# spiraldb/vortex

Hardware: AMD Instinct MI355X
Metric: decoded GB/s/GPU (device-resident) per encoding; % HBM roofline (higher is better)
Workload: dtype u32

## Files before the change

include/vortex_gpu.h:

```cpp
#ifndef VORTEX_GPU_H
#define VORTEX_GPU_H

#include <stddef.h>
#include <stdint.h>

#ifdef __cplusplus
extern "C" {
#endif

#define VXG_ABI_VERSION 10

typedef enum vxg_status {
    VXG_OK = 0,
    VXG_ERR_OUT_OF_BOUNDS = 1,
    VXG_ERR_COMPUTE = 2,
    VXG_ERR_INVALID_ARGUMENT = 3,
    VXG_ERR_INVALID_SERDE = 4,
    VXG_ERR_NOT_IMPLEMENTED = 5,
    VXG_ERR_MISMATCHED_TYPES = 6,
    VXG_ERR_ASSERTION_FAILED = 7,
    VXG_ERR_HIP = 8,
    VXG_ERR_OUT_OF_MEMORY = 9
} vxg_status;

enum {
    VXG_ENC_BOOL = 2, VXG_ENC_PRIMITIVE = 3, VXG_ENC_STRUCT = 4, VXG_ENC_VARBIN = 5,
    VXG_ENC_VARBINVIEW = 6, VXG_ENC_SPARSE = 8, VXG_ENC_CONSTANT = 9, VXG_ENC_CHUNKED = 10,
    VXG_ENC_ALP = 17, VXG_ENC_BYTE_BOOL = 18, VXG_ENC_DICT = 20, VXG_ENC_FL_BITPACKED = 21,
    VXG_ENC_FL_DELTA = 22, VXG_ENC_FL_FOR = 23, VXG_ENC_FSST = 24, VXG_ENC_ROARING_BOOL = 25, VXG_ENC_RUN_END = 27,
    VXG_ENC_RUN_END_BOOL = 28, VXG_ENC_ZIGZAG = 29, VXG_ENC_ALP_RD = 30
};

enum {
    VXG_U8 = 0, VXG_U16 = 1, VXG_U32 = 2, VXG_U64 = 3, VXG_I8 = 4, VXG_I16 = 5, VXG_I32 = 6,
    VXG_I64 = 7, VXG_F16 = 8, VXG_F32 = 9, VXG_F64 = 10
};

enum { VXG_DTYPE_NULL = 0, VXG_DTYPE_BOOL = 1, VXG_DTYPE_PRIMITIVE = 2, VXG_DTYPE_UTF8 = 3,
       VXG_DTYPE_BINARY = 4 };

enum { VXG_VALIDITY_NON_NULLABLE = 0, VXG_VALIDITY_ALL_VALID = 1, VXG_VALIDITY_ALL_INVALID = 2,
       VXG_VALIDITY_ARRAY = 3 };

typedef struct vxg_buffer {
    const void* ptr;
    uint64_t len;
} vxg_buffer;

typedef union vxg_meta {
    struct { uint8_t bit_width; uint8_t has_patches; uint16_t offset; } bitpacked;
    struct { uint64_t reference; uint8_t shift; } for_;
    struct { uint64_t deltas_len; uint16_t offset; } delta;
    struct { uint8_t e; uint8_t f; uint8_t has_patches; } alp;
    struct { uint8_t right_bit_width; uint8_t dict_len; uint8_t left_parts_ptype;
             uint8_t has_exceptions; uint16_t dict[8]; } alprd;
    struct { uint8_t codes_ptype; uint64_t values_len; } dict;
    struct { uint64_t symbols_len; uint8_t codes_nullable; uint8_t uncompressed_lengths_ptype; } fsst;
    struct { uint8_t ends_ptype; uint64_t num_runs; uint64_t offset; } runend;
    struct { uint64_t indices_offset; uint64_t indices_len; uint8_t fill_is_null; uint8_t fill[16]; } sparse;
    struct { uint8_t is_null; uint8_t scalar[16]; } constant;
    struct { uint64_t nchunks; } chunked;
    struct { uint8_t offsets_ptype; uint64_t bytes_len; } varbin;
    struct { uint8_t first_byte_bit_offset; } boolean;
    struct { uint8_t start; uint8_t ends_ptype; uint64_t num_runs; uint64_t offset; } runendbool;
    struct { uint32_t n_buffers; } varbinview;
    uint64_t raw[5];
} vxg_meta;

typedef struct vxg_array {
    uint16_t encoding;
    uint8_t dtype;
    uint8_t ptype;
    uint8_t nullable;
    uint8_t validity;
    uint16_t reserved;
    uint64_t len;
    vxg_meta meta;
    uint32_t n_buffers;
    uint32_t n_children;
    const vxg_buffer* buffers;
    const struct vxg_array* children;
} vxg_array;

typedef struct vxg_data_buffer {
    uint64_t offset;
    uint64_t len;
} vxg_data_buffer;

typedef struct vxg_canonical {
    uint16_t kind;
    uint8_t ptype;
    uint8_t dtype;
    uint32_t reserved;
    uint64_t len;
    void* values;
    uint64_t values_bytes;
    void* views;
    void* data;
    uint64_t data_bytes;
    void* validity;
    uint32_t n_data_buffers;
    uint32_t data_buffers_cap;
    vxg_data_buffer* data_buffers;
} vxg_canonical;

typedef struct vxg_ctx vxg_ctx;

int vxg_abi_version(void);
vxg_status vxg_open(int device, vxg_ctx** out);
vxg_status vxg_close(vxg_ctx* ctx);
const char* vxg_last_error(void);
vxg_status vxg_alloc(vxg_ctx* ctx, uint64_t bytes, void** dptr);
vxg_status vxg_free(vxg_ctx* ctx, void* dptr);
vxg_status vxg_host_alloc(vxg_ctx* ctx, uint64_t bytes, void** hptr);
vxg_status vxg_host_free(vxg_ctx* ctx, void* hptr);
vxg_status vxg_memcpy_h2d(vxg_ctx* ctx, void* dst, const void* src, uint64_t bytes, void* stream);
vxg_status vxg_memcpy_d2h(vxg_ctx* ctx, void* dst, const void* src, uint64_t bytes, void* stream);
vxg_status vxg_memcpy_d2d(vxg_ctx* ctx, void* dst, const void* src, uint64_t bytes, void* stream);
vxg_status vxg_stream_sync(vxg_ctx* ctx, void* stream);

typedef enum vxg_option {
    VXG_OPT_K1W_MIN_GROUPS = 1,
    VXG_OPT_K1W_BPW = 2,
    VXG_OPT_K1_WAVE = 3
} vxg_option;
vxg_status vxg_set_option(vxg_ctx* ctx, int option, int64_t value);
vxg_status vxg_get_option(vxg_ctx* ctx, int option, int64_t* value);

typedef struct vxg_launch_stats {
    uint64_t k1w_launches;
    uint64_t k1w_last_groups;
    uint32_t k1w_last_bpw;
    uint32_t k1w_last_bpw_max;
    uint32_t k1w_min_bpw;
    uint32_t k1w_max_bpw;
} vxg_launch_stats;
vxg_status vxg_get_launch_stats(vxg_ctx* ctx, vxg_launch_stats* out, int reset);

vxg_status vxg_canonical_size(vxg_ctx* ctx, const vxg_array* a, uint64_t* values_bytes,
                              uint64_t* data_bytes);
vxg_status vxg_canonicalize(vxg_ctx* ctx, const vxg_array* a, vxg_canonical* out, void* stream);

vxg_status vxg_canonical_layout(vxg_ctx* ctx, const vxg_array* a, uint64_t* values_bytes,
                                uint64_t* data_bytes, vxg_data_buffer* bufs, uint32_t cap,
                                uint32_t* n_bufs);

typedef struct vxg_plan vxg_plan;
enum { VXG_PLAN_MEASURE = 1 };
vxg_status vxg_plan_create(vxg_ctx* ctx, const vxg_array* arrays, vxg_canonical* outs, uint32_t n,
                           vxg_plan** plan);
vxg_status vxg_plan_create_ex(vxg_ctx* ctx, const vxg_array* arrays, vxg_canonical* outs, uint32_t n,
                              uint32_t flags, vxg_plan** plan);
vxg_status vxg_plan_launch(vxg_plan* plan, void* stream);
vxg_status vxg_plan_destroy(vxg_plan* plan);

typedef struct vxg_plan_info {
    uint32_t batched;
    uint32_t branches;
    uint32_t direct_nodes;
    uint32_t n_candidates;
    uint32_t candidate_batched[2];
    float candidate_ms[2];
    float create_ms;
    uint32_t selection;
    uint32_t candidate_cost[2];
    uint32_t reserved;
} vxg_plan_info;
vxg_status vxg_plan_get_info(const vxg_plan* plan, vxg_plan_info* info);

typedef enum vxg_plan_selection {
    VXG_PLAN_SEL_SINGLE = 0,
    VXG_PLAN_SEL_FASTER = 1,
    VXG_PLAN_SEL_TIE_COST = 2,
    VXG_PLAN_SEL_UNMEASURED = 3
} vxg_plan_selection;
uint32_t vxg_plan_select(const float* ms, const uint32_t* cost, uint32_t n, uint32_t* selection);


vxg_status vxg_bitunpack(vxg_ctx* ctx, int ptype, unsigned bit_width, unsigned offset,
                         uint64_t len, const void* packed, uint64_t packed_bytes, void* out,
                         void* stream);

vxg_status vxg_bitunpack_for(vxg_ctx* ctx, int ptype, unsigned bit_width, unsigned offset,
                             uint64_t len, const void* packed, uint64_t packed_bytes,
                             uint64_t reference, unsigned shift, int zigzag, void* out,
                             void* stream);

vxg_status vxg_bitunpack_alp(vxg_ctx* ctx, int float_ptype, unsigned bit_width, unsigned offset,
                             uint64_t len, const void* packed, uint64_t packed_bytes,
                             uint64_t for_reference, unsigned for_shift, unsigned e, unsigned f,
                             void* out, void* stream);

vxg_status vxg_bitunpack_dict(vxg_ctx* ctx, int codes_ptype, unsigned bit_width,
                              unsigned offset, uint64_t len, const void* packed,
                              uint64_t packed_bytes, const void* dict_values,
                              uint64_t dict_len, unsigned value_width, void* out, void* stream);

vxg_status vxg_patch(vxg_ctx* ctx, int ptype, void* out, uint64_t out_len, int indices_ptype,
                     const void* indices, uint64_t indices_offset, const void* values,
                     uint64_t n_patches, void* stream);

vxg_status vxg_for_decode(vxg_ctx* ctx, int ptype, const void* in, uint64_t n,
                          uint64_t reference, unsigned shift, void* out, void* stream);

vxg_status vxg_zigzag_decode(vxg_ctx* ctx, int out_ptype, const void* in, uint64_t n, void* out,
                             void* stream);

vxg_status vxg_alp_decode(vxg_ctx* ctx, int float_ptype, const void* encoded, uint64_t n,
                          unsigned e, unsigned f, void* out, void* stream);

vxg_status vxg_alprd_decode(vxg_ctx* ctx, int float_ptype, const uint16_t* left_codes,
                            const uint16_t* dict_host, unsigned dict_len, unsigned right_bw,
                            const void* right, uint64_t n, const uint64_t* exc_pos,
                            const uint16_t* exc_vals, uint64_t n_exc, void* out, void* stream);

vxg_status vxg_take(vxg_ctx* ctx, unsigned value_width, const void* values, uint64_t n_values,
                    int codes_ptype, const void* codes, uint64_t n, void* out, void* stream);

vxg_status vxg_delta_decode(vxg_ctx* ctx, int ptype, const void* bases, uint64_t n_bases,
                            const void* deltas, uint64_t n_deltas, uint64_t offset,
                            uint64_t len, void* out, void* stream);

vxg_status vxg_runend_decode(vxg_ctx* ctx, unsigned value_width, const void* values,
                             int ends_ptype, const void* ends, uint64_t n_runs, uint64_t offset,
                             uint64_t len, void* out, void* stream);

uint64_t vxg_fsst_scratch_bytes(uint64_t n);
vxg_status vxg_fsst_decode(vxg_ctx* ctx, const uint64_t* symbols, const uint8_t* sym_lens,
                           unsigned n_symbols, const uint8_t* code_bytes, int offs_ptype,
                           const void* code_offsets, int lens_ptype, const void* lens, uint64_t n,
                           const uint8_t* validity, void* scratch, uint8_t* heap,
                           uint8_t* views, void* stream);

vxg_status vxg_runend_bool_decode(vxg_ctx* ctx, int ends_ptype, const void* ends, uint64_t n_runs,
                                  uint64_t offset, int start, uint64_t len, void* out_bits,
                                  uint64_t out_bit_offset, void* stream);

vxg_status vxg_bytebool_to_bits(vxg_ctx* ctx, const uint8_t* bytes, uint64_t n, void* out_bits,
                                uint64_t out_bit_offset, void* stream);

vxg_status vxg_fill(vxg_ctx* ctx, unsigned value_width, const void* scalar_host, uint64_t n,
                    void* out, void* stream);

vxg_status vxg_take_array(vxg_ctx* ctx, const vxg_array* a, int indices_ptype, const void* indices,
                          uint64_t n_indices, vxg_canonical* out, void* stream);

vxg_status vxg_filter_array(vxg_ctx* ctx, const vxg_array* a, const vxg_array* predicate, vxg_canonical* out,
                            void* stream);

typedef enum vxg_cmp_op { VXG_CMP_EQ = 0, VXG_CMP_NOT_EQ = 1, VXG_CMP_GT = 2, VXG_CMP_GTE = 3,
                          VXG_CMP_LT = 4, VXG_CMP_LTE = 5 } vxg_cmp_op;
enum { VXG_CMP_NULL_AS_FALSE = 1 };
typedef struct vxg_compare_info {
    uint32_t fused_launches;
    uint32_t fused_chunks;
    uint32_t fallback_arrays;
    uint32_t patch_launches;
} vxg_compare_info;
vxg_status vxg_compare_scalar(vxg_ctx* ctx, const vxg_array* a, int op, const void* scalar_host,
                              uint32_t flags, vxg_canonical* out, vxg_compare_info* info, void* stream);

typedef struct vxg_compare_bytes_info {
    uint32_t dict_launches;
    uint32_t dict_chunks;
    uint32_t table_launches;
    uint32_t direct_launches;
    uint32_t direct_chunks;
    uint32_t fallback_arrays;
} vxg_compare_bytes_info;
vxg_status vxg_compare_bytes(vxg_ctx* ctx, const vxg_array* a, int op, const void* scalar_host,
                             uint64_t scalar_len, uint32_t flags, vxg_canonical* out,
                             vxg_compare_bytes_info* info, void* stream);

typedef struct vxg_int_stats {
    uint64_t n;
    uint64_t min_bits;
    uint64_t max_bits;
// ... 46 lines not shown
```

rust/vortex-gpu/src/ffi.rs:

```rust
#![allow(non_camel_case_types, non_upper_case_globals, dead_code)]

use std::os::raw::{c_char, c_int, c_uint, c_void};

pub const VXG_ABI_VERSION: c_int = 10;
pub type vxg_status = c_int;
pub const VXG_OK: vxg_status = 0;
pub const VXG_ERR_OUT_OF_BOUNDS: vxg_status = 1;
pub const VXG_ERR_COMPUTE: vxg_status = 2;
pub const VXG_ERR_INVALID_ARGUMENT: vxg_status = 3;
pub const VXG_ERR_INVALID_SERDE: vxg_status = 4;
pub const VXG_ERR_NOT_IMPLEMENTED: vxg_status = 5;
pub const VXG_ERR_MISMATCHED_TYPES: vxg_status = 6;
pub const VXG_ERR_ASSERTION_FAILED: vxg_status = 7;
pub const VXG_ERR_HIP: vxg_status = 8;
pub const VXG_ERR_OUT_OF_MEMORY: vxg_status = 9;
pub const VXG_ENC_BOOL: c_int = 2;
pub const VXG_ENC_PRIMITIVE: c_int = 3;
pub const VXG_ENC_STRUCT: c_int = 4;
pub const VXG_ENC_VARBIN: c_int = 5;
pub const VXG_ENC_VARBINVIEW: c_int = 6;
pub const VXG_ENC_SPARSE: c_int = 8;
pub const VXG_ENC_CONSTANT: c_int = 9;
pub const VXG_ENC_CHUNKED: c_int = 10;
pub const VXG_ENC_ALP: c_int = 17;
// ... 71 lines not shown
pub struct vxg_meta_alprd {
    pub right_bit_width: u8,
    pub dict_len: u8,
    pub left_parts_ptype: u8,
    pub has_exceptions: u8,
    pub dict: [u16; 8],
}

#[repr(C)]
#[derive(Copy, Clone, Debug)]
pub struct vxg_meta_dict {
    pub codes_ptype: u8,
    pub values_len: u64,
}

#[repr(C)]
#[derive(Copy, Clone, Debug)]
pub struct vxg_meta_fsst {
    pub symbols_len: u64,
    pub codes_nullable: u8,
    pub uncompressed_lengths_ptype: u8,
}

#[repr(C)]
#[derive(Copy, Clone, Debug)]
pub struct vxg_meta_runend {
    pub ends_ptype: u8,
    pub num_runs: u64,
    pub offset: u64,
}

#[repr(C)]
#[derive(Copy, Clone, Debug)]
pub struct vxg_meta_sparse {
    pub indices_offset: u64,
    pub indices_len: u64,
    pub fill_is_null: u8,
    pub fill: [u8; 16],
}

#[repr(C)]
#[derive(Copy, Clone, Debug)]
pub struct vxg_meta_constant {
    pub is_null: u8,
    pub scalar: [u8; 16],
}

#[repr(C)]
#[derive(Copy, Clone, Debug)]
pub struct vxg_meta_chunked {
    pub nchunks: u64,
}

#[repr(C)]
#[derive(Copy, Clone, Debug)]
pub struct vxg_meta_varbin {
    pub offsets_ptype: u8,
    pub bytes_len: u64,
}

#[repr(C)]
#[derive(Copy, Clone, Debug)]
pub struct vxg_meta_boolean {
    pub first_byte_bit_offset: u8,
}

#[repr(C)]
#[derive(Copy, Clone, Debug)]
pub struct vxg_meta_runendbool {
    pub start: u8,
    pub ends_ptype: u8,
    pub num_runs: u64,
    pub offset: u64,
}

#[repr(C)]
#[derive(Copy, Clone, Debug)]
pub struct vxg_meta_varbinview {
    pub n_buffers: u32,
}

#[repr(C)]
#[derive(Copy, Clone)]
pub union vxg_meta {
    pub bitpacked: vxg_meta_bitpacked,
    pub for_: vxg_meta_for_,
    pub delta: vxg_meta_delta,
    pub alp: vxg_meta_alp,
    pub alprd: vxg_meta_alprd,
    pub dict: vxg_meta_dict,
    pub fsst: vxg_meta_fsst,
    pub runend: vxg_meta_runend,
    pub sparse: vxg_meta_sparse,
    pub constant: vxg_meta_constant,
    pub chunked: vxg_meta_chunked,
    pub varbin: vxg_meta_varbin,
    pub boolean: vxg_meta_boolean,
    pub runendbool: vxg_meta_runendbool,
    pub varbinview: vxg_meta_varbinview,
    pub raw: [u64; 5],
}

#[repr(C)]
#[derive(Copy, Clone, Debug)]
pub struct vxg_array {
    pub encoding: u16,
    pub dtype: u8,
    pub ptype: u8,
    pub nullable: u8,
    pub validity: u8,
    pub reserved: u16,
    pub len: u64,
    pub meta: vxg_meta,
    pub n_buffers: u32,
    pub n_children: u32,
    pub buffers: *const vxg_buffer,
    pub children: *const vxg_array,
}

#[repr(C)]
#[derive(Copy, Clone, Debug)]
pub struct vxg_data_buffer {
    pub offset: u64,
    pub len: u64,
}

#[repr(C)]
#[derive(Copy, Clone, Debug)]
pub struct vxg_canonical {
    pub kind: u16,
    pub ptype: u8,
    pub dtype: u8,
    pub reserved: u32,
    pub len: u64,
    pub values: *mut c_void,
    pub values_bytes: u64,
    pub views: *mut c_void,
    pub data: *mut c_void,
    pub data_bytes: u64,
    pub validity: *mut c_void,
    pub n_data_buffers: u32,
    pub data_buffers_cap: u32,
    pub data_buffers: *mut vxg_data_buffer,
}

#[repr(C)]
pub struct vxg_ctx {
    _private: [u8; 0],
}
pub type vxg_option = c_int;
pub const VXG_OPT_K1W_MIN_GROUPS: vxg_option = 1;
pub const VXG_OPT_K1W_BPW: vxg_option = 2;
pub const VXG_OPT_K1_WAVE: vxg_option = 3;

#[repr(C)]
#[derive(Copy, Clone, Debug)]
pub struct vxg_launch_stats {
    pub k1w_launches: u64,
    pub k1w_last_groups: u64,
    pub k1w_last_bpw: u32,
    pub k1w_last_bpw_max: u32,
    pub k1w_min_bpw: u32,
    pub k1w_max_bpw: u32,
}

#[repr(C)]
pub struct vxg_plan {
    _private: [u8; 0],
}
pub const VXG_PLAN_MEASURE: c_int = 1;

#[repr(C)]
#[derive(Copy, Clone, Debug)]
pub struct vxg_plan_info {
    pub batched: u32,
    pub branches: u32,
    pub direct_nodes: u32,
    pub n_candidates: u32,
    pub candidate_batched: [u32; 2],
    pub candidate_ms: [f32; 2],
    pub create_ms: f32,
    pub selection: u32,
    pub candidate_cost: [u32; 2],
    pub reserved: u32,
}
pub type vxg_plan_selection = c_int;
pub const VXG_PLAN_SEL_SINGLE: vxg_plan_selection = 0;
pub const VXG_PLAN_SEL_FASTER: vxg_plan_selection = 1;
pub const VXG_PLAN_SEL_TIE_COST: vxg_plan_selection = 2;
pub const VXG_PLAN_SEL_UNMEASURED: vxg_plan_selection = 3;
pub type vxg_cmp_op = c_int;
pub const VXG_CMP_EQ: vxg_cmp_op = 0;
pub const VXG_CMP_NOT_EQ: vxg_cmp_op = 1;
pub const VXG_CMP_GT: vxg_cmp_op = 2;
pub const VXG_CMP_GTE: vxg_cmp_op = 3;
pub const VXG_CMP_LT: vxg_cmp_op = 4;
pub const VXG_CMP_LTE: vxg_cmp_op = 5;
pub const VXG_CMP_NULL_AS_FALSE: c_int = 1;

#[repr(C)]
#[derive(Copy, Clone, Debug)]
pub struct vxg_compare_info {
    pub fused_launches: u32,
    pub fused_chunks: u32,
    pub fallback_arrays: u32,
    pub patch_launches: u32,
}

#[repr(C)]
#[derive(Copy, Clone, Debug)]
pub struct vxg_compare_bytes_info {
    pub dict_launches: u32,
    pub dict_chunks: u32,
    pub table_launches: u32,
    pub direct_launches: u32,
    pub direct_chunks: u32,
    pub fallback_arrays: u32,
}

#[repr(C)]
#[derive(Copy, Clone, Debug)]
pub struct vxg_int_stats {
    pub n: u64,
    pub min_bits: u64,
    pub max_bits: u64,
    pub trailing_zeros: u32,
    pub reserved: u32,
    pub bit_width_freq: [u64; 65],
}

#[repr(C)]
#[derive(Copy, Clone, Debug)]
pub struct vxg_dict_chunk {
    pub packed: *const c_void,
    pub dict_values: *const c_void,
    pub out: *mut c_void,
    pub n_blocks: u64,
    pub len: u64,
    pub dict_len: u64,
}

#[repr(C)]
pub struct vxg_file {
    _private: [u8; 0],
}

#[repr(C)]
#[derive(Copy, Clone, Debug)]
pub struct vxg_file_column {
    pub name: *const c_char,
    pub dtype: u8,
    pub ptype: u8,
    pub nullable: u8,
    pub is_extension: u8,
    pub n_chunks: u32,
    pub extension_id: *const c_char,
    pub extension_metadata: *const u8,
    pub extension_metadata_len: u64,
    pub rows: u64,
}

#[repr(C)]
#[derive(Copy, Clone, Debug)]
pub struct vxg_file_chunk {
    pub row_offset: u64,
    pub rows: u64,
    pub message_begin: u64,
    pub message_end: u64,
    pub buffers_begin: u64,
}

#[link(name = "vortex_gpu")]
extern "C" {
    pub fn vxg_abi_version() -> c_int;
    pub fn vxg_open(device: c_int, out: *mut *mut vxg_ctx) -> vxg_status;
    pub fn vxg_close(ctx: *mut vxg_ctx) -> vxg_status;
    pub fn vxg_last_error() -> *const c_char;
    pub fn vxg_alloc(ctx: *mut vxg_ctx, bytes: u64, dptr: *mut *mut c_void) -> vxg_status;
    pub fn vxg_free(ctx: *mut vxg_ctx, dptr: *mut c_void) -> vxg_status;
    pub fn vxg_host_alloc(ctx: *mut vxg_ctx, bytes: u64, hptr: *mut *mut c_void) -> vxg_status;
    pub fn vxg_host_free(ctx: *mut vxg_ctx, hptr: *mut c_void) -> vxg_status;
    pub fn vxg_memcpy_h2d(ctx: *mut vxg_ctx, dst: *mut c_void, src: *const c_void, bytes: u64, stream: *mut c_void) -> vxg_status;
    pub fn vxg_memcpy_d2h(ctx: *mut vxg_ctx, dst: *mut c_void, src: *const c_void, bytes: u64, stream: *mut c_void) -> vxg_status;
    pub fn vxg_memcpy_d2d(ctx: *mut vxg_ctx, dst: *mut c_void, src: *const c_void, bytes: u64, stream: *mut c_void) -> vxg_status;
    pub fn vxg_stream_sync(ctx: *mut vxg_ctx, stream: *mut c_void) -> vxg_status;
    pub fn vxg_set_option(ctx: *mut vxg_ctx, option: c_int, value: i64) -> vxg_status;
    pub fn vxg_get_option(ctx: *mut vxg_ctx, option: c_int, value: *mut i64) -> vxg_status;
    pub fn vxg_get_launch_stats(ctx: *mut vxg_ctx, out: *mut vxg_launch_stats, reset: c_int) -> vxg_status;
    pub fn vxg_canonical_size(ctx: *mut vxg_ctx, a: *const vxg_array, values_bytes: *mut u64, data_bytes: *mut u64) -> vxg_status;
    pub fn vxg_canonicalize(ctx: *mut vxg_ctx, a: *const vxg_array, out: *mut vxg_canonical, stream: *mut c_void) -> vxg_status;
    pub fn vxg_canonical_layout(ctx: *mut vxg_ctx, a: *const vxg_array, values_bytes: *mut u64, data_bytes: *mut u64, bufs: *mut vxg_data_buffer, cap: u32, n_bufs: *mut u32) -> vxg_status;
    pub fn vxg_plan_create(ctx: *mut vxg_ctx, arrays: *const vxg_array, outs: *mut vxg_canonical, n: u32, plan: *mut *mut vxg_plan) -> vxg_status;
    pub fn vxg_plan_create_ex(ctx: *mut vxg_ctx, arrays: *const vxg_array, outs: *mut vxg_canonical, n: u32, flags: u32, plan: *mut *mut vxg_plan) -> vxg_status;
    pub fn vxg_plan_launch(plan: *mut vxg_plan, stream: *mut c_void) -> vxg_status;
    pub fn vxg_plan_destroy(plan: *mut vxg_plan) -> vxg_status;
    pub fn vxg_plan_get_info(plan: *const vxg_plan, info: *mut vxg_plan_info) -> vxg_status;
    pub fn vxg_plan_select(ms: *const f32, cost: *const u32, n: u32, selection: *mut u32) -> u32;
    pub fn vxg_bitunpack(ctx: *mut vxg_ctx, ptype: c_int, bit_width: c_uint, offset: c_uint, len: u64, packed: *const c_void, packed_bytes: u64, out: *mut c_void, stream: *mut c_void) -> vxg_status;
    pub fn vxg_bitunpack_for(ctx: *mut vxg_ctx, ptype: c_int, bit_width: c_uint, offset: c_uint, len: u64, packed: *const c_void, packed_bytes: u64, reference: u64, shift: c_uint, zigzag: c_int, out: *mut c_void, stream: *mut c_void) -> vxg_status;
    pub fn vxg_bitunpack_alp(ctx: *mut vxg_ctx, float_ptype: c_int, bit_width: c_uint, offset: c_uint, len: u64, packed: *const c_void, packed_bytes: u64, for_reference: u64, for_shift: c_uint, e: c_uint, f: c_uint, out: *mut c_void, stream: *mut c_void) -> vxg_status;
    pub fn vxg_bitunpack_dict(ctx: *mut vxg_ctx, codes_ptype: c_int, bit_width: c_uint, offset: c_uint, len: u64, packed: *const c_void, packed_bytes: u64, dict_values: *const c_void, dict_len: u64, value_width: c_uint, out: *mut c_void, stream: *mut c_void) -> vxg_status;
    pub fn vxg_patch(ctx: *mut vxg_ctx, ptype: c_int, out: *mut c_void, out_len: u64, indices_ptype: c_int, indices: *const c_void, indices_offset: u64, values: *const c_void, n_patches: u64, stream: *mut c_void) -> vxg_status;
    pub fn vxg_for_decode(ctx: *mut vxg_ctx, ptype: c_int, r#in: *const c_void, n: u64, reference: u64, shift: c_uint, out: *mut c_void, stream: *mut c_void) -> vxg_status;
    pub fn vxg_zigzag_decode(ctx: *mut vxg_ctx, out_ptype: c_int, r#in: *const c_void, n: u64, out: *mut c_void, stream: *mut c_void) -> vxg_status;
    pub fn vxg_alp_decode(ctx: *mut vxg_ctx, float_ptype: c_int, encoded: *const c_void, n: u64, e: c_uint, f: c_uint, out: *mut c_void, stream: *mut c_void) -> vxg_status;
    pub fn vxg_alprd_decode(ctx: *mut vxg_ctx, float_ptype: c_int, left_codes: *const u16, dict_host: *const u16, dict_len: c_uint, right_bw: c_uint, right: *const c_void, n: u64, exc_pos: *const u64, exc_vals: *const u16, n_exc: u64, out: *mut c_void, stream: *mut c_void) -> vxg_status;
// ... 29 lines not shown
```

vortex_amd/_lib.py:

```python
from __future__ import annotations

import ctypes as C
import os
from pathlib import Path

_HERE = Path(__file__).resolve().parent
GPU_LIB_PATH = Path(os.environ["VXG_GPU_LIB"]) if os.environ.get("VXG_GPU_LIB") else _HERE / "libvortex_gpu.so"
ENC_LIB_PATH = _HERE / "libvortex_enc.so"

ENC = dict(BOOL=2, PRIMITIVE=3, STRUCT=4, VARBIN=5, VARBINVIEW=6, SPARSE=8, CONSTANT=9,
           CHUNKED=10, ALP=17, BYTE_BOOL=18, DICT=20, FL_BITPACKED=21, FL_DELTA=22, FL_FOR=23,
           FSST=24, ROARING_BOOL=25, RUN_END=27, RUN_END_BOOL=28, ZIGZAG=29, ALP_RD=30)
PTYPES = ["u8", "u16", "u32", "u64", "i8", "i16", "i32", "i64", "f16", "f32", "f64"]
PTYPE = {n: i for i, n in enumerate(PTYPES)}
DTYPE = dict(NULL=0, BOOL=1, PRIMITIVE=2, UTF8=3, BINARY=4)
VALIDITY = dict(NON_NULLABLE=0, ALL_VALID=1, ALL_INVALID=2, ARRAY=3)
ABI_VERSION = 10
STATUS = {0: "OK", 1: "OutOfBounds", 2: "ComputeError", 3: "InvalidArgument", 4: "InvalidSerde",
          5: "NotImplemented", 6: "MismatchedTypes", 7: "AssertionFailed", 8: "HipError",
          9: "OutOfMemory"}


class VortexGpuError(RuntimeError):

    def __init__(self, status: int, msg: str):
        super().__init__(f"{STATUS.get(status, status)}: {msg}")
        self.status = status
        self.kind = STATUS.get(status, str(status))


class VxgBuffer(C.Structure):
    _fields_ = [("ptr", C.c_void_p), ("len", C.c_uint64)]


class _MBitPacked(C.Structure):
    _fields_ = [("bit_width", C.c_uint8), ("has_patches", C.c_uint8), ("offset", C.c_uint16)]


class _MFoR(C.Structure):
    _fields_ = [("reference", C.c_uint64), ("shift", C.c_uint8)]


class _MDelta(C.Structure):
    _fields_ = [("deltas_len", C.c_uint64), ("offset", C.c_uint16)]


class _MAlp(C.Structure):
    _fields_ = [("e", C.c_uint8), ("f", C.c_uint8), ("has_patches", C.c_uint8)]


class _MAlpRd(C.Structure):
    _fields_ = [("right_bit_width", C.c_uint8), ("dict_len", C.c_uint8),
                ("left_parts_ptype", C.c_uint8), ("has_exceptions", C.c_uint8),
                ("dict", C.c_uint16 * 8)]


class _MDict(C.Structure):
    _fields_ = [("codes_ptype", C.c_uint8), ("values_len", C.c_uint64)]


class _MFsst(C.Structure):
    _fields_ = [("symbols_len", C.c_uint64), ("codes_nullable", C.c_uint8),
                ("uncompressed_lengths_ptype", C.c_uint8)]


class _MRunEnd(C.Structure):
    _fields_ = [("ends_ptype", C.c_uint8), ("num_runs", C.c_uint64), ("offset", C.c_uint64)]


class _MSparse(C.Structure):
    _fields_ = [("indices_offset", C.c_uint64), ("indices_len", C.c_uint64),
                ("fill_is_null", C.c_uint8), ("fill", C.c_uint8 * 16)]


class _MConstant(C.Structure):
    _fields_ = [("is_null", C.c_uint8), ("scalar", C.c_uint8 * 16)]


class _MChunked(C.Structure):
    _fields_ = [("nchunks", C.c_uint64)]


class _MVarBin(C.Structure):
    _fields_ = [("offsets_ptype", C.c_uint8), ("bytes_len", C.c_uint64)]


class _MBool(C.Structure):
    _fields_ = [("first_byte_bit_offset", C.c_uint8)]


class _MRunEndBool(C.Structure):
    _fields_ = [("start", C.c_uint8), ("ends_ptype", C.c_uint8), ("num_runs", C.c_uint64),
                ("offset", C.c_uint64)]


class _MVarBinView(C.Structure):
    _fields_ = [("n_buffers", C.c_uint32)]


class VxgMeta(C.Union):
    _fields_ = [("bitpacked", _MBitPacked), ("for_", _MFoR), ("delta", _MDelta), ("alp", _MAlp),
                ("alprd", _MAlpRd), ("dict", _MDict), ("fsst", _MFsst), ("runend", _MRunEnd),
                ("sparse", _MSparse), ("constant", _MConstant), ("chunked", _MChunked),
                ("varbin", _MVarBin), ("boolean", _MBool), ("runendbool", _MRunEndBool),
                ("varbinview", _MVarBinView), ("raw", C.c_uint64 * 5)]


class VxgArray(C.Structure):
    pass


VxgArray._fields_ = [("encoding", C.c_uint16), ("dtype", C.c_uint8), ("ptype", C.c_uint8),
                     ("nullable", C.c_uint8), ("validity", C.c_uint8), ("reserved", C.c_uint16),
                     ("len", C.c_uint64), ("meta", VxgMeta), ("n_buffers", C.c_uint32),
                     ("n_children", C.c_uint32), ("buffers", C.POINTER(VxgBuffer)),
                     ("children", C.POINTER(VxgArray))]


class VxgDataBuffer(C.Structure):
    _fields_ = [("offset", C.c_uint64), ("len", C.c_uint64)]


class VxgCanonical(C.Structure):
    _fields_ = [("kind", C.c_uint16), ("ptype", C.c_uint8), ("dtype", C.c_uint8),
                ("reserved", C.c_uint32), ("len", C.c_uint64), ("values", C.c_void_p),
                ("values_bytes", C.c_uint64), ("views", C.c_void_p), ("data", C.c_void_p),
                ("data_bytes", C.c_uint64), ("validity", C.c_void_p),
                ("n_data_buffers", C.c_uint32), ("data_buffers_cap", C.c_uint32),
                ("data_buffers", C.POINTER(VxgDataBuffer))]


PLAN_MEASURE = 1


class VxgPlanInfo(C.Structure):
    _fields_ = [("batched", C.c_uint32), ("branches", C.c_uint32), ("direct_nodes", C.c_uint32),
                ("n_candidates", C.c_uint32), ("candidate_batched", C.c_uint32 * 2),
                ("candidate_ms", C.c_float * 2), ("create_ms", C.c_float), ("selection", C.c_uint32),
                ("candidate_cost", C.c_uint32 * 2), ("reserved", C.c_uint32)]


PLAN_SELECTION = {0: "single", 1: "faster", 2: "tie_fewer_nodes", 3: "unmeasured"}


OPT_K1W_MIN_GROUPS, OPT_K1W_BPW, OPT_K1_WAVE = 1, 2, 3


class VxgLaunchStats(C.Structure):
    _fields_ = [("k1w_launches", C.c_uint64), ("k1w_last_groups", C.c_uint64), ("k1w_last_bpw", C.c_uint32),
                ("k1w_last_bpw_max", C.c_uint32), ("k1w_min_bpw", C.c_uint32), ("k1w_max_bpw", C.c_uint32)]


CMP_OP = {"==": 0, "!=": 1, ">": 2, ">=": 3, "<": 4, "<=": 5}
CMP_NULL_AS_FALSE = 1


class VxgCompareInfo(C.Structure):
    _fields_ = [("fused_launches", C.c_uint32), ("fused_chunks", C.c_uint32), ("fallback_arrays", C.c_uint32),
                ("patch_launches", C.c_uint32)]


class VxgCompareBytesInfo(C.Structure):
    _fields_ = [("dict_launches", C.c_uint32), ("dict_chunks", C.c_uint32), ("table_launches", C.c_uint32),
                ("direct_launches", C.c_uint32), ("direct_chunks", C.c_uint32), ("fallback_arrays", C.c_uint32)]


class VxgIntStats(C.Structure):
    _fields_ = [("n", C.c_uint64), ("min_bits", C.c_uint64), ("max_bits", C.c_uint64), ("trailing_zeros", C.c_uint32),
                ("reserved", C.c_uint32), ("bit_width_freq", C.c_uint64 * 65)]


class VxgDictChunk(C.Structure):
    _fields_ = [("packed", C.c_void_p), ("dict_values", C.c_void_p), ("out", C.c_void_p),
                ("n_blocks", C.c_uint64), ("len", C.c_uint64), ("dict_len", C.c_uint64)]


assert C.sizeof(VxgMeta) == 40, C.sizeof(VxgMeta)
assert C.sizeof(VxgArray) == 80, C.sizeof(VxgArray)

VP, U64, U32, INT, UINT = C.c_void_p, C.c_uint64, C.c_uint32, C.c_int, C.c_uint
ST = C.c_int

GPU_SIGNATURES = {
    "vxg_abi_version": (C.c_int, []),
    "vxg_open": (ST, [INT, C.POINTER(VP)]),
    "vxg_close": (ST, [VP]),
    "vxg_last_error": (C.c_char_p, []),
    "vxg_alloc": (ST, [VP, U64, C.POINTER(VP)]),
    "vxg_free": (ST, [VP, VP]),
    "vxg_host_alloc": (ST, [VP, U64, C.POINTER(VP)]),
    "vxg_host_free": (ST, [VP, VP]),
    "vxg_memcpy_h2d": (ST, [VP, VP, VP, U64, VP]),
    "vxg_memcpy_d2h": (ST, [VP, VP, VP, U64, VP]),
    "vxg_memcpy_d2d": (ST, [VP, VP, VP, U64, VP]),
    "vxg_stream_sync": (ST, [VP, VP]),
    "vxg_set_option": (ST, [VP, INT, C.c_int64]),
    "vxg_get_option": (ST, [VP, INT, C.POINTER(C.c_int64)]),
    "vxg_get_launch_stats": (ST, [VP, C.POINTER(VxgLaunchStats), INT]),
    "vxg_canonical_size": (ST, [VP, C.POINTER(VxgArray), C.POINTER(U64), C.POINTER(U64)]),
    "vxg_canonicalize": (ST, [VP, C.POINTER(VxgArray), C.POINTER(VxgCanonical), VP]),
    "vxg_plan_create": (ST, [VP, C.POINTER(VxgArray), C.POINTER(VxgCanonical), U32, C.POINTER(VP)]),
    "vxg_plan_create_ex": (ST, [VP, C.POINTER(VxgArray), C.POINTER(VxgCanonical), U32, U32, C.POINTER(VP)]),
    "vxg_plan_get_info": (ST, [VP, C.c_void_p]),
    "vxg_plan_select": (U32, [C.POINTER(C.c_float), C.POINTER(U32), U32, C.POINTER(U32)]),
    "vxg_plan_launch": (ST, [VP, VP]),
    "vxg_plan_destroy": (ST, [VP]),
    "vxg_canonical_layout": (ST, [VP, C.POINTER(VxgArray), C.POINTER(U64), C.POINTER(U64),
                                  C.POINTER(VxgDataBuffer), U32, C.POINTER(U32)]),
    "vxg_bitunpack": (ST, [VP, INT, UINT, UINT, U64, VP, U64, VP, VP]),
    "vxg_bitunpack_for": (ST, [VP, INT, UINT, UINT, U64, VP, U64, U64, UINT, INT, VP, VP]),
    "vxg_bitunpack_alp": (ST, [VP, INT, UINT, UINT, U64, VP, U64, U64, UINT, UINT, UINT, VP, VP]),
    "vxg_bitunpack_dict": (ST, [VP, INT, UINT, UINT, U64, VP, U64, VP, U64, UINT, VP, VP]),
    "vxg_bitunpack_dict_chunks": (ST, [VP, INT, UINT, UINT, C.POINTER(VxgDictChunk), U32, VP]),
    "vxg_patch": (ST, [VP, INT, VP, U64, INT, VP, U64, VP, U64, VP]),
    "vxg_for_decode": (ST, [VP, INT, VP, U64, U64, UINT, VP, VP]),
    "vxg_zigzag_decode": (ST, [VP, INT, VP, U64, VP, VP]),
    "vxg_alp_decode": (ST, [VP, INT, VP, U64, UINT, UINT, VP, VP]),
    "vxg_alprd_decode": (ST, [VP, INT, VP, VP, UINT, UINT, VP, U64, VP, VP, U64, VP, VP]),
    "vxg_take": (ST, [VP, UINT, VP, U64, INT, VP, U64, VP, VP]),
    "vxg_delta_decode": (ST, [VP, INT, VP, U64, VP, U64, U64, U64, VP, VP]),
    "vxg_runend_decode": (ST, [VP, UINT, VP, INT, VP, U64, U64, U64, VP, VP]),
    "vxg_runend_bool_decode": (ST, [VP, INT, VP, U64, U64, INT, U64, VP, U64, VP]),
    "vxg_bytebool_to_bits": (ST, [VP, VP, U64, VP, U64, VP]),
    "vxg_take_array": (ST, [VP, VP, INT, VP, U64, VP, VP]),
    "vxg_filter_array": (ST, [VP, VP, VP, VP, VP]),
    "vxg_compare_scalar": (ST, [VP, VP, INT, VP, U32, VP, C.POINTER(VxgCompareInfo), VP]),
    "vxg_compare_bytes": (ST, [VP, VP, INT, VP, U64, U32, VP, C.POINTER(VxgCompareBytesInfo), VP]),
    "vxg_fsst_scratch_bytes": (U64, [U64]),
    "vxg_fsst_decode": (ST, [VP, VP, VP, UINT, VP, INT, VP, INT, VP, U64, VP, VP, VP, VP, VP]),
    "vxg_fill": (ST, [VP, UINT, VP, U64, VP, VP]),
    "vxg_compute_int_stats": (ST, [VP, INT, VP, U64, C.POINTER(VxgIntStats), VP]),
    "vxg_bitpack": (ST, [VP, INT, UINT, VP, U64, VP, U64, VP]),
    "vxg_for_encode": (ST, [VP, INT, VP, U64, U64, UINT, VP, VP]),
    "vxg_for_bitpack": (ST, [VP, INT, U64, UINT, UINT, VP, U64, VP, U64, VP]),
    "vxg_gather_patches": (ST, [VP, INT, UINT, VP, U64, VP, VP, U64, C.POINTER(U64), VP]),
    "vxg_alp_encode": (ST, [VP, INT, VP, U64, C.POINTER(C.c_uint8), C.POINTER(C.c_uint8), VP, VP, VP, U64,
                            C.POINTER(U64), VP]),
    "vxg_fsst_compress": (ST, [VP, VP, VP, C.c_uint32, INT, VP, VP, U64, VP, U64, VP, U64, VP, VP, C.POINTER(U64), VP]),
}

class VxgFileColumn(C.Structure):
    _fields_ = [("name", C.c_char_p), ("dtype", C.c_uint8), ("ptype", C.c_uint8), ("nullable", C.c_uint8),
                ("is_extension", C.c_uint8), ("n_chunks", C.c_uint32), ("extension_id", C.c_char_p),
                ("extension_metadata", C.POINTER(C.c_uint8)), ("extension_metadata_len", C.c_uint64),
                ("rows", C.c_uint64)]


class VxgFileChunk(C.Structure):
    _fields_ = [("row_offset", C.c_uint64), ("rows", C.c_uint64), ("message_begin", C.c_uint64),
                ("message_end", C.c_uint64), ("buffers_begin", C.c_uint64)]


FILE_SIGNATURES = {
    "vxg_file_open": (ST, [VP, U64, C.POINTER(VP)]),
    "vxg_file_close": (ST, [VP]),
    "vxg_file_info": (ST, [VP, C.POINTER(U64), C.POINTER(U32)]),
    "vxg_file_column_info": (ST, [VP, U32, C.POINTER(VxgFileColumn)]),
    "vxg_file_chunk_info": (ST, [VP, U32, U32, C.POINTER(VxgFileChunk)]),
    "vxg_file_chunk_offsets": (ST, [VP, U32, U32, U32, C.POINTER(U64)]),
    "vxg_file_column_array": (ST, [VP, U32, U32, U32, VP, U64, U64, VP, C.POINTER(C.POINTER(VxgArray))]),
}

ENC_SIGNATURES = {
    "vxe_bitpack": (U64, [INT, UINT, VP, U64, VP]),
    "vxe_roaring_bool_encode": (U64, [VP, U64, VP, U64]),
    "vxe_best_bit_width": (UINT, [INT, VP, U64]),
    "vxe_min_patchless_bit_width": (UINT, [INT, VP, U64]),
    "vxe_gather_patches": (U64, [INT, UINT, VP, U64, VP, VP, U64]),
    "vxe_for_compress": (INT, [INT, VP, U64, VP, C.POINTER(U64), C.POINTER(UINT)]),
    "vxe_delta_compress": (None, [INT, VP, U64, VP, VP]),
    "vxe_zigzag_encode": (None, [INT, VP, U64, VP]),
    "vxe_alp_encode_f64": (U64, [VP, U64, VP, VP, VP, VP, VP, U64]),
    "vxe_alp_encode_f32": (U64, [VP, U64, VP, VP, VP, VP, VP, U64]),
    "vxe_alprd_encode_f64": (U64, [VP, U64, VP, VP, VP, VP, VP, VP, VP, U64]),
    "vxe_alprd_encode_f32": (U64, [VP, U64, VP, VP, VP, VP, VP, VP, VP, U64]),
    "vxe_dict_encode": (U64, [INT, VP, U64, VP, VP, U64]),
    "vxe_runend_encode": (U64, [INT, VP, U64, VP, VP]),
    "vxe_fsst_train": (None, [VP, VP, U64, VP]),
    "vxe_fsst_compress": (U64, [VP, VP, VP, U64, VP, U64, VP]),
}


class VxeFsstTable(C.Structure):
    _fields_ = [("symbols", C.c_uint64 * 255), ("lens", C.c_uint8 * 255), ("n_symbols", C.c_uint32)]


def _load(path: Path, sigs: dict) -> C.CDLL:
    if not path.exists():
        raise ImportError(f"{path.name} is not built (run __graft_entry__.build() or make -C "
                          f"vortex_amd/csrc); the decode engine has no CPU fallback")
    lib = C.CDLL(str(path))
    for name, (res, args) in sigs.items():
        fn = getattr(lib, name)
        fn.restype = res
        fn.argtypes = args
    return lib


# ... 25 lines not shown
```

vortex_amd/arrays.py:

```python
from __future__ import annotations

import ctypes as C
from dataclasses import dataclass, field
from typing import Any, Optional, Sequence

import numpy as np

from . import _lib
from ._lib import DTYPE, ENC, PTYPE, PTYPES, VALIDITY, VortexGpuError

NP_OF_PTYPE = {"u8": np.uint8, "u16": np.uint16, "u32": np.uint32, "u64": np.uint64,
               "i8": np.int8, "i16": np.int16, "i32": np.int32, "i64": np.int64,
               "f16": np.float16, "f32": np.float32, "f64": np.float64}
PTYPE_OF_NP = {np.dtype(v): k for k, v in NP_OF_PTYPE.items()}


def ptype_width(p: str) -> int:
    return np.dtype(NP_OF_PTYPE[p]).itemsize


def unsigned_of(p: str) -> str:
    return "u" + p[1:] if p[0] == "i" else p


# ... 281 lines not shown

def varbin(offsets: Array, data: Array, utf8: bool = True, validity=None) -> Array:
    nullable = validity is not None
    vk, vchild = _validity_kind(nullable, validity)
    return Array(ENC["VARBIN"], offsets.len - 1, DTYPE["UTF8" if utf8 else "BINARY"], "u8", nullable,
                 vk, {"offsets_ptype": PTYPE[offsets.ptype], "bytes_len": data.len}, [],
                 [offsets, data] + ([vchild] if vchild is not None else []))


def varbinview(views, buffers: Sequence, utf8: bool = True, validity=None) -> Array:
    v = np.ascontiguousarray(views, dtype=np.uint8).reshape(-1)
    if v.size % 16:
        _bail("InvalidArgument", "views must be a multiple of 16 bytes")
    bufs = [np.ascontiguousarray(b, dtype=np.uint8).reshape(-1) for b in buffers]
    if any(b.size >= 2 ** 32 for b in bufs):
        _bail("InvalidArgument", "buffer must be within 32-bit range")
    nullable = validity is not None
    vk, vchild = _validity_kind(nullable, validity)
    return Array(ENC["VARBINVIEW"], v.size // 16, DTYPE["UTF8" if utf8 else "BINARY"], "u8", nullable, vk,
                 {"n_buffers": len(bufs)}, [],
                 [primitive(v)] + [primitive(b) for b in bufs] + ([vchild] if vchild is not None else []))


def fsst(symbols: Array, symbol_lengths: Array, codes: Array, uncompressed_lengths: Array,
         utf8: bool = True) -> Array:
    if symbols.len > 255:
        _bail("InvalidArgument", "symbols array must have length <= 255")
    if symbols.len != symbol_lengths.len:
        _bail("InvalidArgument", "symbols and symbol_lengths arrays must have same length")
    if uncompressed_lengths.len != codes.len:
        _bail("InvalidArgument", "uncompressed_lengths must be same len as codes")
    if codes.encoding != ENC["VARBIN"]:
        _bail("InvalidArgument", "codes array must be VarBin")
    return Array(ENC["FSST"], codes.len, DTYPE["UTF8" if utf8 else "BINARY"], "u8", codes.nullable,
                 VALIDITY["NON_NULLABLE"],
                 {"symbols_len": symbols.len, "codes_nullable": codes.nullable,
                  "uncompressed_lengths_ptype": PTYPE[uncompressed_lengths.ptype]}, [],
                 [symbols, symbol_lengths, codes, uncompressed_lengths])


def _fill_meta(m: _lib.VxgMeta, a: Array) -> None:
    md = a.meta
    e = a.encoding
    if e == ENC["FL_BITPACKED"]:
        m.bitpacked.bit_width, m.bitpacked.has_patches, m.bitpacked.offset = (
            md["bit_width"], int(md["has_patches"]), md["offset"])
    elif e == ENC["FL_FOR"]:
        m.for_.reference, m.for_.shift = md["reference"], md["shift"]
    elif e == ENC["FL_DELTA"]:
        m.delta.deltas_len, m.delta.offset = md["deltas_len"], md["offset"]
    elif e == ENC["ALP"]:
        m.alp.e, m.alp.f, m.alp.has_patches = md["e"], md["f"], int(md["has_patches"])
    elif e == ENC["ALP_RD"]:
        m.alprd.right_bit_width = md["right_bit_width"]
        m.alprd.dict_len = md["dict_len"]
        m.alprd.left_parts_ptype = md["left_parts_ptype"]
        m.alprd.has_exceptions = int(md["has_exceptions"])
        for i, v in enumerate(md["dict"]):
            m.alprd.dict[i] = v
    elif e == ENC["DICT"]:
        m.dict.codes_ptype, m.dict.values_len = md["codes_ptype"], md["values_len"]
    elif e == ENC["FSST"]:
        m.fsst.symbols_len = md["symbols_len"]
        m.fsst.codes_nullable = int(md["codes_nullable"])
        m.fsst.uncompressed_lengths_ptype = md["uncompressed_lengths_ptype"]
    elif e == ENC["RUN_END"]:
        m.runend.ends_ptype, m.runend.num_runs, m.runend.offset = (
            md["ends_ptype"], md["num_runs"], md["offset"])
    elif e == ENC["SPARSE"]:
        m.sparse.indices_offset = md["indices_offset"]
        m.sparse.indices_len = md["indices_len"]
        m.sparse.fill_is_null = int(md["fill_is_null"])
        for i, b in enumerate(md["fill"][:16]):
            m.sparse.fill[i] = b
    elif e == ENC["CONSTANT"]:
        m.constant.is_null = int(md["is_null"])
        for i, b in enumerate(md["scalar"][:16]):
            m.constant.scalar[i] = b
    elif e == ENC["CHUNKED"]:
        m.chunked.nchunks = md["nchunks"]
    elif e == ENC["VARBIN"]:
        m.varbin.offsets_ptype, m.varbin.bytes_len = md["offsets_ptype"], md["bytes_len"]
    elif e == ENC["BOOL"]:
        m.boolean.first_byte_bit_offset = md.get("first_byte_bit_offset", 0)
    elif e == ENC["RUN_END_BOOL"]:
        m.runendbool.start, m.runendbool.ends_ptype = int(md["start"]), md["ends_ptype"]
        m.runendbool.num_runs, m.runendbool.offset = md["num_runs"], md["offset"]
    elif e == ENC["VARBINVIEW"]:
        m.varbinview.n_buffers = md["n_buffers"]


def _buf_ptr(b) -> tuple[int, int]:
    import torch
    if not isinstance(b, torch.Tensor) or not b.is_cuda:
        raise VortexError(3, "array buffers must be device tensors: call Array.to(device) first")
    return b.data_ptr(), b.numel() * b.element_size()


def flatten(a: Array, keep: list) -> _lib.VxgArray:
    node = _lib.VxgArray()
    node.encoding = a.encoding
    node.dtype = a.dtype
    node.ptype = PTYPE[a.ptype]
    node.nullable = int(a.nullable)
    node.validity = a.validity
    node.len = a.len
    _fill_meta(node.meta, a)
    if a.buffers:
        bufs = (_lib.VxgBuffer * len(a.buffers))()
        for i, b in enumerate(a.buffers):
            bufs[i].ptr, bufs[i].len = _buf_ptr(b)
            keep.append(b)
        keep.append(bufs)
        node.buffers = C.cast(bufs, C.POINTER(_lib.VxgBuffer))
        node.n_buffers = len(a.buffers)
    if a.children:
        kids = (_lib.VxgArray * len(a.children))()
        for i, c in enumerate(a.children):
            kids[i] = flatten(c, keep)
        keep.append(kids)
        node.children = C.cast(kids, C.POINTER(_lib.VxgArray))
        node.n_children = len(a.children)
    return node


class Context:

    def __init__(self, device: int = 0):
        self.lib = _lib.gpu_lib()
        self.device = device
        h = C.c_void_p()
        _lib.check(self.lib.vxg_open(device, C.byref(h)))
        self.handle = h

    def close(self):
        if self.handle:
            self.lib.vxg_close(self.handle)
            self.handle = None

    def __del__(self):
        try:
            self.close()
        except Exception:
            pass

    def stream_ptr(self):
        import torch
        return C.c_void_p(torch.cuda.current_stream(self.device).cuda_stream)

    def sync(self):
        _lib.check(self.lib.vxg_stream_sync(self.handle, self.stream_ptr()))

    _OPTIONS = {"k1w_min_groups": _lib.OPT_K1W_MIN_GROUPS, "k1w_bpw": _lib.OPT_K1W_BPW,
                "k1_wave": _lib.OPT_K1_WAVE}

    def set_option(self, name: str, value: int):
        _lib.check(self.lib.vxg_set_option(self.handle, self._OPTIONS[name], int(value)))

    def get_option(self, name: str) -> int:
        v = C.c_int64()
        _lib.check(self.lib.vxg_get_option(self.handle, self._OPTIONS[name], C.byref(v)))
        return v.value

    def launch_stats(self, reset: bool = False) -> dict:
        st = _lib.VxgLaunchStats()
        _lib.check(self.lib.vxg_get_launch_stats(self.handle, C.byref(st), int(reset)))
        return {f: getattr(st, f) for f, _ in st._fields_}


@dataclass
class Canonical:
    kind: str
    len: int
    ptype: str
    values: Any = None
    views: Any = None
    data: Any = None
    validity: Any = None
    data_buffers: Any = None
    binary: bool = False
    info: Any = None

    def to_arrow(self):
        import pyarrow as pa
        validity = None if self.validity is None else pa.py_buffer(self.validity.cpu().numpy()[: (self.len + 7) // 8].copy())
        nulls = -1 if validity is not None else 0
        if self.kind == "primitive":
            t = {"u8": pa.uint8(), "u16": pa.uint16(), "u32": pa.uint32(), "u64": pa.uint64(), "i8": pa.int8(),
                 "i16": pa.int16(), "i32": pa.int32(), "i64": pa.int64(), "f16": pa.float16(), "f32": pa.float32(),
                 "f64": pa.float64()}[self.ptype]
            return pa.Array.from_buffers(t, self.len, [validity, pa.py_buffer(self.values.cpu().numpy().copy())],
                                         null_count=nulls)
        if self.kind == "bool":
            bits = self.values.cpu().numpy()[: (self.len + 7) // 8].copy()
            return pa.Array.from_buffers(pa.bool_(), self.len, [validity, pa.py_buffer(bits)], null_count=nulls)
        data = self.data.cpu().numpy()
        bufs = [pa.py_buffer(data[o: o + n].copy()) for o, n in self.data_buffers]
        views = pa.py_buffer(self.views.cpu().numpy()[: 16 * self.len].copy())
        return pa.Array.from_buffers(pa.binary_view() if self.binary else pa.string_view(), self.len,
                                     [validity, views] + bufs, null_count=nulls)

    def numpy(self):
        if self.kind == "primitive":
            return self.values.cpu().numpy().view(NP_OF_PTYPE[self.ptype])
        if self.kind == "bool":
            return np.unpackbits(self.values.cpu().numpy(), bitorder="little")[: self.len].astype(bool)
        return self.views.cpu().numpy().reshape(-1, 16), self.data.cpu().numpy()

    def buffers(self):
        d = self.data.cpu().numpy()
        return [d[o: o + n] for o, n in self.data_buffers]

    def validity_mask(self):
        if self.validity is None:
            return None
        bits = self.validity.cpu().numpy()
        return np.unpackbits(bits, bitorder="little")[: self.len].astype(bool)


def _kind(a: Array) -> str:
    return {DTYPE["PRIMITIVE"]: "primitive", DTYPE["BOOL"]: "bool"}.get(a.dtype, "varbinview")


def canonicalize(a: Array, ctx: Context, out_values=None, sync: bool = True) -> Canonical:
    import torch
    keep: list = []
    node = flatten(a, keep)
    dev = torch.device("cuda", ctx.device)
    vb, db, nb = C.c_uint64(), C.c_uint64(), C.c_uint32()
    cap = 256
    while True:
        table = (_lib.VxgDataBuffer * cap)()
        st = ctx.lib.vxg_canonical_layout(ctx.handle, C.byref(node), C.byref(vb), C.byref(db), table, cap,
                                          C.byref(nb))
        if st == 3 and cap < (1 << 24):
            cap *= 16
            continue
        _lib.check(st)
        break
    out = _lib.VxgCanonical()
    res = Canonical(_kind(a), a.len, a.ptype, binary=a.dtype == DTYPE["BINARY"])
    nbits = ((a.len + 31) // 32) * 4
    valid_t = torch.empty(max(nbits, 4), dtype=torch.uint8, device=dev) if a.nullable else None
    if a.dtype in (DTYPE["PRIMITIVE"], DTYPE["BOOL"]):
        vals = out_values if out_values is not None else torch.empty(max(vb.value, 16), dtype=torch.uint8, device=dev)
        out.values = vals.data_ptr()
        res.values = vals[: vb.value]
    else:
        views = torch.empty(max(vb.value, 16), dtype=torch.uint8, device=dev)
        data = torch.empty(db.value + 16, dtype=torch.uint8, device=dev)
        out.views, out.data = views.data_ptr(), data.data_ptr()
        out.data_bytes = db.value
        out.data_buffers, out.n_data_buffers, out.data_buffers_cap = table, nb.value, nb.value
        res.views, res.data = views[: vb.value], data[: db.value]
        res.data_buffers = [(int(table[i].offset), int(table[i].len)) for i in range(nb.value)]
    if valid_t is not None:
        out.validity = valid_t.data_ptr()
    _lib.check(ctx.lib.vxg_canonicalize(ctx.handle, C.byref(node), C.byref(out), ctx.stream_ptr()))
    if out.validity:
        if valid_t is None or out.validity != valid_t.data_ptr():
            raise VortexError(7, "engine allocated validity for a non-nullable dtype")
        res.validity = valid_t[: (a.len + 7) // 8]
    if sync:
        ctx.sync()
    return res


def take(a: Array, indices, ctx: Context, sync: bool = True) -> Canonical:
    import torch
    keep: list = []
    node = flatten(a, keep)
    dev = torch.device("cuda", ctx.device)
    if isinstance(indices, torch.Tensor):
        it = indices.to(dev)
        tmap = {torch.uint8: "u8", torch.int8: "i8", torch.int16: "i16", torch.int32: "i32", torch.int64: "i64"}
        for name, p in (("uint16", "u16"), ("uint32", "u32"), ("uint64", "u64")):
            if hasattr(torch, name):
                tmap[getattr(torch, name)] = p
        if it.dtype not in tmap:
            raise VortexError(3, f"take: indices must be integers, got {it.dtype}")
        ip = tmap[it.dtype]
    else:
        ia = np.ascontiguousarray(indices)
        if ia.dtype not in PTYPE_OF_NP or ia.dtype.kind not in "iu":
            raise VortexError(3, f"take: indices must be integers, got {ia.dtype}")
        ip = PTYPE_OF_NP[ia.dtype]
        it = torch.from_numpy(ia.view(np.uint8).copy()).to(dev)
    n = int(it.numel() if isinstance(indices, torch.Tensor) else np.asarray(indices).size)
    out = _lib.VxgCanonical()
    w = ptype_width(a.ptype)
    vals = torch.empty(max(n * w, 16), dtype=torch.uint8, device=dev)
    out.values = vals.data_ptr()
    vt = torch.empty(((n + 31) // 32) * 4 + 4, dtype=torch.uint8, device=dev) if a.nullable else None
    if vt is not None:
        out.validity = vt.data_ptr()
    _lib.check(ctx.lib.vxg_take_array(ctx.handle, C.byref(node), PTYPE[ip], C.c_void_p(it.data_ptr()), n,
                                      C.byref(out), ctx.stream_ptr()))
    res = Canonical("primitive", n, a.ptype, values=vals[: n * w])
    if out.validity:
        if vt is None or out.validity != vt.data_ptr():
            raise VortexError(7, "engine allocated validity for a non-nullable dtype")
        res.validity = vt[: (n + 7) // 8]
    if sync:
        ctx.sync()
    return res


# ... 182 lines not shown
```

vortex_amd/csrc/capi.hip:

```cpp
#include <algorithm>
#include <cstring>
#include <mutex>

#include "encode_gpu.hpp"
#include "planner.hpp"

namespace vxg {

const float kF10f[11] = {1.0f, 10.0f, 100.0f, 1000.0f, 10000.0f, 100000.0f, 1000000.0f,
                         10000000.0f, 100000000.0f, 1000000000.0f, 10000000000.0f};
const float kIF10f[11] = {1.0f, 0.1f, 0.01f, 0.001f, 0.0001f, 0.00001f, 0.000001f,
                          0.0000001f, 0.00000001f, 0.000000001f, 0.0000000001f};
const double kF10d[24] = {
    1.0, 10.0, 100.0, 1000.0, 10000.0, 100000.0, 1000000.0, 10000000.0, 100000000.0,
    1000000000.0, 10000000000.0, 100000000000.0, 1000000000000.0, 10000000000000.0,
    100000000000000.0, 1000000000000000.0, 10000000000000000.0, 100000000000000000.0,
    1000000000000000000.0, 10000000000000000000.0, 100000000000000000000.0,
    1000000000000000000000.0, 10000000000000000000000.0, 100000000000000000000000.0};
const double kIF10d[24] = {
    1.0, 0.1, 0.01, 0.001, 0.0001, 0.00001, 0.000001, 0.0000001, 0.00000001, 0.000000001,
    0.0000000001, 0.00000000001, 0.000000000001, 0.0000000000001, 0.00000000000001,
    0.000000000000001, 0.0000000000000001, 0.00000000000000001, 0.000000000000000001,
    0.0000000000000000001, 0.00000000000000000001, 0.000000000000000000001,
    0.0000000000000000000001, 0.00000000000000000000001};

static thread_local std::string g_last_error;

vxg_status set_error(vxg_status s, const std::string& msg) {
    if (s != VXG_OK) g_last_error = msg;
    return s;
}

vxg_status hip_check(hipError_t e, const char* what) {
    if (e == hipSuccess) return VXG_OK;
    return set_error(e == hipErrorOutOfMemory ? VXG_ERR_OUT_OF_MEMORY : VXG_ERR_HIP,
                     std::string(what) + ": " + hipGetErrorString(e));
}

thread_local Ctx* g_cur_ctx = nullptr;

Options default_options() {
    static const Options d = [] {
        Options o;
        o.k1w_min_groups = int64_t(env_int("VXG_K1W_MIN_GROUPS", INT64_MIN, INT64_MAX, o.k1w_min_groups));
        return o;
    }();
    return d;
}

vxg_status use_device(vxg_ctx* ctx) {
    if (!ctx) return set_error(VXG_ERR_INVALID_ARGUMENT, "null vxg_ctx");
    g_cur_ctx = &ctx->c;
    return hip_check(hipSetDevice(ctx->c.device), "hipSetDevice");
}

vxg_status status_of_err_word(uint32_t err) {
    if (err & kErrTakeOOB) return set_error(VXG_ERR_OUT_OF_BOUNDS, "take: index out of bounds");
    if (err & kErrPatchOOB) return set_error(VXG_ERR_OUT_OF_BOUNDS, "patch index out of bounds");
    if (err & kErrPatchOrder) return set_error(VXG_ERR_INVALID_ARGUMENT, "patch indices are not sorted");
    if (err & kErrRunEnd) return set_error(VXG_ERR_INVALID_ARGUMENT, "RunEnd ends do not cover the array");
    if (err & kErrFsst) return set_error(VXG_ERR_INVALID_ARGUMENT, "FSST codes do not decode to uncompressed_lengths");
    if (err & kErrRoaring) return set_error(VXG_ERR_INVALID_SERDE, "RoaringBool buffer is not a croaring Native bitmap");
    if (err & kErrVarBin) return set_error(VXG_ERR_INVALID_ARGUMENT, "VarBin offsets out of range of the bytes");
    if (err & kErrPlanSync)
        return set_error(VXG_ERR_ASSERTION_FAILED, "plan launch: in-grid pre-pass records never published "
                                                   "(overlapping replays of one plan?)");
    return set_error(VXG_ERR_ASSERTION_FAILED, "unknown device error bit");
}

}

using namespace vxg;

static vxg_status bitunpack_common(vxg_ctx* ctx, int T, unsigned W, unsigned offset, uint64_t len,
                                   const void* packed, uint64_t packed_bytes, Epi epi, int vw,
                                   UnpackArgs a, void* out, void* stream) {
    std::vector<K1Job> jobs(1);
    VXG_TRY(make_k1_job(T, W, offset, len, packed, packed_bytes, epi, vw, a, out, jobs[0]));
    return launch_k1_jobs(jobs, ctx->c.err_word, S(stream));
}

extern "C" {

int vxg_abi_version(void) { return VXG_ABI_VERSION; }

const char* vxg_last_error(void) { return g_last_error.c_str(); }

vxg_status vxg_open(int device, vxg_ctx** out) {
    if (!out) return set_error(VXG_ERR_INVALID_ARGUMENT, "null out");
    int n = 0;
    VXG_TRY(hip_check(hipGetDeviceCount(&n), "hipGetDeviceCount"));
    if (device < 0 || device >= n) return set_error(VXG_ERR_INVALID_ARGUMENT, "no such device");
    VXG_TRY(hip_check(hipSetDevice(device), "hipSetDevice"));
    auto* c = new vxg_ctx();
    c->c.device = device;
    c->c.opt = default_options();
    hipError_t e = hipMalloc(&c->c.err_word, 16);
    if (e == hipSuccess) e = hipMemset(c->c.err_word, 0, 16);
    if (e == hipSuccess) {
        hipMemPool_t pool;
        uint64_t keep = ~0ull;
        if (hipDeviceGetDefaultMemPool(&pool, device) == hipSuccess)
            (void)hipMemPoolSetAttribute(pool, hipMemPoolAttrReleaseThreshold, &keep);
    }
    if (e == hipSuccess) e = fsst_diag_init();
    if (e != hipSuccess) {
        vxg_close(c);
        return hip_check(e, "context setup");
    }
    *out = c;
    return VXG_OK;
}

vxg_status vxg_set_option(vxg_ctx* ctx, int option, int64_t value) {
    if (!ctx) return set_error(VXG_ERR_INVALID_ARGUMENT, "null vxg_ctx");
    Options& o = ctx->c.opt;
    switch (option) {
    case VXG_OPT_K1W_MIN_GROUPS:
        if (value < 0 || value > (int64_t(1) << 31)) return set_error(VXG_ERR_INVALID_ARGUMENT, "K1W_MIN_GROUPS out of range");
        o.k1w_min_groups = value;
        return VXG_OK;
    case VXG_OPT_K1W_BPW:
        if (value < 0 || value > 32) return set_error(VXG_ERR_INVALID_ARGUMENT, "K1W_BPW must be in [0, 32]");
        o.k1w_bpw = value;
        return VXG_OK;
    case VXG_OPT_K1_WAVE:
        if (value < -1 || value > 2) return set_error(VXG_ERR_INVALID_ARGUMENT, "K1_WAVE must be -1, 0, 1 or 2");
        o.k1_wave = value;
        return VXG_OK;
    }
    return set_error(VXG_ERR_INVALID_ARGUMENT, "unknown option " + std::to_string(option));
}

vxg_status vxg_get_option(vxg_ctx* ctx, int option, int64_t* value) {
    if (!ctx || !value) return set_error(VXG_ERR_INVALID_ARGUMENT, "null argument");
    const Options& o = ctx->c.opt;
    switch (option) {
    case VXG_OPT_K1W_MIN_GROUPS: *value = o.k1w_min_groups; return VXG_OK;
    case VXG_OPT_K1W_BPW: *value = o.k1w_bpw; return VXG_OK;
    case VXG_OPT_K1_WAVE: *value = o.k1_wave; return VXG_OK;
    }
    return set_error(VXG_ERR_INVALID_ARGUMENT, "unknown option " + std::to_string(option));
}

vxg_status vxg_get_launch_stats(vxg_ctx* ctx, vxg_launch_stats* out, int reset) {
    if (!ctx || !out) return set_error(VXG_ERR_INVALID_ARGUMENT, "null argument");
    std::lock_guard<std::mutex> lk(ctx->c.mu);
    const LaunchStats& st = ctx->c.st;
    *out = vxg_launch_stats{};
    out->k1w_launches = st.k1w_launches;
    out->k1w_last_groups = st.k1w_last_groups;
    out->k1w_last_bpw = st.k1w_last_bpw;
    out->k1w_min_bpw = st.k1w_min_bpw;
    out->k1w_max_bpw = st.k1w_max_bpw;
    out->k1w_last_bpw_max = st.k1w_last_bpw_max;
    if (reset) ctx->c.st = LaunchStats{};
    return VXG_OK;
}

vxg_status vxg_close(vxg_ctx* ctx) {
    if (!ctx) return VXG_OK;
    if (g_cur_ctx == &ctx->c) g_cur_ctx = nullptr;
    (void)hipSetDevice(ctx->c.device);
    (void)hipDeviceSynchronize();
    if (ctx->c.err_word) (void)hipFree(ctx->c.err_word);
    delete ctx;
    return VXG_OK;
}

vxg_status vxg_alloc(vxg_ctx* ctx, uint64_t bytes, void** dptr) {
    VXG_TRY(use_device(ctx));
    return hip_check(hipMalloc(dptr, bytes ? bytes : 16), "hipMalloc");
}

vxg_status vxg_free(vxg_ctx* ctx, void* dptr) {
    VXG_TRY(use_device(ctx));
    return hip_check(hipFree(dptr), "hipFree");
}

vxg_status vxg_host_alloc(vxg_ctx* ctx, uint64_t bytes, void** hptr) {
    VXG_TRY(use_device(ctx));
    return hip_check(hipHostMalloc(hptr, bytes ? bytes : 16, hipHostMallocDefault), "hipHostMalloc");
}

vxg_status vxg_host_free(vxg_ctx* ctx, void* hptr) {
    VXG_TRY(use_device(ctx));
    return hip_check(hipHostFree(hptr), "hipHostFree");
}

vxg_status vxg_memcpy_h2d(vxg_ctx* ctx, void* dst, const void* src, uint64_t bytes, void* stream) {
    VXG_TRY(use_device(ctx));
    return hip_check(hipMemcpyAsync(dst, src, bytes, hipMemcpyHostToDevice, S(stream)), "h2d");
}

vxg_status vxg_memcpy_d2h(vxg_ctx* ctx, void* dst, const void* src, uint64_t bytes, void* stream) {
    VXG_TRY(use_device(ctx));
    return hip_check(hipMemcpyAsync(dst, src, bytes, hipMemcpyDeviceToHost, S(stream)), "d2h");
}

vxg_status vxg_memcpy_d2d(vxg_ctx* ctx, void* dst, const void* src, uint64_t bytes, void* stream) {
    VXG_TRY(use_device(ctx));
    return hip_check(hipMemcpyAsync(dst, src, bytes, hipMemcpyDeviceToDevice, S(stream)), "d2d");
}

vxg_status vxg_stream_sync(vxg_ctx* ctx, void* stream) {
    VXG_TRY(use_device(ctx));
    VXG_TRY(hip_check(hipStreamSynchronize(S(stream)), "hipStreamSynchronize"));
    uint32_t err = 0;
    VXG_TRY(hip_check(hipMemcpy(&err, ctx->c.err_word, 4, hipMemcpyDeviceToHost), "error word readback"));
    if (err) {
        VXG_TRY(hip_check(hipMemset(ctx->c.err_word, 0, 4), "error word reset"));
        return status_of_err_word(err);
    }
    return VXG_OK;
}

vxg_status vxg_canonical_size(vxg_ctx* ctx, const vxg_array* a, uint64_t* values_bytes, uint64_t* data_bytes) {
    VXG_TRY(use_device(ctx));
    if (!a) return set_error(VXG_ERR_INVALID_ARGUMENT, "null array");
    Planner p(ctx, nullptr);
    uint64_t vb = 0, db = 0;
    VXG_TRY(p.canonical_size(*a, vb, db));
    if (values_bytes) *values_bytes = vb;
    if (data_bytes) *data_bytes = db;
    return VXG_OK;
}

vxg_status vxg_canonical_layout(vxg_ctx* ctx, const vxg_array* a, uint64_t* values_bytes, uint64_t* data_bytes,
                                vxg_data_buffer* bufs, uint32_t cap, uint32_t* n_bufs) {
    VXG_TRY(use_device(ctx));
    if (!a) return set_error(VXG_ERR_INVALID_ARGUMENT, "null array");
    Planner p(ctx, nullptr);
    uint64_t vb = 0, db = 0;
    uint32_t n = 0;
    if (is_string(*a)) {
        std::vector<vxg_data_buffer> v;
        VXG_TRY(p.string_layout(*a, v, db));
        vb = 16 * a->len;
        n = uint32_t(v.size());
        if (bufs && cap < n) return set_error(VXG_ERR_INVALID_ARGUMENT, "buffer table too small");
        if (bufs) std::copy(v.begin(), v.end(), bufs);
    } else {
        VXG_TRY(p.canonical_size(*a, vb, db));
    }
    if (values_bytes) *values_bytes = vb;
    if (data_bytes) *data_bytes = db;
    if (n_bufs) *n_bufs = n;
    return VXG_OK;
}

vxg_status vxg_canonicalize(vxg_ctx* ctx, const vxg_array* a, vxg_canonical* out, void* stream) {
    VXG_TRY(use_device(ctx));
    if (!a || !out) return set_error(VXG_ERR_INVALID_ARGUMENT, "null array/out");
    Planner p(ctx, S(stream));
    return p.canonical(*a, *out);
}

static int unsigned_T(int ptype) { return 8 * ptype_width(ptype); }

vxg_status vxg_bitunpack(vxg_ctx* ctx, int ptype, unsigned bit_width, unsigned offset, uint64_t len,
                         const void* packed, uint64_t packed_bytes, void* out, void* stream) {
    VXG_TRY(use_device(ctx));
    if (!ptype_is_int(ptype)) return set_error(VXG_ERR_MISMATCHED_TYPES, "BitPacked needs an integer ptype");
    return bitunpack_common(ctx, unsigned_T(ptype), bit_width, offset, len, packed, packed_bytes, Epi::Plain, 0,
                            UnpackArgs{}, out, stream);
}

vxg_status vxg_bitunpack_for(vxg_ctx* ctx, int ptype, unsigned bit_width, unsigned offset, uint64_t len,
                             const void* packed, uint64_t packed_bytes, uint64_t reference, unsigned shift,
                             int zigzag, void* out, void* stream) {
    VXG_TRY(use_device(ctx));
    if (!ptype_is_int(ptype)) return set_error(VXG_ERR_MISMATCHED_TYPES, "FoR needs an integer ptype");
    UnpackArgs a{};
    a.reference = reference;
    a.shift = shift;
    return bitunpack_common(ctx, unsigned_T(ptype), bit_width, offset, len, packed, packed_bytes,
                            zigzag ? Epi::ForZigZag : Epi::For, 0, a, out, stream);
}

vxg_status vxg_bitunpack_alp(vxg_ctx* ctx, int float_ptype, unsigned bit_width, unsigned offset, uint64_t len,
                             const void* packed, uint64_t packed_bytes, uint64_t for_reference,
                             unsigned for_shift, unsigned e, unsigned f, void* out, void* stream) {
    VXG_TRY(use_device(ctx));
    const bool f32 = float_ptype == VXG_F32;
    if (!f32 && float_ptype != VXG_F64) return set_error(VXG_ERR_MISMATCHED_TYPES, "ALP decodes to f32/f64");
    if ((f32 && (e > 10 || f > 10)) || (!f32 && (e > 23 || f > 23)))
        return set_error(VXG_ERR_INVALID_ARGUMENT, "ALP exponents out of range");
    UnpackArgs a{};
    a.reference = for_reference;
    a.shift = for_shift;
    a.alp_a = f32 ? double(kF10f[f]) : kF10d[f];
    a.alp_b = f32 ? double(kIF10f[e]) : kIF10d[e];
    return bitunpack_common(ctx, f32 ? 32 : 64, bit_width, offset, len, packed, packed_bytes,
                            f32 ? Epi::AlpF32 : Epi::AlpF64, 0, a, out, stream);
}

vxg_status vxg_bitunpack_dict(vxg_ctx* ctx, int codes_ptype, unsigned bit_width, unsigned offset, uint64_t len,
                              const void* packed, uint64_t packed_bytes, const void* dict_values,
                              uint64_t dict_len, unsigned value_width, void* out, void* stream) {
    VXG_TRY(use_device(ctx));
    if (!ptype_is_unsigned(codes_ptype)) return set_error(VXG_ERR_MISMATCHED_TYPES, "Dict codes must be unsigned");
    if (bit_width > unsigned(kDictFusedMaxW))
        return set_error(VXG_ERR_NOT_IMPLEMENTED, "fused dict decode supports code widths <= 16");
    UnpackArgs a{};
    a.dict = dict_values;
    a.dict_len = dict_len;
    return bitunpack_common(ctx, unsigned_T(codes_ptype), bit_width, offset, len, packed, packed_bytes, Epi::Dict,
                            int(value_width), a, out, stream);
}

vxg_status vxg_bitunpack_dict_chunks(vxg_ctx* ctx, int codes_ptype, unsigned bit_width, unsigned value_width,
                                     const vxg_dict_chunk* chunks_host, uint32_t n_chunks, void* stream) {
    VXG_TRY(use_device(ctx));
    if (!ptype_is_unsigned(codes_ptype)) return set_error(VXG_ERR_MISMATCHED_TYPES, "Dict codes must be unsigned");
    if (bit_width > unsigned(kDictFusedMaxW))
        return set_error(VXG_ERR_NOT_IMPLEMENTED, "fused dict decode supports code widths <= 16");
    std::vector<K1Job> jobs(n_chunks);
    for (uint32_t i = 0; i < n_chunks; i++) {
        const vxg_dict_chunk& c = chunks_host[i];
        if (c.n_blocks != (c.len + 1023) / 1024)
            return set_error(VXG_ERR_INVALID_ARGUMENT, "chunk n_blocks != ceil(len/1024)");
        UnpackArgs a{};
        a.dict = c.dict_values;
        a.dict_len = c.dict_len;
        VXG_TRY(make_k1_job(unsigned_T(codes_ptype), bit_width, 0, c.len, c.packed, c.n_blocks * 128ull * bit_width,
                            Epi::Dict, int(value_width), a, c.out, jobs[i]));
    }
    return launch_k1_jobs(jobs, ctx->c.err_word, S(stream));
}

vxg_status vxg_patch(vxg_ctx* ctx, int ptype, void* out, uint64_t out_len, int indices_ptype, const void* indices,
                     uint64_t indices_offset, const void* values, uint64_t n_patches, void* stream) {
    VXG_TRY(use_device(ctx));
    const int w = ptype_width(ptype);
    if (!w || !ptype_is_int(indices_ptype)) return set_error(VXG_ERR_INVALID_ARGUMENT, "bad ptype");
    UnpackArgs a{};
    a.err = ctx->c.err_word;
    IntCol ic{};
    ic.p = indices;
    ic.width = ptype_width(indices_ptype);
    ic.sgn = ptype_is_signed(indices_ptype);
    return launch_patch(0, ic, Epi::Plain, 8 * w, out, out_len, indices_offset, values, n_patches, a, S(stream));
}

vxg_status vxg_for_decode(vxg_ctx* ctx, int ptype, const void* in, uint64_t n, uint64_t reference,
                          unsigned shift, void* out, void* stream) {
    VXG_TRY(use_device(ctx));
    if (!ptype_is_int(ptype)) return set_error(VXG_ERR_MISMATCHED_TYPES, "FoR needs an integer ptype");
    return launch_for(ptype_width(ptype), in, n, reference, shift, false, out, S(stream));
}

vxg_status vxg_zigzag_decode(vxg_ctx* ctx, int out_ptype, const void* in, uint64_t n, void* out, void* stream) {
    VXG_TRY(use_device(ctx));
    if (!ptype_is_signed(out_ptype)) return set_error(VXG_ERR_MISMATCHED_TYPES, "ZigZag decodes to signed ints");
    return launch_zigzag(ptype_width(out_ptype), in, n, out, S(stream));
}

vxg_status vxg_alp_decode(vxg_ctx* ctx, int float_ptype, const void* encoded, uint64_t n, unsigned e, unsigned f,
                          void* out, void* stream) {
    VXG_TRY(use_device(ctx));
    const bool f32 = float_ptype == VXG_F32;
    if ((f32 && (e > 10 || f > 10)) || (!f32 && (e > 23 || f > 23)))
        return set_error(VXG_ERR_INVALID_ARGUMENT, "ALP exponents out of range");
    return launch_alp(float_ptype, encoded, n, f32 ? double(kF10f[f]) : kF10d[f],
                      f32 ? double(kIF10f[e]) : kIF10d[e], out, S(stream));
}

vxg_status vxg_alprd_decode(vxg_ctx* ctx, int float_ptype, const uint16_t* left_codes, const uint16_t* dict_host,
                            unsigned dict_len, unsigned right_bw, const void* right, uint64_t n,
                            const uint64_t* exc_pos, const uint16_t* exc_vals, uint64_t n_exc, void* out,
                            void* stream) {
    VXG_TRY(use_device(ctx));
    if (dict_len > 8) return set_error(VXG_ERR_INVALID_ARGUMENT, "ALP-RD dictionary holds at most 8 entries");
    return launch_alprd(float_ptype, left_codes, dict_host, dict_len, right_bw, right, n, exc_pos, 8, false, 0,
                        exc_vals, n_exc, out, ctx->c.err_word, S(stream));
}

vxg_status vxg_take(vxg_ctx* ctx, unsigned value_width, const void* values, uint64_t n_values, int codes_ptype,
                    const void* codes, uint64_t n, void* out, void* stream) {
    VXG_TRY(use_device(ctx));
    if (!ptype_is_unsigned(codes_ptype)) return set_error(VXG_ERR_MISMATCHED_TYPES, "take indices must be unsigned");
    return launch_take(int(value_width), values, n_values, ptype_width(codes_ptype), ptype_is_signed(codes_ptype), codes, n, out,
                       ctx->c.err_word, S(stream));
}

vxg_status vxg_delta_decode(vxg_ctx* ctx, int ptype, const void* bases, uint64_t n_bases, const void* deltas,
                            uint64_t n_deltas, uint64_t offset, uint64_t len, void* out, void* stream) {
    VXG_TRY(use_device(ctx));
    const int w = ptype_width(ptype);
    if (!ptype_is_unsigned(ptype)) return set_error(VXG_ERR_MISMATCHED_TYPES, "Delta decodes unsigned ints");
    const uint64_t lanes = 1024 / (8 * w);
    if (n_bases != (n_deltas / 1024) * lanes + (n_deltas % 1024 ? 1 : 0))
        return set_error(VXG_ERR_INVALID_ARGUMENT, "DeltaArray: bases.len() != expected_bases_len");
    if (offset + len > n_deltas) return set_error(VXG_ERR_INVALID_ARGUMENT, "offset + len > deltas len");
    return launch_delta(w, bases, deltas, n_deltas, offset, len, out, S(stream));
}

vxg_status vxg_runend_decode(vxg_ctx* ctx, unsigned value_width, const void* values, int ends_ptype,
                             const void* ends, uint64_t n_runs, uint64_t offset, uint64_t len, void* out,
                             void* stream) {
    VXG_TRY(use_device(ctx));
    if (!ptype_is_int(ends_ptype)) return set_error(VXG_ERR_MISMATCHED_TYPES, "RunEnd ends must be integers");
    RunEndChunk c{};
    c.ends.p = ends;
    c.ends.width = ptype_width(ends_ptype);
    c.ends.sgn = ptype_is_signed(ends_ptype);
    c.values.p = values;
    c.values.width = int(value_width);
    c.out = out;
    c.n_runs = n_runs;
    c.offset = offset;
    c.len = len;
    return launch_runend(int(value_width), c, ctx->c.err_word, S(stream));
}

vxg_status vxg_take_array(vxg_ctx* ctx, const vxg_array* a, int indices_ptype, const void* indices,
                          uint64_t n_indices, vxg_canonical* out, void* stream) {
    VXG_TRY(use_device(ctx));
    if (!a || !out || (n_indices && !indices)) return set_error(VXG_ERR_INVALID_ARGUMENT, "null array/indices/out");
    if (!ptype_is_int(indices_ptype)) return set_error(VXG_ERR_INVALID_ARGUMENT, "take indices must be integers");
    Planner p(ctx, S(stream));
    return p.take(*a, indices, ptype_width(indices_ptype), ptype_is_signed(indices_ptype), n_indices, *out);
}

vxg_status vxg_compare_scalar(vxg_ctx* ctx, const vxg_array* a, int op, const void* scalar_host, uint32_t flags,
                              vxg_canonical* out, vxg_compare_info* info, void* stream) {
    VXG_TRY(use_device(ctx));
    if (!a || !out || !scalar_host) return set_error(VXG_ERR_INVALID_ARGUMENT, "null array/scalar/out");
    uint64_t bits = 0;
    if (a->dtype == VXG_DTYPE_PRIMITIVE) std::memcpy(&bits, scalar_host, size_t(ptype_width(a->ptype)));
    vxg_compare_info ci{};
    Planner p(ctx, S(stream));
    void* const values_in = out->values;
    void* const validity_in = out->validity;
    const vxg_status st = p.compare(*a, op, bits, flags, *out, ci);
    if (info) *info = ci;
    if (st != VXG_OK) {
        if (out->values && out->values != values_in) (void)hipFree(out->values);
        if (out->validity && out->validity != validity_in) (void)hipFree(out->validity);
        out->values = values_in;
        out->validity = validity_in;
    }
    return st;
}

// ... 185 lines not shown
```

vortex_amd/csrc/chunk_pack.hpp:

```cpp
#pragma once

#include <algorithm>
#include <type_traits>

#include "vxg_internal.hpp"

namespace vxg {

template <class Tab, class It, class Entry, class Groups>
vxg_status pack_chunk_table(Tab& tab, It& it, It end, DevTables* dt, Entry entry, Groups groups_of, uint64_t* groups) {
    using E = std::remove_reference_t<decltype(tab.c[0])>;
    constexpr size_t cap = sizeof(tab.c) / sizeof(tab.c[0]);
    size_t take = 0;
    for (It k = it; k != end; ++k) take += entry(*k) != nullptr;
    E* cs = tab.c;
    if (dt && take > cap) {
        if (take > 0xFFFFFFFFull) return set_error(VXG_ERR_INVALID_ARGUMENT, "too many chunks");
        E* host;
        const vxg_status st = dt->table(take, &host, &tab.ext);
        if (st != VXG_OK) return st;
        if constexpr (requires { tab.host; }) tab.host = host;
        cs = host;
    } else {
        take = std::min(take, cap);
    }
    tab.n = 0;
    *groups = 0;
    for (; it != end && tab.n < take; ++it) {
        const E* e = entry(*it);
        if (!e) continue;
        E& c = cs[tab.n++];
        c = *e;
        c.first_group = *groups;
        *groups += groups_of(c);
    }
    while (it != end && !entry(*it)) ++it;
    if (*groups > 0xFFFFFFFFull) return set_error(VXG_ERR_INVALID_ARGUMENT, "array too long for one launch");
    return VXG_OK;
}

}
```

vortex_amd/csrc/compare.hip:

```cpp
#include "compare_impl.hpp"

namespace vxg {

namespace {

template <int OP, class V>
__device__ __forceinline__ bool cmp_op(V v, V s) {
    if constexpr (OP == VXG_CMP_EQ) return v == s;
    else if constexpr (OP == VXG_CMP_NOT_EQ) return v != s;
    else if constexpr (OP == VXG_CMP_GT) return v > s;
    else if constexpr (OP == VXG_CMP_GTE) return v >= s;
    else if constexpr (OP == VXG_CMP_LT) return v < s;
    else return v <= s;
}

template <class V>
__device__ __forceinline__ bool cmp_rt(int op, V v, V s) {
    switch (op) {
    case VXG_CMP_EQ: return v == s;
    case VXG_CMP_NOT_EQ: return v != s;
    case VXG_CMP_GT: return v > s;
    case VXG_CMP_GTE: return v >= s;
    case VXG_CMP_LT: return v < s;
    default: return v <= s;
    }
}

template <class O, int CK>
using CmpV = std::conditional_t<CK == kCmpSigned, std::make_signed_t<std::conditional_t<std::is_integral_v<O>, O, int>>, O>;

template <class V>
__device__ __forceinline__ V scalar_of(uint64_t bits) {
    V s;
    __builtin_memcpy(&s, &bits, sizeof(V));
    return s;
}

template <Epi EPI>
__device__ __forceinline__ void alp_factors(uint32_t e, uint32_t f, double& a, double& b) {
    if constexpr (EPI == Epi::AlpF32) {
        constexpr float f10[11] = {1.0f, 10.0f, 100.0f, 1000.0f, 10000.0f, 100000.0f, 1000000.0f,
                                   10000000.0f, 100000000.0f, 1000000000.0f, 10000000000.0f};
        constexpr float if10[11] = {1.0f, 0.1f, 0.01f, 0.001f, 0.0001f, 0.00001f, 0.000001f,
                                    0.0000001f, 0.00000001f, 0.000000001f, 0.0000000001f};
        a = double(f10[f < 11 ? f : 0]);
        b = double(if10[e < 11 ? e : 0]);
    } else if constexpr (EPI == Epi::AlpF64) {
        constexpr double f10[24] = {
            1.0, 10.0, 100.0, 1000.0, 10000.0, 100000.0, 1000000.0, 10000000.0, 100000000.0,
            1000000000.0, 10000000000.0, 100000000000.0, 1000000000000.0, 10000000000000.0,
            100000000000000.0, 1000000000000000.0, 10000000000000000.0, 100000000000000000.0,
            1000000000000000000.0, 10000000000000000000.0, 100000000000000000000.0,
            1000000000000000000000.0, 10000000000000000000000.0, 100000000000000000000000.0};
        constexpr double if10[24] = {
            1.0, 0.1, 0.01, 0.001, 0.0001, 0.00001, 0.000001, 0.0000001, 0.00000001, 0.000000001,
            0.0000000001, 0.00000000001, 0.000000000001, 0.0000000000001, 0.00000000000001,
            0.000000000000001, 0.0000000000000001, 0.00000000000000001, 0.000000000000000001,
            0.0000000000000000001, 0.00000000000000000001, 0.000000000000000000001,
            0.0000000000000000000001, 0.00000000000000000000001};
        a = f10[f < 24 ? f : 0];
        b = if10[e < 24 ? e : 0];
    } else {
        a = b = 0.0;
    }
}

template <int T, Epi EPI, int CK, int OP>
struct EpiPred {
    using E = typename Fl<T>::E;
    using V = CmpV<typename EpiOut<T, EPI, 0>::type, CK>;
    static constexpr bool kChecks = false;
    EpiParams ep;
    V s;
    __device__ __forceinline__ bool test(E raw) const { return cmp_op<OP>(V(apply_epi<T, EPI, 0>(raw, ep)), s); }
    __device__ __forceinline__ void check(bool) const {}
};

template <int T, Epi EPI, int CK, int OP>
__device__ __forceinline__ void cmp_chunk(const CmpChunk& c, uint32_t g, uint64_t* __restrict__ out, uint64_t sbits,
                                          uint8_t* lds) {
    using P = EpiPred<T, EPI, CK, OP>;
    cmp_blocks<T>(c, g, out, lds, [&] {
        EpiParams ep{};
        ep.reference = c.reference;
        ep.shift = c.shift;
        alp_factors<EPI>(c.alp_e, c.alp_f, ep.alp_a, ep.alp_b);
        return P{ep, scalar_of<typename P::V>(sbits)};
    });
}

template <int T, Epi EPI, int CK>
__global__ __launch_bounds__(kCmpThreads) void cmp_packed_kernel(CmpTable tab, uint64_t* __restrict__ out,
                                                                 uint64_t sbits, int op) {
    extern __shared__ __attribute__((aligned(16))) uint8_t cmp_lds[];
    const uint32_t g = blockIdx.x;
    uint32_t lo = 0, hi = tab.n;
    while (hi - lo > 1) {
        const uint32_t mid = (lo + hi) >> 1;
        if (tab.c[mid].first_group <= g) lo = mid; else hi = mid;
    }
    const CmpChunk& c = tab.c[lo];
    switch (op) {
    case VXG_CMP_EQ: cmp_chunk<T, EPI, CK, VXG_CMP_EQ>(c, g, out, sbits, cmp_lds); break;
    case VXG_CMP_NOT_EQ: cmp_chunk<T, EPI, CK, VXG_CMP_NOT_EQ>(c, g, out, sbits, cmp_lds); break;
    case VXG_CMP_GT: cmp_chunk<T, EPI, CK, VXG_CMP_GT>(c, g, out, sbits, cmp_lds); break;
    case VXG_CMP_GTE: cmp_chunk<T, EPI, CK, VXG_CMP_GTE>(c, g, out, sbits, cmp_lds); break;
    case VXG_CMP_LT: cmp_chunk<T, EPI, CK, VXG_CMP_LT>(c, g, out, sbits, cmp_lds); break;
    default: cmp_chunk<T, EPI, CK, VXG_CMP_LTE>(c, g, out, sbits, cmp_lds); break;
    }
}

template <class V, int OP>
__device__ __forceinline__ void cmp_plain_body(const V* __restrict__ in, uint64_t n, uint64_t* __restrict__ out,
                                               uint64_t out_bit, V s, bool excl) {
    const uint32_t l = threadIdx.x & 63;
    const int64_t cb = int64_t(out_bit), ce = int64_t(out_bit + n);
    const int64_t first = cb >> 6, n_words = ((ce + 63) >> 6) - first;
    const int64_t waves = int64_t(gridDim.x) * (kCmpThreads / 64);
    for (int64_t w = int64_t(blockIdx.x) * (kCmpThreads / 64) + (threadIdx.x >> 6); w < n_words; w += waves) {
        const int64_t i = (first + w) * 64 + int64_t(l) - cb;
        const bool in_range = i >= 0 && uint64_t(i) < n;
        const V v = in_range ? gload(in + i) : V(0);
        const uint64_t bal = __ballot(in_range && cmp_op<OP>(v, s));
        if (l == 0) put_word(out, first + w, bal, true, excl, cb, ce);
    }
}

template <class V>
__global__ __launch_bounds__(kCmpThreads) void cmp_plain_kernel(const V* __restrict__ in, uint64_t n,
                                                                uint64_t* __restrict__ out, uint64_t out_bit,
                                                                uint64_t sbits, int op, int excl) {
    const V s = scalar_of<V>(sbits);
    switch (op) {
    case VXG_CMP_EQ: cmp_plain_body<V, VXG_CMP_EQ>(in, n, out, out_bit, s, excl != 0); break;
    case VXG_CMP_NOT_EQ: cmp_plain_body<V, VXG_CMP_NOT_EQ>(in, n, out, out_bit, s, excl != 0); break;
    case VXG_CMP_GT: cmp_plain_body<V, VXG_CMP_GT>(in, n, out, out_bit, s, excl != 0); break;
    case VXG_CMP_GTE: cmp_plain_body<V, VXG_CMP_GTE>(in, n, out, out_bit, s, excl != 0); break;
    case VXG_CMP_LT: cmp_plain_body<V, VXG_CMP_LT>(in, n, out, out_bit, s, excl != 0); break;
    default: cmp_plain_body<V, VXG_CMP_LTE>(in, n, out, out_bit, s, excl != 0); break;
    }
}

__device__ __forceinline__ uint64_t patch_pos(const TakePatches& p, uint64_t i) {
    uint64_t v;
    switch (p.iw) {
    case 1: v = p.isg ? uint64_t(int64_t(gload(static_cast<const int8_t*>(p.idx) + i))) : gload(static_cast<const uint8_t*>(p.idx) + i); break;
    case 2: v = p.isg ? uint64_t(int64_t(gload(static_cast<const int16_t*>(p.idx) + i))) : gload(static_cast<const uint16_t*>(p.idx) + i); break;
    case 4: v = p.isg ? uint64_t(int64_t(gload(static_cast<const int32_t*>(p.idx) + i))) : gload(static_cast<const uint32_t*>(p.idx) + i); break;
    default: v = gload(static_cast<const uint64_t*>(p.idx) + i); break;
    }
    return v - p.off;
}

__device__ __forceinline__ void assign_bit(uint32_t* __restrict__ out, uint64_t bit, bool v) {
    const uint32_t m = 1u << (bit & 31);
    if (v) __hip_atomic_fetch_or(out + (bit >> 5), m, __ATOMIC_RELAXED, __HIP_MEMORY_SCOPE_AGENT);
    else __hip_atomic_fetch_and(out + (bit >> 5), ~m, __ATOMIC_RELAXED, __HIP_MEMORY_SCOPE_AGENT);
}

template <int T, Epi EPI, int CK>
__global__ __launch_bounds__(kCmpThreads) void cmp_patch_kernel(TakePatches p, uint64_t len, uint32_t* __restrict__ out,
                                                                uint64_t out_bit, EpiParams ep, uint64_t sbits, int op) {
    using E = typename Fl<T>::E;
    using V = CmpV<typename EpiOut<T, EPI, 0>::type, CK>;
    const V s = scalar_of<V>(sbits);
    for (uint64_t i = uint64_t(blockIdx.x) * blockDim.x + threadIdx.x; i < p.n; i += uint64_t(gridDim.x) * blockDim.x) {
        const uint64_t pos = patch_pos(p, i);
        if (pos >= len) {
            __hip_atomic_fetch_or(ep.err, kErrPatchOOB, __ATOMIC_RELAXED, __HIP_MEMORY_SCOPE_AGENT);
            continue;
        }
        const V v = V(apply_epi<T, EPI, 0>(gload(static_cast<const E*>(p.values) + i), ep));
        assign_bit(out, out_bit + pos, cmp_rt(op, v, s));
    }
}

template <class V>
__global__ __launch_bounds__(kCmpThreads) void cmp_patch_raw_kernel(TakePatches p, uint64_t len, uint32_t* __restrict__ out,
                                                                    uint64_t out_bit, uint64_t sbits, int op, uint32_t* err) {
    const V s = scalar_of<V>(sbits);
    for (uint64_t i = uint64_t(blockIdx.x) * blockDim.x + threadIdx.x; i < p.n; i += uint64_t(gridDim.x) * blockDim.x) {
        const uint64_t pos = patch_pos(p, i);
        if (pos >= len) {
            __hip_atomic_fetch_or(err, kErrPatchOOB, __ATOMIC_RELAXED, __HIP_MEMORY_SCOPE_AGENT);
            continue;
        }
        assign_bit(out, out_bit + pos, cmp_rt(op, gload(static_cast<const V*>(p.values) + i), s));
    }
}

__global__ __launch_bounds__(kCmpThreads) void and_words_kernel(uint64_t* __restrict__ bits, const uint64_t* __restrict__ mask,
                                                                uint64_t n) {
    for (uint64_t i = uint64_t(blockIdx.x) * blockDim.x + threadIdx.x; i < n; i += uint64_t(gridDim.x) * blockDim.x)
        bits[i] &= mask[i];
}

unsigned cmp_grid(uint64_t n_threads) {
    const uint64_t g = (n_threads + kCmpThreads - 1) / kCmpThreads;
    return unsigned(g > 32768 ? 32768 : (g ? g : 1));
}

template <int T, Epi EPI, int CK>
vxg_status packed_launch(const CmpTable& tab, uint64_t groups, uint32_t lds_bytes, void* out, uint64_t sbits, int op,
                         hipStream_t s) {
    hipLaunchKernelGGL((cmp_packed_kernel<T, EPI, CK>), dim3(unsigned(groups)), dim3(kCmpThreads), lds_bytes, s, tab,
                       static_cast<uint64_t*>(out), sbits, op);
    return hip_check(hipGetLastError(), "cmp_packed_kernel");
}

}

vxg_status launch_cmp_packed(int T, Epi epi, int ck, const CmpTable& tab, uint64_t groups, uint32_t lds_bytes, void* out,
                             uint64_t sbits, int op, hipStream_t s) {
    if (groups == 0 || groups > 0x7FFFFFFFull || lds_bytes > 64 * 1024)
        return set_error(VXG_ERR_INVALID_ARGUMENT, "compare: bad launch shape");
#define VXG_CMP(TT, EE, CC)                                                                          \
    if (T == TT && epi == EE && ck == CC) return packed_launch<TT, EE, CC>(tab, groups, lds_bytes, out, sbits, op, s);
// ... 75 lines not shown
```

vortex_amd/csrc/dict_rows.hip:

```cpp
#include "fl_unpack_impl.hpp"

namespace vxg {

namespace {

constexpr int kRowsThreads = 256;
constexpr int kRowsMaxW = 16;

template <int VW> struct DVal;
template <> struct DVal<16> { using t = uint4; };

template <int T, int VW, int BPW, bool LDSD, bool EXT>
__global__ __launch_bounds__(kRowsThreads) void dict_rows_kernel(ChunkTable tab, unsigned W) {
    using E = typename Fl<T>::E;
    using V = typename DVal<VW>::t;
    constexpr unsigned LANES = 1024 / T;
    const uint64_t g = blockIdx.x;
    uint32_t ci;
    if constexpr (EXT) {
        ci = ext_chunk_index(tab.ext, tab.n, g, [](const ChunkDev& d) { return d.first_group; });
    } else {
        uint32_t lo = 0, hi = tab.n;
        while (hi - lo > 1) {
            const uint32_t mid = (lo + hi) >> 1;
            if (tab.c[mid].first_group <= g) lo = mid; else hi = mid;
        }
        ci = lo;
    }
    const ChunkDev& c = EXT ? tab.ext[ci] : tab.c[ci];
    __shared__ __attribute__((aligned(16))) E s_packed[BPW * 128 * kRowsMaxW / sizeof(E)];
    __shared__ __attribute__((aligned(16))) uint8_t s_dict[LDSD ? kDictLdsBytes : 16];
    const unsigned tid = threadIdx.x;
    const uint64_t blk0 = (g - c.first_group) * BPW;
    const unsigned nb = unsigned(c.n_blocks - blk0 < uint64_t(BPW) ? c.n_blocks - blk0 : uint64_t(BPW));
    const unsigned q16 = nb * 8 * W;
    for (unsigned q = tid; q < q16; q += kRowsThreads)
        reinterpret_cast<uint4*>(s_packed)[q] = reinterpret_cast<const uint4*>(c.packed + blk0 * (128ull * W))[q];
    const V* dict = static_cast<const V*>(c.dict);
    if constexpr (LDSD) {
        const unsigned n16 = unsigned((c.dict_len * VW + 15) / 16);
        for (unsigned q = tid; q < n16; q += kRowsThreads)
            reinterpret_cast<uint4*>(s_dict)[q] = static_cast<const uint4*>(c.dict)[q];
        dict = reinterpret_cast<const V*>(s_dict);
    }
    __syncthreads();
    V* __restrict__ out = static_cast<V*>(c.out);
    const RtRows<T> rows(W);
    bool oob = false;
    for (unsigned b = 0; b < nb; b++) {
        const E* __restrict__ pw = s_packed + b * (LANES * W);
        const int64_t base = int64_t((blk0 + b) * 1024) - int64_t(c.offset);
        const bool whole = base >= 0 && uint64_t(base) + 1024 <= c.len;
#pragma unroll
        for (unsigned k = 0; k < 4; k++) {
            const int64_t o = base + int64_t(k * kRowsThreads + tid);
            if (!whole && (o < 0 || uint64_t(o) >= c.len)) continue;
            const uint64_t code = W ? uint64_t(rows.get(pw, k)) : 0;
            const bool bad = code >= c.dict_len;
            oob |= bad;
            nt_store(out + o, dict[bad ? 0 : code]);
        }
    }
    if (oob) __hip_atomic_fetch_or(tab.err, kErrTakeOOB, __ATOMIC_RELAXED, __HIP_MEMORY_SCOPE_AGENT);
}

template <int T, int VW, int BPW, bool LDSD, bool EXT>
vxg_status launch_rows(ChunkTable tab, unsigned W, hipStream_t s) {
    ChunkDev* cs = tab.ext ? tab.host : tab.c;
    uint64_t groups = 0;
    for (uint32_t k = 0; k < tab.n; k++) {
        cs[k].first_group = groups;
        groups += (cs[k].n_blocks + BPW - 1) / BPW;
    }
    if (groups == 0) return VXG_OK;
    if (groups > 0xFFFFFFFFull) return set_error(VXG_ERR_INVALID_ARGUMENT, "array too long for one launch");
    hipLaunchKernelGGL((dict_rows_kernel<T, VW, BPW, LDSD, EXT>), dim3(unsigned(groups)), dim3(kRowsThreads), 0, s,
                       tab, W);
    return hip_check(hipGetLastError(), "dict_rows_kernel launch");
}

template <int T, int VW, int BPW>
vxg_status launch_rows_b(const ChunkTable& tab, unsigned W, bool lds, hipStream_t s) {
    if (tab.ext) return lds ? launch_rows<T, VW, BPW, true, true>(tab, W, s) : launch_rows<T, VW, BPW, false, true>(tab, W, s);
    return lds ? launch_rows<T, VW, BPW, true, false>(tab, W, s) : launch_rows<T, VW, BPW, false, false>(tab, W, s);
}

template <int T, int VW>
vxg_status launch_rows_t(const ChunkTable& tab, unsigned W, hipStream_t s) {
    const ChunkDev* cs = tab.ext ? tab.host : tab.c;
    bool lds = true;
    uint64_t max_dict = 0;
    for (uint32_t k = 0; k < tab.n; k++) {
        lds = lds && cs[k].dict_len * VW <= uint64_t(kDictLdsBytes) && (reinterpret_cast<uintptr_t>(cs[k].dict) & 15) == 0;
        max_dict = cs[k].dict_len * VW > max_dict ? cs[k].dict_len * VW : max_dict;
    }
    if (lds && max_dict > 1024) return launch_rows_b<T, VW, 8>(tab, W, lds, s);
    return launch_rows_b<T, VW, 1>(tab, W, lds, s);
}

}

vxg_status launch_dict_rows(int T, int W, const ChunkTable& tab, hipStream_t s) {
    if (W < 0 || W > kRowsMaxW || W > T) return VXG_ERR_NOT_IMPLEMENTED;
    const unsigned w = unsigned(W);
    switch (T) {
    case 8: return launch_rows_t<8, 16>(tab, w, s);
    case 16: return launch_rows_t<16, 16>(tab, w, s);
    case 32: return launch_rows_t<32, 16>(tab, w, s);
    case 64: return launch_rows_t<64, 16>(tab, w, s);
    }
    return VXG_ERR_NOT_IMPLEMENTED;
}

}
```

vortex_amd/csrc/fl_unpack_impl.hpp:

```cpp
#pragma once

#include <hip/hip_runtime.h>

#include <cstdint>
#include <cstdlib>
#include <type_traits>
#include <utility>

#include "vxg_internal.hpp"
#include "intcol.hpp"

namespace vxg {

template <int T> struct Fl;
template <> struct Fl<8> {
    using E = uint8_t;  using U = uint32_t;
    static constexpr uint32_t rep(uint32_t m) { return m * 0x01010101u; }
};
template <> struct Fl<16> {
    using E = uint16_t; using U = uint32_t;
    static constexpr uint32_t rep(uint32_t m) { return m * 0x00010001u; }
};
template <> struct Fl<32> {
    using E = uint32_t; using U = uint32_t;
// ... 147 lines not shown
}

template <int T>
struct RtRows {
    using E = typename Fl<T>::E;
    static constexpr uint32_t LANES = 1024 / T;
    uint32_t lane, start0, W;
    E mask;
    __device__ __forceinline__ explicit RtRows(uint32_t w) : W(w) {
        const uint32_t t = threadIdx.x;
        lane = t % LANES;
        const uint32_t fl = ((t & 127) - lane) >> 4;
        const uint32_t row = (((fl & 1) << 2) | (fl & 2) | (fl >> 2)) * 8 + (t >> 7);
        start0 = __umul24(row, w);
        mask = w >= uint32_t(T) ? E(~E(0)) : E((E(1) << w) - E(1));
    }
    __device__ __forceinline__ E get(const E* __restrict__ pw, uint32_t k) const {
        if constexpr (T == 64) {
            const uint32_t start = start0 + 2 * k * W, w0 = start >> 6, sh = start & 63;
            const uint32_t w1 = w0 + 1 < W ? w0 + 1 : w0;
            const uint64_t lo = pw[LANES * w0 + lane], hi = pw[LANES * w1 + lane];
            return (sh ? (lo >> sh) | (hi << (64 - sh)) : lo) & mask;
        } else {
            constexpr uint32_t LT = T == 32 ? 5 : (T == 16 ? 4 : 3);
            const uint32_t start = start0 + 2 * k * W, w0 = start >> LT, sh = start & (T - 1);
            const uint32_t w1 = w0 + 1 < W ? w0 + 1 : w0;
            const uint32_t lo = pw[LANES * w0 + lane], hi = pw[LANES * w1 + lane];
            if constexpr (T == 32) return E(__builtin_amdgcn_alignbit(hi, lo, sh) & mask);
            else return E(((lo | (hi << T)) >> sh) & mask);
        }
    }
};

#ifndef VXG_OUT_NT
#define VXG_OUT_NT 1
#endif
constexpr int kOutNT = VXG_OUT_NT;

template <int NBYTES, int NT = 0>
__device__ __forceinline__ void store_bytes(uint8_t* dst, const void* src) {
    using u32x4 = unsigned int __attribute__((ext_vector_type(4)));
    if constexpr (NBYTES >= 16) {
#pragma unroll
        for (int i = 0; i < NBYTES / 16; i++) {
            u32x4 vv;
            __builtin_memcpy(&vv, static_cast<const uint8_t*>(src) + 16 * i, 16);
            if constexpr (NT) __builtin_nontemporal_store(vv, (gptr<u32x4>)dst + i);
            else ((gptr<u32x4>)dst)[i] = vv;
        }
    } else if constexpr (NBYTES == 8) {
        uint64_t q; __builtin_memcpy(&q, src, 8); *(gptr<uint64_t>)dst = q;
    } else if constexpr (NBYTES == 4) {
        uint32_t q; __builtin_memcpy(&q, src, 4); *(gptr<uint32_t>)dst = q;
    } else if constexpr (NBYTES == 2) {
        uint16_t q; __builtin_memcpy(&q, src, 2); *(gptr<uint16_t>)dst = q;
    } else {
        *(gptr<uint8_t>)dst = *static_cast<const uint8_t*>(src);
    }
}

template <int T, int W, Epi EPI, int VW, int NT, int R, bool FULL>
__device__ __forceinline__ void process_row(const Vec16<T>* p, int lane0,
                                            typename EpiOut<T, EPI, VW>::type* __restrict__ out,
                                            int64_t out_base, uint64_t len, const EpiParams& ep, bool& oob) {
    using E = typename Fl<T>::E;
    using O = typename EpiOut<T, EPI, VW>::type;
    constexpr int EPV = 16 / int(sizeof(E));
    const Vec16<T> v = extract_row<T, W, R>(p);
    const int idx = fl_index(R, lane0);
    if constexpr (FULL) {
        O* dst = out + (out_base + idx);
        if constexpr (EPI == Epi::Plain) {
            store_bytes<16, NT>(reinterpret_cast<uint8_t*>(dst), v.w);
        } else {
            O o[EPV];
#pragma unroll
            for (int j = 0; j < EPV; j++) o[j] = apply_epi<T, EPI, VW>(v.elem(j), ep, oob);
            store_bytes<EPV * int(sizeof(O)), NT>(reinterpret_cast<uint8_t*>(dst), o);
        }
    } else {
#pragma unroll
        for (int j = 0; j < EPV; j++) {
            const int64_t o = out_base + idx + j;
            if (o >= 0 && uint64_t(o) < len) gstore(out + o, apply_epi<T, EPI, VW>(v.elem(j), ep, oob));
        }
    }
}

template <int T, int W, Epi EPI, int VW, int NT, bool FULL, int... Rs>
__device__ __forceinline__ void process_rows(const Vec16<T>* p, int lane0,
                                             typename EpiOut<T, EPI, VW>::type* __restrict__ out,
                                             int64_t out_base, uint64_t len, const EpiParams& ep, bool& oob,
                                             std::integer_sequence<int, Rs...>) {
    (process_row<T, W, EPI, VW, NT, Rs, FULL>(p, lane0, out, out_base, len, ep, oob), ...);
}

template <int T, int W, Epi EPI, int VW, int NT = 0>
__device__ __forceinline__ void unpack_block(const uint8_t* __restrict__ blk_packed, int t,
                                             typename EpiOut<T, EPI, VW>::type* __restrict__ out,
                                             int64_t out_base, bool full, uint64_t len,
                                             const EpiParams& ep) {
    using E = typename Fl<T>::E;
    constexpr int EPV = 16 / int(sizeof(E));
    constexpr int NW = W > 0 ? W : 1;
    Vec16<T> p[NW];
    if constexpr (W > 0) {
#pragma unroll
        for (int w = 0; w < W; w++) p[w] = load16<T>(blk_packed + 128 * w + 16 * t);
    }
    bool oob = false;
    if (full)
        process_rows<T, W, EPI, VW, NT, true>(p, t * EPV, out, out_base, len, ep, oob,
                                              std::make_integer_sequence<int, T>{});
    else
        process_rows<T, W, EPI, VW, NT, false>(p, t * EPV, out, out_base, len, ep, oob,
                                               std::make_integer_sequence<int, T>{});
    if constexpr (EPI == Epi::Dict)
        if (oob) __hip_atomic_fetch_or(ep.err, kErrTakeOOB, __ATOMIC_RELAXED, __HIP_MEMORY_SCOPE_AGENT);
}

template <int T, int W, Epi EPI, int VW, int NT, int S, int Q, bool FULL, int... Rs>
__device__ __forceinline__ void process_rows_part(const Vec16<T>* p, int lane0,
                                                  typename EpiOut<T, EPI, VW>::type* __restrict__ out,
                                                  int64_t out_base, uint64_t len, const EpiParams& ep, bool& oob,
                                                  std::integer_sequence<int, Rs...>) {
    (process_row<T, W, EPI, VW, NT, Q * (T / S) + Rs, FULL>(p, lane0, out, out_base, len, ep, oob), ...);
}

template <int T, int W, Epi EPI, int VW, int NT, int S, int Q>
__device__ __forceinline__ void unpack_block_part(const uint8_t* __restrict__ blk_packed, int t,
                                                  typename EpiOut<T, EPI, VW>::type* __restrict__ out,
                                                  int64_t out_base, bool full, uint64_t len,
                                                  const EpiParams& ep) {
    using E = typename Fl<T>::E;
    constexpr int EPV = 16 / int(sizeof(E));
    constexpr int NW = W > 0 ? W : 1;
    constexpr int R0 = Q * (T / S), R1 = (Q + 1) * (T / S);
    constexpr int WLO = W > 0 ? (R0 * W) / T : 0;
    constexpr int WHI = W > 0 ? (R1 * W - 1) / T : 0;
    Vec16<T> p[NW];
    if constexpr (W > 0) {
#pragma unroll
        for (int w = WLO; w <= WHI && w < W; w++) p[w] = load16<T>(blk_packed + 128 * w + 16 * t);
    }
    bool oob = false;
    if (full)
        process_rows_part<T, W, EPI, VW, NT, S, Q, true>(p, t * EPV, out, out_base, len, ep, oob,
                                                         std::make_integer_sequence<int, T / S>{});
    else
        process_rows_part<T, W, EPI, VW, NT, S, Q, false>(p, t * EPV, out, out_base, len, ep, oob,
                                                          std::make_integer_sequence<int, T / S>{});
    if constexpr (EPI == Epi::Dict)
        if (oob) __hip_atomic_fetch_or(ep.err, kErrTakeOOB, __ATOMIC_RELAXED, __HIP_MEMORY_SCOPE_AGENT);
}

constexpr int kDictLdsBytes = 16 * 1024;

template <int VW>
__device__ __forceinline__ void stage_dict(uint8_t* s_dict, const void* dict, uint64_t dict_len) {
    const int n16 = int((dict_len * VW + 15) / 16);
    for (int q = threadIdx.x; q < n16; q += blockDim.x)
        reinterpret_cast<uint4*>(s_dict)[q] = static_cast<const uint4*>(dict)[q];
    __syncthreads();
}

template <int T, int W, Epi EPI, int VW, bool LDSD, int S>
__device__ __forceinline__ void unpack_chunk(const ChunkDev& c, uint64_t g, uint32_t* err) {
    using O = typename EpiOut<T, EPI, VW>::type;
    constexpr int BPG = 32 / S;
    const uint64_t blk = (g - c.first_group) * BPG + ((threadIdx.x >> 3) % BPG);
    const int t = int(threadIdx.x & 7);
    EpiParams ep;
    ep.reference = c.reference;
    ep.shift = c.shift;
    ep.alp_a = c.alp_a;
    ep.alp_b = c.alp_b;
    ep.dict = c.dict;
    ep.dict_len = c.dict_len;
    ep.err = err;
    if constexpr (LDSD) {
        __shared__ __attribute__((aligned(16))) uint8_t s_dict[kDictLdsBytes];
        stage_dict<VW>(s_dict, c.dict, c.dict_len);
        ep.dict = s_dict;
        ep.dict_lds = true;
    }
    if (blk >= c.n_blocks) return;
    const int64_t out_base = int64_t(blk * 1024) - int64_t(c.offset);
    const bool full =
        c.offset == 0 && (blk + 1) * 1024 <= c.len && (reinterpret_cast<uintptr_t>(c.out) & 15) == 0;
    const uint8_t* bp = c.packed + blk * (128 * W);
    if constexpr (S == 1) {
        unpack_block<T, W, EPI, VW, kOutNT>(bp, t, static_cast<O*>(c.out), out_base, full, c.len, ep);
    } else {
        static_assert(S == 4, "row split 1 or 4");
        switch (threadIdx.x >> 6) {
        case 0: unpack_block_part<T, W, EPI, VW, kOutNT, 4, 0>(bp, t, static_cast<O*>(c.out), out_base, full, c.len, ep); break;
        case 1: unpack_block_part<T, W, EPI, VW, kOutNT, 4, 1>(bp, t, static_cast<O*>(c.out), out_base, full, c.len, ep); break;
        case 2: unpack_block_part<T, W, EPI, VW, kOutNT, 4, 2>(bp, t, static_cast<O*>(c.out), out_base, full, c.len, ep); break;
        default: unpack_block_part<T, W, EPI, VW, kOutNT, 4, 3>(bp, t, static_cast<O*>(c.out), out_base, full, c.len, ep); break;
        }
    }
}

constexpr int kw_bpw(int W, bool lds_dict = false) {
    const int b = ((lds_dict ? 16 : 32) * 1024) / (128 * (W > 0 ? W : 1));
    const int b4 = (b / 4) * 4;
    return b4 < 4 ? 4 : (b4 > 32 ? 32 : b4);
}

template <int T>
__device__ __forceinline__ int kw_row(int q) {
    constexpr int P = T / 8;
    const int s = q / P, f = (q % P) * (64 / T);
    const int o = ((f & 1) << 2) | (f & 2) | (f >> 2);
    return o * 8 + s;
}

template <typename U>
__device__ __forceinline__ U kw_mask(int n) {
    return n >= int(8 * sizeof(U)) ? ~U(0) : ((U(1) << n) - U(1));
}

template <int T, int W>
__device__ __forceinline__ Vec16<T> kw_extract(const uint8_t* blk, int r, int t) {
    using U = typename Fl<T>::U;
    constexpr int NV = Vec16<T>::NV;
    Vec16<T> v;
    if constexpr (W == 0) {
#pragma unroll
        for (int k = 0; k < NV; k++) v.w[k] = 0;
    } else {
        const int start = r * W, w0 = start / T, sh = start % T;
        const Vec16<T> lo = load16<T>(blk + w0 * 128 + 16 * t);
        if constexpr (W == T) {
            v = lo;
        } else {
            const Vec16<T> hi = load16<T>(blk + (w0 + 1) * 128 + 16 * t);
            const int cur = T - sh;
            const int nlo = cur < W ? cur : W, nhi = W - nlo;
            const U mlo = Fl<T>::rep(kw_mask<U>(nlo)), mhi = Fl<T>::rep(kw_mask<U>(nhi));
            const int hs = cur & (int(8 * sizeof(U)) - 1);
#pragma unroll
            for (int k = 0; k < NV; k++) v.w[k] = ((lo.w[k] >> sh) & mlo) | ((hi.w[k] & mhi) << hs);
        }
    }
    return v;
}

template <int T, int W, Epi EPI, int VW, int NT>
__device__ __forceinline__ void kw_block(const uint8_t* pk, int gq, int t, typename EpiOut<T, EPI, VW>::type* __restrict__ out,
                                         int64_t out_base, bool full, uint64_t len, const EpiParams& ep, bool& oob) {
    using E = typename Fl<T>::E;
    using O = typename EpiOut<T, EPI, VW>::type;
    constexpr int EPV = 16 / int(sizeof(E));
#pragma unroll
    for (int k = 0; k < T / 8; k++) {
        const int q = 8 * k + gq;
        const Vec16<T> v = kw_extract<T, W>(pk, kw_row<T>(q), t);
        const int idx = q * (1024 / T) + t * EPV;
        if (full) {
            O* dst = out + (out_base + idx);
            if constexpr (EPI == Epi::Plain) {
                store_bytes<16, NT>(reinterpret_cast<uint8_t*>(dst), v.w);
            } else {
                O o[EPV];
#pragma unroll
                for (int j = 0; j < EPV; j++) o[j] = apply_epi<T, EPI, VW>(v.elem(j), ep, oob);
                store_bytes<EPV * int(sizeof(O)), NT>(reinterpret_cast<uint8_t*>(dst), o);
            }
        } else {
#pragma unroll
            for (int j = 0; j < EPV; j++) {
                const int64_t o = out_base + idx + j;
                if (o >= 0 && uint64_t(o) < len) gstore(out + o, apply_epi<T, EPI, VW>(v.elem(j), ep, oob));
            }
        }
    }
}

template <int W, bool LDSD>
constexpr int kw_packed_lds() {
    return (W > 0 ? kw_bpw(W, LDSD) * 128 * W : 0) + 128;
}

__device__ __forceinline__ uint64_t patch_lower_bound(const PatchCol& pc, uint64_t x, uint32_t* s_cnt) {
    uint64_t lo = 0, hi = pc.n;
    while (lo < hi) {
        const uint64_t step = (hi - lo + 255) / 256;
        const uint64_t i = lo + uint64_t(threadIdx.x) * step;
        const bool below = i < hi && uint64_t(intcol_get(pc.idx, i)) - pc.idx_off < x;
        const uint32_t cw = uint32_t(__popcll(__ballot(below)));
        if ((threadIdx.x & 63) == 0) s_cnt[threadIdx.x >> 6] = cw;
        __syncthreads();
        const uint64_t cnt = uint64_t(s_cnt[0]) + s_cnt[1] + s_cnt[2] + s_cnt[3];
        __syncthreads();
        if (cnt == 0) {
            hi = lo;
        } else {
            const uint64_t nhi = lo + cnt * step;
            lo = lo + (cnt - 1) * step + 1;
            hi = nhi < hi ? nhi : hi;
        }
    }
    return lo;
}

template <int T, int W, Epi EPI, int VW, bool LDSD>
__device__ __forceinline__ void unpack_chunk_w(const ChunkDev& c, uint64_t g, uint32_t* err, const PatchCol& pc,
                                               uint32_t bpw_rt) {
    using O = typename EpiOut<T, EPI, VW>::type;
    constexpr int BPW_MAX = kw_bpw(W, LDSD);
    const int BPW = bpw_rt ? int(bpw_rt) : BPW_MAX;
    extern __shared__ __attribute__((aligned(16))) uint8_t k1w_lds[];
    uint8_t* const s_pk = k1w_lds;
    EpiParams ep;
    ep.reference = c.reference;
    ep.shift = c.shift;
    ep.alp_a = c.alp_a;
    ep.alp_b = c.alp_b;
    ep.dict = c.dict;
    ep.dict_len = c.dict_len;
    ep.err = err;
    if constexpr (LDSD) {
        uint8_t* const s_dict = k1w_lds + kw_packed_lds<W, LDSD>();
        stage_dict<VW>(s_dict, c.dict, c.dict_len);
        ep.dict = s_dict;
        ep.dict_lds = true;
    }
    const uint64_t blk0 = (g - c.first_group) * BPW;
    const int nb = c.n_blocks - blk0 < uint64_t(BPW) ? int(c.n_blocks - blk0) : BPW;
    uint32_t* const s_pscr = reinterpret_cast<uint32_t*>(k1w_lds + (W > 0 ? BPW * 128 * W : 0));
    const bool patched = pc.n != 0;
    uint64_t olo = 0, ohi = 0, pbase = 0, pw0 = 0, pw1 = 0;
    uint32_t psh = 0;
    O pval{};
    if (patched) {
        const uint64_t s0 = blk0 * 1024, s1 = (blk0 + uint64_t(nb)) * 1024;
        olo = s0 > c.offset ? s0 - c.offset : 0;
        ohi = s1 - c.offset < c.len ? s1 - c.offset : c.len;
        const uint64_t guess = uint64_t(double(olo) * double(pc.n) / double(c.len));
        pbase = guess > 128 ? guess - 128 : 0;
        if (pbase + 256 > pc.n) pbase = pc.n > 256 ? pc.n - 256 : 0;
        const uint64_t i0 = pbase + threadIdx.x, i = i0 < pc.n ? i0 : pc.n - 1;
        const uint64_t* ip = static_cast<const uint64_t*>(pc.idx.p);
        uint64_t a0 = i, a1 = i;
        if (pc.idx.packed) {
            const uint64_t g2 = i + pc.idx.offset;
            const uint32_t e = uint32_t(g2 & 1023), lane = e % 16, s = e >> 7;
            const uint32_t fl = ((e & 127) - lane) >> 4;
            const uint32_t row = (((fl & 1) << 2) | (fl & 2) | (fl >> 2)) * 8 + s;
            const uint32_t start = __umul24(row, pc.idx.W), word = start / 64;
            psh = start % 64;
            const uint64_t blk = (g2 >> 10) * (16ull * pc.idx.W);
            a0 = blk + 16ull * word + lane;
            a1 = blk + 16ull * (word + 1 < pc.idx.W ? word + 1 : word) + lane;
        }
        pw0 = ip[a0];
        pw1 = ip[a1];
        pval = static_cast<const O*>(pc.vals)[i];
    }
    if constexpr (W > 0) {
        using u32x4 = unsigned int __attribute__((ext_vector_type(4)));
        const gptr<const u32x4> src = (gptr<const u32x4>)(c.packed + blk0 * (128 * W));
#if VXG_K1W_BURST
        constexpr int NQ = BPW_MAX * 8 * W, PQ = (NQ + 255) / 256;
        if (nb == BPW_MAX) {
            u32x4 v[PQ];
#pragma unroll
            for (int p = 0; p < PQ; p++) {
                const int q = int(threadIdx.x) + 256 * p;
                v[p] = __builtin_nontemporal_load(src + (q < NQ ? q : NQ - 1));
            }
#pragma unroll
            for (int p = 0; p < PQ; p++) {
                const int q = int(threadIdx.x) + 256 * p;
                if (q < NQ) reinterpret_cast<uint4*>(s_pk)[q] = make_uint4(v[p][0], v[p][1], v[p][2], v[p][3]);
            }
        } else
#endif
        for (int q = threadIdx.x; q < nb * 8 * W; q += 256) {
            const u32x4 v = __builtin_nontemporal_load(src + q);
            reinterpret_cast<uint4*>(s_pk)[q] = make_uint4(v[0], v[1], v[2], v[3]);
        }
    }
    __syncthreads();
    const int wave = threadIdx.x >> 6, lane = threadIdx.x & 63, gq = lane >> 3, t = lane & 7;
    O* const out = static_cast<O*>(c.out);
    const bool aligned = (reinterpret_cast<uintptr_t>(c.out) & 15) == 0;
    bool oob = false;
    const int PER = (BPW + 3) / 4;
    for (int j = 0; j < PER; j++) {
        const int b = wave * PER + j;
        if (b >= nb) break;
        const uint64_t blk = blk0 + b;
        const int64_t out_base = int64_t(blk * 1024) - int64_t(c.offset);
        const bool full = c.offset == 0 && (blk + 1) * 1024 <= c.len && aligned;
        kw_block<T, W, EPI, VW, kOutNT>(s_pk + b * 128 * W, gq, t, out, out_base, full, c.len, ep, oob);
    }
    if constexpr (EPI == Epi::Dict)
        if (oob) __hip_atomic_fetch_or(err, kErrTakeOOB, __ATOMIC_RELAXED, __HIP_MEMORY_SCOPE_AGENT);
    if (patched) {
        asm volatile("" : "+v"(pw0), "+v"(pw1));
        uint64_t pkey = pw0;
        if (pc.idx.packed) {
            const uint64_t mask = pc.idx.W >= 64 ? ~0ull : ((1ull << pc.idx.W) - 1);
            const uint64_t v = pc.idx.W ? ((psh ? (pw0 >> psh) | (pw1 << (64 - psh)) : pw0) & mask) : 0;
            pkey = (v << pc.idx.shift) + pc.idx.reference;
        }
        const bool valid = pbase + threadIdx.x < pc.n;
        pkey = valid ? pkey - pc.idx_off : ~0ull;
        const bool pin = pkey >= olo && pkey < ohi;
        if (threadIdx.x == 0) s_pscr[0] = pbase == 0 || pkey < olo;
        if (threadIdx.x == 255) s_pscr[1] = pbase + 256 >= pc.n || pkey >= ohi;
        const uint64_t nk = __shfl_down(pkey, 1, 64);
        if ((threadIdx.x & 63) != 63 && pbase + threadIdx.x + 1 < pc.n && nk < pkey)
            __hip_atomic_fetch_or(err, kErrPatchOrder, __ATOMIC_RELAXED, __HIP_MEMORY_SCOPE_AGENT);
        if (g == c.first_group && threadIdx.x == 0) {
            const uint64_t k0 = uint64_t(intcol_get(pc.idx, 0)) - pc.idx_off;
            const uint64_t k1 = uint64_t(intcol_get(pc.idx, pc.n - 1)) - pc.idx_off;
            if (k0 >= c.len || k1 >= c.len)
                __hip_atomic_fetch_or(err, kErrPatchOOB, __ATOMIC_RELAXED, __HIP_MEMORY_SCOPE_AGENT);
        }
        __builtin_amdgcn_s_waitcnt(0);
        __syncthreads();
        if (s_pscr[0] && s_pscr[1]) {
            if (pin) gstore(out + pkey, pval);
        } else {
            const uint64_t ps = patch_lower_bound(pc, olo, s_pscr + 4);
            const uint64_t pe = patch_lower_bound(pc, ohi, s_pscr + 4);
            bool bad = false;
            for (uint64_t i = ps + threadIdx.x; i < pe; i += 256) {
                const uint64_t key = uint64_t(intcol_get(pc.idx, i)) - pc.idx_off;
                if (key >= olo && key < ohi) gstore(out + key, gload(static_cast<const O*>(pc.vals) + i));
                else bad = true;
            }
            if (bad) __hip_atomic_fetch_or(err, kErrPatchOrder, __ATOMIC_RELAXED, __HIP_MEMORY_SCOPE_AGENT);
        }
    }
}

template <int T, int W, Epi EPI, int VW, bool LDSD, bool EXT>
__global__ __launch_bounds__(256) void fl_unpack_w_kernel(ChunkTable tab) {
    const uint64_t g = blockIdx.x;
    if constexpr (EXT) {
        const ChunkDev& c =
            tab.ext[ext_chunk_index(tab.ext, tab.n, g, [](const ChunkDev& d) { return d.first_group; })];
        unpack_chunk_w<T, W, EPI, VW, LDSD>(c, g, tab.err, PatchCol{}, tab.bpw);
    } else {
        uint32_t lo = 0, hi = tab.n;
        while (hi - lo > 1) {
            const uint32_t mid = (lo + hi) >> 1;
            if (tab.c[mid].first_group <= g) lo = mid; else hi = mid;
        }
        unpack_chunk_w<T, W, EPI, VW, LDSD>(tab.c[lo], g, tab.err, tab.patch, tab.bpw);
    }
}

template <int T, int W, Epi EPI, int VW, bool LDSD = false, int S = 1, bool EXT = false>
__global__ __launch_bounds__(256) void fl_unpack_kernel(ChunkTable tab) {
    const uint64_t g = blockIdx.x;
    if constexpr (EXT) {
        const ChunkDev& c =
            tab.ext[ext_chunk_index(tab.ext, tab.n, g, [](const ChunkDev& d) { return d.first_group; })];
        unpack_chunk<T, W, EPI, VW, LDSD, S>(c, g, tab.err);
    } else {
        uint32_t lo = 0, hi = tab.n;
        while (hi - lo > 1) {
            const uint32_t mid = (lo + hi) >> 1;
            if (tab.c[mid].first_group <= g) lo = mid; else hi = mid;
        }
        unpack_chunk<T, W, EPI, VW, LDSD, S>(tab.c[lo], g, tab.err);
    }
}


inline int k1w_pick_bpw(uint64_t blocks, int bpw_max, int64_t min_groups, int64_t forced) {
    if (forced > 0) return int(forced < bpw_max ? forced : bpw_max);
    if (min_groups <= 0 || blocks >= uint64_t(min_groups) * uint64_t(bpw_max)) return bpw_max;
    const uint64_t b = blocks / uint64_t(min_groups);
    const int bpw = int(b < 4 ? 4 : (b / 4) * 4);
    return bpw > bpw_max ? bpw_max : bpw;
}

template <int T, int W, Epi EPI, int VW, bool LDSD, bool EXT>
vxg_status launch_w(ChunkTable tab, hipStream_t s) {
    constexpr int BPW_MAX = kw_bpw(W, LDSD);
    ChunkDev* cs = tab.ext ? tab.host : tab.c;
    uint64_t blocks = 0;
    for (uint32_t k = 0; k < tab.n; k++) blocks += cs[k].n_blocks;
    const Options o = cur_options();
    const int BPW = k1w_pick_bpw(blocks, BPW_MAX, o.k1w_min_groups, o.k1w_bpw);
    tab.bpw = uint32_t(BPW);
    uint64_t groups = 0, dict_bytes = 0;
    for (uint32_t k = 0; k < tab.n; k++) {
        cs[k].first_group = groups;
        groups += (cs[k].n_blocks + BPW - 1) / BPW;
        const uint64_t db = (cs[k].dict_len * uint64_t(VW > 0 ? VW : 1) + 15) & ~15ull;
        dict_bytes = db > dict_bytes ? db : dict_bytes;
    }
    if (groups == 0) return VXG_OK;
    if (groups > 0xFFFFFFFFull) return set_error(VXG_ERR_INVALID_ARGUMENT, "array too long for one launch");
    const size_t shm = LDSD ? size_t(kw_packed_lds<W, LDSD>()) + size_t(dict_bytes)
                            : size_t(W > 0 ? BPW * 128 * W : 0) + 128;
    hipLaunchKernelGGL((fl_unpack_w_kernel<T, W, EPI, VW, LDSD, EXT>), dim3(unsigned(groups)), dim3(256), shm, s, tab);
    note_k1w_launch(uint32_t(BPW), uint32_t(BPW_MAX), groups);
    if constexpr (!EXT) {
        if (tab.patch.n) g_k1w_wrote_patches = true;
    }
    return hip_check(hipGetLastError(), "fl_unpack_w_kernel launch");
}


template <int T, int W, Epi EPI, int VW, bool LDSD, int S, bool EXT = false>
vxg_status launch_s(ChunkTable tab, hipStream_t s) {
    ChunkDev* cs = tab.ext ? tab.host : tab.c;
    uint64_t groups = 0;
    for (uint32_t k = 0; k < tab.n; k++) {
        cs[k].first_group = groups;
        groups += (cs[k].n_blocks + (32 / S) - 1) / (32 / S);
    }
    if (groups == 0) return VXG_OK;
    if (groups > 0xFFFFFFFFull) return set_error(VXG_ERR_INVALID_ARGUMENT, "array too long for one launch");
    hipLaunchKernelGGL((fl_unpack_kernel<T, W, EPI, VW, LDSD, S, EXT>), dim3(unsigned(groups)), dim3(256), 0, s, tab);
    return hip_check(hipGetLastError(), "fl_unpack_kernel launch");
}

template <int T, int W, Epi EPI, int VW>
vxg_status launch_one(const ChunkTable& tab, uint64_t groups32, hipStream_t s) {
    if (groups32 == 0) return VXG_OK;
    constexpr bool kSplit = (T == 32 || T == 64) && W > 0;
    const bool split = kSplit && groups32 < split_below_groups();
    bool lds = false;
    if constexpr (EPI == Epi::Dict) {
        const ChunkDev* cs = tab.ext ? tab.host : tab.c;
        lds = true;
        for (uint32_t k = 0; k < tab.n; k++)
            lds = lds && cs[k].dict_len * VW <= uint64_t(kDictLdsBytes) &&
                  (reinterpret_cast<uintptr_t>(cs[k].dict) & 15) == 0;
    }
    constexpr uint64_t kExtWaveGroups = 128;
    const int mode = k1_wave_mode();
    const bool big = !split || (tab.ext && groups32 >= kExtWaveGroups);
    const bool wave = mode == 2 || (mode == 1 && big && EPI != Epi::Dict);
    if (tab.ext) {
        if (wave) {
            if constexpr (EPI == Epi::Dict) {
                if (lds) return launch_w<T, W, EPI, VW, true, true>(tab, s);
            }
            return launch_w<T, W, EPI, VW, false, true>(tab, s);
        }
        constexpr int SX = kSplit ? 4 : 1;
        if constexpr (EPI == Epi::Dict) {
            if (lds) return launch_s<T, W, EPI, VW, true, SX, true>(tab, s);
        }
        return launch_s<T, W, EPI, VW, false, SX, true>(tab, s);
    }
    if constexpr (kSplit) {
        if (split && !wave) return lds ? launch_s<T, W, EPI, VW, true, 4>(tab, s) : launch_s<T, W, EPI, VW, false, 4>(tab, s);
    }
    if (wave) {
        if constexpr (EPI == Epi::Dict) {
            if (lds) return launch_w<T, W, EPI, VW, true, false>(tab, s);
        }
        return launch_w<T, W, EPI, VW, false, false>(tab, s);
    }
    if constexpr (EPI == Epi::Dict) {
        if (lds) return launch_s<T, W, EPI, VW, true, 1>(tab, s);
    }
    return launch_s<T, W, EPI, VW, false, 1>(tab, s);
}

template <int T, Epi EPI, int VW, int... Ws>
vxg_status dispatch_w_impl(int W, const ChunkTable& tab, uint64_t groups, hipStream_t s,
                           std::integer_sequence<int, Ws...>) {
    using Fn = vxg_status (*)(const ChunkTable&, uint64_t, hipStream_t);
    static constexpr Fn table[] = {&launch_one<T, Ws, EPI, VW>...};
    if (W < 0 || W >= int(sizeof...(Ws))) return VXG_ERR_NOT_IMPLEMENTED;
    return table[W](tab, groups, s);
}

template <int T, Epi EPI, int VW, int WMAX>
vxg_status dispatch_w(int W, const ChunkTable& tab, uint64_t groups, hipStream_t s) {
    return dispatch_w_impl<T, EPI, VW>(W, tab, groups, s, std::make_integer_sequence<int, WMAX + 1>{});
}

}
```

vortex_amd/csrc/planner.hpp:

```cpp
#pragma once

#include <hip/hip_runtime.h>

#include <cstdint>
#include <string>
#include <utility>
#include <vector>

#include "compare.hpp"
#include "compare_str.hpp"
#include "env.hpp"
#include "take.hpp"
#include "vxg_internal.hpp"

struct vxg_ctx {
    vxg::Ctx c;
};

#define VXG_TRY(expr)                         \
    do {                                      \
        vxg_status _s = (expr);               \
        if (_s != VXG_OK) return _s;          \
    } while (0)

namespace vxg {

inline hipStream_t S(void* s) { return static_cast<hipStream_t>(s); }

vxg_status use_device(vxg_ctx* ctx);
vxg_status status_of_err_word(uint32_t err);

inline bool is_string(const vxg_array& a) { return a.dtype == VXG_DTYPE_UTF8 || a.dtype == VXG_DTYPE_BINARY; }

struct K1Job {
    int T, W;
    Epi epi;
    int vw;
    ChunkDev d;
    bool vb = false;
    VarBinChunk vbc{};
};

struct PlanBatch {
    struct Run {
        int w;
        RunEndChunk c;
        bool indep;
    };
    std::vector<VarBinChunk> dicts;
    std::vector<K1Job> jobs;
    std::vector<Run> runs;
    std::vector<FsstChunk> fssts;
    bool empty() const { return dicts.empty() && jobs.empty() && runs.empty() && fssts.empty(); }
};

vxg_status make_k1_job(int T, unsigned W, unsigned offset, uint64_t len, const void* packed, uint64_t packed_bytes,
                       Epi epi, int vw, const UnpackArgs& a, void* out, K1Job& j);
vxg_status launch_k1_jobs(std::vector<K1Job>& jobs, uint32_t* err, hipStream_t s, DevTables* dt = nullptr,
                          bool generic_small = false,
                          const std::vector<std::pair<int, RunEndChunk>>* gen_runs = nullptr,
                          const PatchCol* patch = nullptr, const FsstFused* fuse = nullptr);
vxg_status launch_runs(std::vector<RunEndChunk> runs, int w, uint32_t* err, hipStream_t s, DevTables* dt);
vxg_status launch_varbin_dicts(const std::vector<VarBinChunk>& dicts, uint32_t* err, hipStream_t s, DevTables* dt);
vxg_status flush_plan_batch(PlanBatch& b, uint32_t* err, hipStream_t s, DevTables* dt);

class Planner {
  public:
    Planner(vxg_ctx* ctx, hipStream_t s, DevTables* plan = nullptr, PlanBatch* batch = nullptr)
        : ctx_(ctx), s_(s), plan_(plan), batch_(batch) {}
    ~Planner() {
        for (void* p : temps_) (void)hipFreeAsync(p, s_);
    }

    vxg_status canonical(const vxg_array& a, vxg_canonical& out);
    vxg_status take(const vxg_array& a, const void* idx, int iw, bool isg, uint64_t n, vxg_canonical& out);
    vxg_status filter(const vxg_array& a, const vxg_array& pred, vxg_canonical& out);
    vxg_status compare(const vxg_array& a, int op, uint64_t scalar_bits, uint32_t flags, vxg_canonical& out,
                       vxg_compare_info& info);
    vxg_status compare_bytes(const vxg_array& a, int op, const void* scalar_host, uint64_t scalar_len, uint32_t flags,
                             vxg_canonical& out, vxg_compare_bytes_info& info);
    vxg_status canonical_size(const vxg_array& a, uint64_t& vb, uint64_t& db);
    vxg_status string_layout(const vxg_array& a, std::vector<vxg_data_buffer>& bufs, uint64_t& extent);
    static vxg_status string_buffer_count(const vxg_array& a, uint32_t& n);

  private:
    vxg_ctx* ctx_;
    hipStream_t s_;
    std::vector<void*> temps_;
    DevTables* plan_ = nullptr;
    PlanBatch* batch_ = nullptr;
    const vxg_array* root_ = nullptr;
    bool defer(const vxg_array& a) const { return batch_ && &a == root_; }
    struct PatchJob {
        const vxg_array* sp;
        int T;
        Epi epi;
        int vw;
        UnpackArgs a;
        void* dst;
        uint64_t out_len;
    };
    std::vector<K1Job>* k1_batch_ = nullptr;
    std::vector<PatchJob>* patch_batch_ = nullptr;
    const PatchCol* fused_patch_ = nullptr;
    std::vector<FsstChunk>* fsst_batch_ = nullptr;
    bool k1_fusable(const vxg_array& c) const;

    vxg_status temp(uint64_t bytes, void** p) {
        if (bytes == 0) bytes = 16;
        if (plan_) {
            VXG_TRY(hip_check(hipMalloc(p, (bytes + 15) & ~15ull), "hipMalloc (plan temporary)"));
            plan_->allocs.push_back(*p);
            return VXG_OK;
        }
        VXG_TRY(hip_check(hipMallocAsync(p, (bytes + 15) & ~15ull, s_), "hipMallocAsync"));
        temps_.push_back(*p);
        return VXG_OK;
    }

    static bool is_primitive_dtype(const vxg_array& a) { return a.dtype == VXG_DTYPE_PRIMITIVE; }
    static int width(const vxg_array& a) { return ptype_width(a.ptype); }

    const vxg_buffer* buf(const vxg_array& a, uint32_t i) const {
        return i < a.n_buffers ? &a.buffers[i] : nullptr;
    }
    const vxg_array* child(const vxg_array& a, uint32_t i) const {
        return i < a.n_children ? &a.children[i] : nullptr;
    }

    vxg_status decode_into(const vxg_array& a, void* dst);
    vxg_status view_primitive(const vxg_array& a, const void** p);
    vxg_status int_column(const vxg_array& a, IntCol& c);
    vxg_status packed_column(const vxg_array& a, IntCol& c, bool* packed);
    vxg_status runend_column(const vxg_array& a, bool in_place, IntCol& c);

    vxg_status decode_bitpacked(const vxg_array& bp, Epi epi, int vw, UnpackArgs a, void* dst);
    bool patch_fusable(const vxg_array& sparse, int value_width) const;
    vxg_status sparse_patch_col(const vxg_array& sparse, PatchCol& pc);
    vxg_status apply_sparse_patches(const vxg_array& sparse, int T, Epi epi, int vw, const UnpackArgs& a,
                                    void* dst, uint64_t out_len);
    vxg_status decode_alp(const vxg_array& a, void* dst);
    vxg_status decode_dict_primitive(const vxg_array& a, void* dst);
    vxg_status decode_chunked_primitive(const vxg_array& a, void* dst);
    vxg_status decode_alprd(const vxg_array& a, void* dst);
    vxg_status decode_sparse_values(const vxg_array& a, void* dst);

    vxg_status take_values(const vxg_array& a, const void* idx, int iw, bool isg, uint64_t n, void* dst);
    vxg_status take_patches(const vxg_array& sp, TakePatches& p);
    struct CmpFused {
        const vxg_array* arr;
        const vxg_array* bp;
        const vxg_array* outer;
        int T, ck;
        Epi epi;
        EpiParams ep;
        CmpChunk d;
        bool excl;
    };
    vxg_status compare_shape(const vxg_array& a, uint64_t out_bit, CmpFused& f, bool* fused);
    vxg_status launch_compare_group(std::vector<CmpFused*>& group, void* out, uint64_t scalar_bits, int op);
    struct StrRows {
        std::vector<VbDictPiece> vbd;
        std::vector<VbPiece> vb;
        std::vector<ViewPiece> vw;
        std::vector<FsstPiece> fs;
    };
    vxg_status compare_rows_of(const vxg_array& s, uint64_t out_bit, bool excl, bool table, StrRows& rows, bool* fell_back);
    vxg_status launch_str_rows(StrRows& rows, const StrScalar& sc, void* out, int op, uint32_t& launches);
    vxg_status validity_into(const vxg_array& a, void** bitmap);
    vxg_status bools_into(const vxg_array& a, void* bits, uint64_t off);
    vxg_status validity_source(const vxg_array& a, const vxg_array** node, int* kind);
    vxg_status string_canonical(const vxg_array& a, vxg_canonical& out);
    vxg_status string_lens(const vxg_array& a, std::vector<uint64_t>& lens,
                           std::vector<std::pair<size_t, const vxg_array*>>& fsst) const;
    vxg_status strings_into(const vxg_array& a, uint8_t* views, uint8_t* data, const vxg_data_buffer* bufs,
                            uint32_t bidx, const uint8_t* validity);
};

}
```

vortex_amd/csrc/planner_decode.hip:

```cpp
#include <algorithm>
#include <cstring>

#include "planner.hpp"

namespace vxg {

static bool fused_patches_enabled() { return env_flag("VXG_FUSED_PATCHES", true); }

vxg_status Planner::view_primitive(const vxg_array& a, const void** p) {
    if (a.encoding == VXG_ENC_PRIMITIVE) {
        const vxg_buffer* b = buf(a, 0);
        if (!b && a.len) return set_error(VXG_ERR_INVALID_ARGUMENT, "Primitive array without buffer");
        if (b && b->len < a.len * width(a))
            return set_error(VXG_ERR_INVALID_ARGUMENT, "Primitive buffer shorter than len * width");
        *p = b ? b->ptr : nullptr;
        return VXG_OK;
    }
    void* t;
    VXG_TRY(temp(a.len * width(a), &t));
    VXG_TRY(decode_into(a, t));
    *p = t;
    return VXG_OK;
}

vxg_status Planner::int_column(const vxg_array& a, IntCol& c) {
    if (!ptype_is_int(a.ptype)) return set_error(VXG_ERR_MISMATCHED_TYPES, "expected an integer array");
    bool packed = false;
    VXG_TRY(packed_column(a, c, &packed));
    return packed ? VXG_OK : view_primitive(a, &c.p);
}

vxg_status Planner::runend_column(const vxg_array& a, bool in_place, IntCol& c) {
    bool packed = false;
    if (in_place && ptype_is_int(a.ptype)) VXG_TRY(packed_column(a, c, &packed));
    if (packed) return VXG_OK;
    c = IntCol{};
    c.width = width(a);
    c.sgn = ptype_is_signed(a.ptype);
    return view_primitive(a, &c.p);
}

vxg_status Planner::packed_column(const vxg_array& a, IntCol& c, bool* packed) {
    *packed = false;
    c = IntCol{};
    c.width = width(a);
    c.sgn = ptype_is_signed(a.ptype);
    const vxg_array* bp = nullptr;
    if (a.encoding == VXG_ENC_FL_FOR && child(a, 0) && child(a, 0)->encoding == VXG_ENC_FL_BITPACKED) {
        bp = child(a, 0);
        c.reference = a.meta.for_.reference;
        c.shift = a.meta.for_.shift;
    } else if (a.encoding == VXG_ENC_FL_BITPACKED) {
        bp = &a;
    }
    if (bp && !bp->meta.bitpacked.has_patches && width(*bp) == c.width && (c.width == 4 || c.width == 8) &&
        bp->len == a.len) {
        const vxg_buffer* pk = buf(*bp, 0);
        const unsigned W = bp->meta.bitpacked.bit_width, off = bp->meta.bitpacked.offset;
        const uint64_t nblk = (bp->len + off + 1023) / 1024;
        if (off > 1023) return set_error(VXG_ERR_INVALID_ARGUMENT, "Offset must be less than full block, i.e. 1024");
        if (W > unsigned(8 * c.width)) return set_error(VXG_ERR_INVALID_ARGUMENT, "Unsupported bit width");
        const uint64_t have = pk ? pk->len : 0;
        if (W > 0 && have != nblk * 128ull * W)
            return set_error(VXG_ERR_INVALID_ARGUMENT, "Expected " + std::to_string(nblk * 128ull * W) +
                                                           " packed bytes, got " + std::to_string(have));
        c.packed = true;
        c.p = pk ? pk->ptr : nullptr;
        c.W = W;
        c.offset = off;
        *packed = true;
    }
    return VXG_OK;
}

vxg_status Planner::apply_sparse_patches(const vxg_array& sp, int T, Epi epi, int vw, const UnpackArgs& a,
                                         void* dst, uint64_t out_len) {
    if (sp.encoding != VXG_ENC_SPARSE)
        return set_error(VXG_ERR_INVALID_ARGUMENT, "Can't patch with a non-Sparse array");
    const vxg_array* idx = child(sp, 0);
    const vxg_array* val = child(sp, 1);
    if (!idx || !val) return set_error(VXG_ERR_INVALID_ARGUMENT, "Sparse patches need indices and values");
    if (idx->len != val->len) return set_error(VXG_ERR_INVALID_ARGUMENT, "Sparse indices/values length mismatch");
    PatchCol pc;
    VXG_TRY(int_column(*idx, pc.idx));
    VXG_TRY(view_primitive(*val, &pc.vals));
    return launch_patch(vw, pc.idx, epi, T, dst, out_len, sp.meta.sparse.indices_offset, pc.vals, idx->len, a, s_);
}

bool Planner::patch_fusable(const vxg_array& sp, int value_width) const {
    const vxg_array* idx = child(sp, 0);
    const vxg_array* val = child(sp, 1);
    return sp.encoding == VXG_ENC_SPARSE && idx && val && idx->len == val->len && idx->len > 0 &&
           width(*val) == value_width && width(*idx) == 8 && ptype_is_int(idx->ptype);
}

vxg_status Planner::sparse_patch_col(const vxg_array& sp, PatchCol& pc) {
    const vxg_array* idx = child(sp, 0);
    VXG_TRY(int_column(*idx, pc.idx));
    VXG_TRY(view_primitive(*child(sp, 1), &pc.vals));
    pc.n = idx->len;
    pc.idx_off = sp.meta.sparse.indices_offset;
    return VXG_OK;
}

vxg_status Planner::decode_bitpacked(const vxg_array& bp, Epi epi, int vw, UnpackArgs a, void* dst) {
    const int T = 8 * width(bp);
    if (!ptype_is_int(bp.ptype)) return set_error(VXG_ERR_MISMATCHED_TYPES, "BitPacked needs an integer ptype");
    const vxg_buffer* packed = buf(bp, 0);
    const unsigned W = bp.meta.bitpacked.bit_width;
    a.err = ctx_->c.err_word;
    K1Job j;
    VXG_TRY(make_k1_job(T, W, bp.meta.bitpacked.offset, bp.len, packed ? packed->ptr : nullptr,
                        packed ? packed->len : 0, epi, vw, a, dst, j));
    const vxg_array* p = nullptr;
    if (bp.meta.bitpacked.has_patches) {
        p = child(bp, 0);
        if (!p) return set_error(VXG_ERR_INVALID_ARGUMENT, "BitPackedArray: patches child missing");
    }
    if (k1_batch_) {
        k1_batch_->push_back(j);
        if (p) patch_batch_->push_back(PatchJob{p, T, epi, vw, a, dst, bp.len});
        return VXG_OK;
    }
    std::vector<K1Job> one{j};
    VXG_TRY(launch_k1_jobs(one, ctx_->c.err_word, s_, plan_, false, nullptr, fused_patch_));
    if (p) VXG_TRY(apply_sparse_patches(*p, T, epi, vw, a, dst, bp.len));
    return VXG_OK;
}

vxg_status Planner::decode_alp(const vxg_array& a, void* dst) {
    const vxg_array* enc = child(a, 0);
    if (!enc) return set_error(VXG_ERR_INVALID_ARGUMENT, "ALPArray: encoded child missing");
    const bool f32 = a.ptype == VXG_F32;
    if (!f32 && a.ptype != VXG_F64) return set_error(VXG_ERR_MISMATCHED_TYPES, "ALP can only encode f32 and f64");
    const unsigned e = a.meta.alp.e, f = a.meta.alp.f;
    if ((f32 && (e > 10 || f > 10)) || (!f32 && (e > 23 || f > 23)))
        return set_error(VXG_ERR_INVALID_ARGUMENT, "ALP exponents out of range");
    UnpackArgs ua{};
    ua.alp_a = f32 ? double(kF10f[f]) : kF10d[f];
    ua.alp_b = f32 ? double(kIF10f[e]) : kIF10d[e];
    const Epi epi = f32 ? Epi::AlpF32 : Epi::AlpF64;
    const vxg_array* bp = nullptr;
    if (enc->encoding == VXG_ENC_FL_FOR && child(*enc, 0) &&
        child(*enc, 0)->encoding == VXG_ENC_FL_BITPACKED) {
        ua.reference = enc->meta.for_.reference;
        ua.shift = enc->meta.for_.shift;
        bp = child(*enc, 0);
    } else if (enc->encoding == VXG_ENC_FL_BITPACKED) {
        bp = enc;
    }
    bool fused = false;
    if (bp && width(*bp) == (f32 ? 4 : 8)) {
        PatchCol pc{};
        const vxg_array* p = a.meta.alp.has_patches ? child(a, 1) : nullptr;
        if (p && !k1_batch_ && !patch_batch_ && !bp->meta.bitpacked.has_patches && bp->len == a.len &&
            patch_fusable(*p, f32 ? 4 : 8) && fused_patches_enabled()) {
            const uint64_t nblk = (bp->len + bp->meta.bitpacked.offset + 1023) / 1024;
            if (k1_takes_wave(f32 ? 32 : 64, int(bp->meta.bitpacked.bit_width), epi, (nblk + 31) / 32)) {
                VXG_TRY(sparse_patch_col(*p, pc));
                fused = !pc.idx.packed || pc.idx.W > 0;
            }
        }
        fused_patch_ = fused ? &pc : nullptr;
        g_k1w_wrote_patches = false;
        const vxg_status st = decode_bitpacked(*bp, epi, 0, ua, dst);
        fused_patch_ = nullptr;
        VXG_TRY(st);
        fused = fused && g_k1w_wrote_patches;
    } else {
        const void* penc;
        VXG_TRY(view_primitive(*enc, &penc));
        VXG_TRY(launch_alp(a.ptype, penc, a.len, ua.alp_a, ua.alp_b, dst, s_));
    }
    if (a.meta.alp.has_patches && !fused) {
        const vxg_array* p = child(a, 1);
        if (!p) return set_error(VXG_ERR_INVALID_ARGUMENT, "ALPArray: patches child missing");
        UnpackArgs plain{};
        plain.err = ctx_->c.err_word;
        if (patch_batch_) {
            patch_batch_->push_back(PatchJob{p, f32 ? 32 : 64, Epi::Plain, 0, plain, dst, a.len});
            return VXG_OK;
        }
        VXG_TRY(apply_sparse_patches(*p, f32 ? 32 : 64, Epi::Plain, 0, plain, dst, a.len));
    }
    return VXG_OK;
}

vxg_status Planner::decode_dict_primitive(const vxg_array& a, void* dst) {
    const vxg_array* values = child(a, 0);
    const vxg_array* codes = child(a, 1);
    if (!values || !codes) return set_error(VXG_ERR_INVALID_ARGUMENT, "DictArray needs values and codes");
    if (!ptype_is_unsigned(codes->ptype) || codes->nullable)
        return set_error(VXG_ERR_MISMATCHED_TYPES, "Dict codes must be non-nullable unsigned int");
    const void* pv;
    VXG_TRY(view_primitive(*values, &pv));
    const int vw = width(*values);
    if (codes->encoding == VXG_ENC_FL_BITPACKED && codes->meta.bitpacked.bit_width <= kDictFusedMaxW) {
        UnpackArgs ua{};
        ua.dict = pv;
        ua.dict_len = values->len;
        return decode_bitpacked(*codes, Epi::Dict, vw, ua, dst);
    }
    const void* pc;
    VXG_TRY(view_primitive(*codes, &pc));
    return launch_take(vw, pv, values->len, width(*codes), false, pc, a.len, dst, ctx_->c.err_word, s_);
}

bool Planner::k1_fusable(const vxg_array& c) const {
    auto bp_of_width = [&](const vxg_array* x, int w) {
        return x && x->encoding == VXG_ENC_FL_BITPACKED && width(*x) == w && ptype_is_int(x->ptype);
    };
    const int w = width(c);
    switch (c.encoding) {
    case VXG_ENC_FL_BITPACKED: return ptype_is_int(c.ptype);
    case VXG_ENC_FL_FOR: return ptype_is_int(c.ptype) && bp_of_width(child(c, 0), w);
    case VXG_ENC_ZIGZAG: return ptype_is_signed(c.ptype) && bp_of_width(child(c, 0), w);
    case VXG_ENC_ALP: {
        if (c.ptype != VXG_F32 && c.ptype != VXG_F64) return false;
        const vxg_array* e = child(c, 0);
        if (e && e->encoding == VXG_ENC_FL_FOR) e = child(*e, 0);
        return bp_of_width(e, w);
    }
    case VXG_ENC_DICT: {
        const vxg_array* v = child(c, 0);
        const vxg_array* k = child(c, 1);
        return v && k && v->encoding == VXG_ENC_PRIMITIVE && k->encoding == VXG_ENC_FL_BITPACKED &&
               ptype_is_unsigned(k->ptype) && !k->nullable && k->meta.bitpacked.bit_width <= kDictFusedMaxW;
    }
    default: return false;
    }
}

vxg_status Planner::decode_chunked_primitive(const vxg_array& a, void* dst) {
    const uint64_t n = a.meta.chunked.nchunks;
    if (a.n_children != n + 1) return set_error(VXG_ERR_INVALID_ARGUMENT, "Chunked child count != nchunks + 1");
    const int w = width(a);
    std::vector<K1Job> jobs;
    std::vector<PatchJob> patches;
    std::vector<RunEndChunk> runs;
    std::vector<uint8_t> runs_indep;
    auto child_ok = [&](const vxg_array* x) {
        return x && ptype_is_int(x->ptype) && (x->encoding == VXG_ENC_PRIMITIVE || k1_fusable(*x));
    };
    auto batch_runend = [&](const vxg_array& c) {
        const vxg_array* e = child(c, 0);
        const vxg_array* v = child(c, 1);
        return c.encoding == VXG_ENC_RUN_END && child_ok(e) && v && width(*v) == w && e->len == v->len &&
               (v->encoding == VXG_ENC_PRIMITIVE || k1_fusable(*v)) && e->len > 0;
    };
    std::vector<IntCol> inplace(2 * n);
    std::vector<uint8_t> is_inplace(2 * n, 0);
    uint64_t tmp_bytes = 0;
    for (uint64_t i = 0; i < n; i++) {
        const vxg_array& c = a.children[i + 1];
        if (!batch_runend(c)) continue;
        const vxg_array* e = child(c, 0);
        const vxg_array* v = child(c, 1);
        const bool short_runs = c.len <= kRunEndShortRun * e->len;
        const vxg_array* xs[2] = {e, v};
        for (int k = 0; k < 2; k++) {
            bool pk = false;
            if (short_runs && ptype_is_int(xs[k]->ptype)) VXG_TRY(packed_column(*xs[k], inplace[2 * i + k], &pk));
            is_inplace[2 * i + k] = pk;
            if (!pk && xs[k]->encoding != VXG_ENC_PRIMITIVE) tmp_bytes += (xs[k]->len * width(*xs[k]) + 15) & ~15ull;
        }
    }
    uint8_t* tmp = nullptr;
    if (tmp_bytes) {
        void* t;
        VXG_TRY(temp(tmp_bytes, &t));
        tmp = static_cast<uint8_t*>(t);
    }
    auto level0 = [&](const vxg_array& x, const void** p) -> vxg_status {
        if (x.encoding == VXG_ENC_PRIMITIVE) return view_primitive(x, p);
        *p = tmp;
        tmp += (x.len * width(x) + 15) & ~15ull;
        k1_batch_ = &jobs;
        patch_batch_ = &patches;
        const vxg_status st = decode_into(x, const_cast<void*>(*p));
        k1_batch_ = nullptr;
        patch_batch_ = nullptr;
        return st;
    };
    uint64_t off = 0;
    for (uint64_t i = 0; i < n; i++) {
        const vxg_array& c = a.children[i + 1];
        if (c.ptype != a.ptype || c.dtype != a.dtype)
            return set_error(VXG_ERR_MISMATCHED_TYPES, "Chunks must have the ChunkedArray's dtype");
        uint8_t* slice = static_cast<uint8_t*>(dst) + off * w;
        if (k1_fusable(c)) {
            k1_batch_ = &jobs;
            patch_batch_ = &patches;
            const vxg_status st = decode_into(c, slice);
// ... 404 lines not shown
```

vortex_amd/csrc/planner_launch.hip:

```cpp
#include <algorithm>
#include <tuple>

#include "chunk_pack.hpp"
#include "k1g.hpp"
#include "planner.hpp"

static_assert(sizeof(vxg::ChunkTable) <= 4096, "ChunkTable exceeds the kernarg limit");
static_assert(sizeof(vxg::FsstTable) <= 4096, "FsstTable exceeds the kernarg limit");
static_assert(sizeof(vxg::RunEndTable) <= 4096, "RunEndTable exceeds the kernarg limit");
static_assert(sizeof(vxg::VarBinTable) <= 4096, "VarBinTable exceeds the kernarg limit");
static_assert(sizeof(vxg::CmpTable) + 32 <= 4096, "CmpTable and the compare arguments exceed the kernarg limit");

namespace vxg {

thread_local bool g_k1w_wrote_patches = false;

void note_k1w_launch(uint32_t bpw, uint32_t bpw_max, uint64_t groups) {
    if (!g_cur_ctx) return;
    std::lock_guard<std::mutex> lk(g_cur_ctx->mu);
    LaunchStats& st = g_cur_ctx->st;
    st.k1w_min_bpw = st.k1w_launches == 0 ? bpw : std::min(st.k1w_min_bpw, bpw);
    st.k1w_max_bpw = st.k1w_launches == 0 ? bpw : std::max(st.k1w_max_bpw, bpw);
    st.k1w_launches++;
    st.k1w_last_bpw = bpw;
    st.k1w_last_bpw_max = bpw_max;
    st.k1w_last_groups = groups;
}

bool k1_takes_wave(int T, int W, Epi epi, uint64_t groups32) {
    const int mode = k1_wave_mode();
    const bool split = (T == 32 || T == 64) && W > 0 && groups32 < split_below_groups();
    return groups32 > 0 && (mode == 2 || (mode == 1 && !split && epi != Epi::Dict));
}

vxg_status launch_fl_unpack(int T, int W, Epi epi, int vw, const ChunkTable& t, uint64_t g, hipStream_t s) {
    if (W < 0 || W > T) return set_error(VXG_ERR_INVALID_ARGUMENT, "bit width out of range");
    switch (epi) {
    case Epi::Plain:
    case Epi::For:
    case Epi::ForZigZag:
        switch (T) {
        case 8: return fl_plain_8(W, epi, t, g, s);
        case 16: return fl_plain_16(W, epi, t, g, s);
        case 32: return fl_plain_32(W, epi, t, g, s);
        case 64: return fl_plain_64(W, epi, t, g, s);
        }
        return set_error(VXG_ERR_INVALID_ARGUMENT, "bad FastLanes width");
    case Epi::AlpF32:
    case Epi::AlpF64:
        return fl_alp(T, W, epi, t, g, s);
    case Epi::Dict:
        if (W > kDictFusedMaxW) return VXG_ERR_NOT_IMPLEMENTED;
        switch (vw) {
        case 1: return fl_dict_1(T, W, t, g, s);
        case 2: return fl_dict_2(T, W, t, g, s);
        case 4: return fl_dict_4(T, W, t, g, s);
        case 8: return fl_dict_8(T, W, t, g, s);
        case 16: return launch_dict_rows(T, W, t, s);
        }
        return set_error(VXG_ERR_INVALID_ARGUMENT, "bad dictionary value width");
    }
    return VXG_ERR_INVALID_ARGUMENT;
}

static bool same_kernel(const K1Job& a, const K1Job& b) {
    return a.T == b.T && a.W == b.W && a.epi == b.epi && a.vw == b.vw && a.vb == b.vb;
}

static uint64_t k1g_max_bytes() {
    static const uint64_t v = env_u64("VXG_K1G_MAX_BYTES", uint64_t(20) << 20);
    return v;
}

static int k1_out_width(int T, Epi epi, int vw) {
    return epi == Epi::Dict ? vw : (epi == Epi::AlpF32 ? 4 : (epi == Epi::AlpF64 ? 8 : T / 8));
}

vxg_status launch_k1_jobs(std::vector<K1Job>& jobs, uint32_t* err, hipStream_t s, DevTables* dt, bool generic_small,
                          const std::vector<std::pair<int, RunEndChunk>>* gen_runs, const PatchCol* patch,
                          const FsstFused* fuse) {
    std::stable_sort(jobs.begin(), jobs.end(), [](const K1Job& a, const K1Job& b) {
        return std::make_tuple(a.T, a.W, int(a.epi), a.vw, a.vb) < std::make_tuple(b.T, b.W, int(b.epi), b.vw, b.vb);
    });
    std::vector<const K1Job*> gen;
    auto launch_group = [&](size_t i, size_t j) -> vxg_status {
        const K1Job* it = jobs.data() + i;
        const K1Job* const end = jobs.data() + j;
        while (it != end) {
            ChunkTable tab{};
            tab.err = err;
            if (patch && jobs.size() == 1) tab.patch = *patch;
            uint64_t groups;
            VXG_TRY(pack_chunk_table(
                tab, it, end, dt, [](const K1Job& jb) { return jb.d.n_blocks ? &jb.d : nullptr; },
                [](const ChunkDev& c) { return (c.n_blocks + 31) / 32; }, &groups));
            if (tab.n) VXG_TRY(launch_fl_unpack(jobs[i].T, jobs[i].W, jobs[i].epi, jobs[i].vw, tab, groups, s));
        }
        return VXG_OK;
    };
    size_t i = 0;
    while (i < jobs.size()) {
        size_t j = i;
        uint64_t out_bytes = 0;
        while (j < jobs.size() && (dt || j - i < size_t(kArgChunks)) && same_kernel(jobs[i], jobs[j])) {
            out_bytes += jobs[j].d.len * uint64_t(k1_out_width(jobs[j].T, jobs[j].epi, jobs[j].vw));
            j++;
        }
        if (jobs[i].vb || (dt && generic_small && out_bytes < k1g_max_bytes() &&
                           gen_kind(jobs[i].T, int(jobs[i].epi), jobs[i].vw) >= 0)) {
            if (!dt) return set_error(VXG_ERR_INVALID_ARGUMENT, "VarBin-dictionary K1 jobs need a plan");
            for (size_t k = i; k < j; k++)
                if (jobs[k].d.n_blocks) gen.push_back(&jobs[k]);
            i = j;
            continue;
        }
        VXG_TRY(launch_group(i, j));
        i = j;
    }
    const size_t n_runs = gen_runs ? gen_runs->size() : 0;
    if (!gen.empty() || n_runs || (fuse && fuse->valid)) {
        if (!dt) return set_error(VXG_ERR_INVALID_ARGUMENT, "internal: K1g launch outside a plan");
        if (gen.size() + n_runs > 0xFFFFFFFFull) return set_error(VXG_ERR_INVALID_ARGUMENT, "too many chunks");
        GenChunk* host;
        const GenChunk* ext;
        VXG_TRY(dt->table(gen.size() + n_runs, &host, &ext));
        uint64_t groups = 0;
        bool dict_lds = true;
        uint32_t packed_bytes = 0, dict_bytes = 0, runs_bytes = 0;
        const bool vb_alone = n_runs == 0 && !(fuse && fuse->valid) &&
                              std::all_of(gen.begin(), gen.end(), [](const K1Job* jp) { return jp->vb; });
        uint64_t gen_blocks = 0;
        for (const K1Job* jp : gen) gen_blocks += jp->d.n_blocks;
        const uint32_t bpw_cap = gen_bpw_cap(gen_blocks);
        for (size_t k = 0; k < gen.size(); k++) {
            const K1Job& jb = *gen[k];
            GenChunk& g = host[k];
            g.d = jb.d;
            g.kind = uint32_t(gen_kind(jb.T, int(jb.epi), jb.vw, jb.vb));
            g.W = uint32_t(jb.W);
            g.bpw = jb.vb ? gen_vb_bpw(jb.T, jb.W, vb_alone, bpw_cap) : gen_bpw(jb.T, jb.W, bpw_cap);
            g.d.first_group = groups;
            groups += (jb.d.n_blocks + g.bpw - 1) / g.bpw;
            packed_bytes = std::max(packed_bytes, g.bpw * 128u * uint32_t(jb.W));
            if (jb.vb) {
                dict_bytes = std::max(dict_bytes, gen_vb_stage_bytes(jb.d.dict_len, jb.vbc.bytes));
                g.vb_src = jb.vbc.src;
                g.vb_offs = jb.vbc.offsets;
                g.vb_offs_width = jb.vbc.offs_width;
                g.vb_dst = jb.vbc.dst;
                g.vb_bytes = jb.vbc.bytes;
                g.vb_bidx = jb.vbc.bidx;
            } else if (jb.epi == Epi::Dict) {
                dict_lds = dict_lds && jb.d.dict_len * uint64_t(jb.vw) <= uint64_t(kDictLdsBytes) &&
                           (reinterpret_cast<uintptr_t>(jb.d.dict) & 15) == 0;
            }
        }
        if (dict_lds)
            for (const K1Job* jp : gen)
                if (jp->epi == Epi::Dict && !jp->vb)
                    dict_bytes = std::max(dict_bytes, uint32_t((jp->d.dict_len * uint64_t(jp->vw) + 15) & ~15ull));
        for (size_t k = 0; k < n_runs; k++) {
            const auto& [w, r] = (*gen_runs)[k];
            GenChunk& g = host[gen.size() + k];
            g.kind = uint32_t(gen_runs_kind(w));
            g.re = r;
            g.d.first_group = groups;
            g.d.n_blocks = r.n_runs;
            groups += (r.n_runs + kRunEndRunsPerGroup - 1) / kRunEndRunsPerGroup;
            runs_bytes = std::max(runs_bytes, gen_runs_lds_bytes(w));
        }
        std::vector<uint64_t> cnt(gen.size() + n_runs);
        for (size_t k = 0; k < cnt.size(); k++)
            cnt[k] = (k + 1 < cnt.size() ? host[k + 1].d.first_group : groups) - host[k].d.first_group;
        uint64_t gpe = common_groups(cnt.data(), cnt.size());
        if (!gpe && cnt.size() > 1) {
            const uint64_t m = *std::max_element(cnt.begin(), cnt.end());
            if (m * cnt.size() - groups <= groups / 10) {
                for (size_t k = 0; k < cnt.size(); k++) host[k].d.first_group = k * m;
                groups = m * cnt.size();
                gpe = m;
            }
        }
        VXG_TRY(launch_k1_generic(ext, uint32_t(gen.size() + n_runs), groups, dict_lds, packed_bytes, dict_bytes,
                                    runs_bytes, err, s, gpe, fuse));
    }
    return VXG_OK;
}

vxg_status make_k1_job(int T, unsigned W, unsigned offset, uint64_t len, const void* packed, uint64_t packed_bytes,
                       Epi epi, int vw, const UnpackArgs& a, void* out, K1Job& j) {
    if (offset > 1023) return set_error(VXG_ERR_INVALID_ARGUMENT, "Offset must be less than full block, i.e. 1024");
    if (W > unsigned(T)) return set_error(VXG_ERR_INVALID_ARGUMENT, "Unsupported bit width");
    const uint64_t nblk = (len + offset + 1023) / 1024;
    if (W > 0 && packed_bytes != nblk * 128ull * W)
        return set_error(VXG_ERR_INVALID_ARGUMENT, "Expected " + std::to_string(nblk * 128ull * W) +
                                                       " packed bytes, got " + std::to_string(packed_bytes));
    if (W > 0 && (reinterpret_cast<uintptr_t>(packed) & 15))
        return set_error(VXG_ERR_INVALID_ARGUMENT, "packed buffer must be 16-byte aligned");
    if (reinterpret_cast<uintptr_t>(out) % uint64_t(k1_out_width(T, epi, vw)))
        return set_error(VXG_ERR_INVALID_ARGUMENT, "output buffer must be aligned to the value width");
    if (epi == Epi::Dict && W > unsigned(kDictFusedMaxW)) return VXG_ERR_NOT_IMPLEMENTED;
    if (epi == Epi::Dict && a.dict_len == 0 && len > 0)
        return set_error(VXG_ERR_OUT_OF_BOUNDS, "take: index out of bounds");
    j.T = T;
    j.W = int(W);
    j.epi = epi;
    j.vw = epi == Epi::Dict ? vw : 0;
    j.d = ChunkDev{};
    j.d.packed = static_cast<const uint8_t*>(packed);
    j.d.out = out;
    j.d.n_blocks = len ? nblk : 0;
    j.d.len = len;
    j.d.reference = a.reference;
    j.d.alp_a = a.alp_a;
    j.d.alp_b = a.alp_b;
    j.d.dict = a.dict;
    j.d.dict_len = a.dict_len;
    j.d.offset = offset;
    j.d.shift = a.shift;
    return VXG_OK;
}

vxg_status launch_runs(std::vector<RunEndChunk> runs, int w, uint32_t* err, hipStream_t s, DevTables* dt) {
    runs.erase(std::remove_if(runs.begin(), runs.end(), [](const RunEndChunk& r) { return r.len == 0; }), runs.end());
    std::vector<RunEndChunk> short_runs, long_runs;
    for (const RunEndChunk& r : runs) (r.len <= kRunEndShortRun * r.n_runs ? short_runs : long_runs).push_back(r);
    for (int pass = 0; pass < 2; pass++) {
        const std::vector<RunEndChunk>& rs = pass == 0 ? short_runs : long_runs;
        for (const RunEndChunk* it = rs.data(), * const end = rs.data() + rs.size(); it != end;) {
            RunEndTable tab{};
            tab.err = err;
            uint64_t groups;
            VXG_TRY(pack_chunk_table(
                tab, it, end, dt, [](const RunEndChunk& r) { return &r; },
                [pass](const RunEndChunk& r) {
                    return pass == 0 ? (r.n_runs + kRunEndRunsPerGroup - 1) / kRunEndRunsPerGroup
                                     : (r.len + kRunEndSpan - 1) / kRunEndSpan;
                },
                &groups));
            VXG_TRY(pass == 0 ? launch_runend_runs(w, tab, groups, s) : launch_runend_chunks(w, tab, groups, s));
        }
    }
    return VXG_OK;
}

static bool plan_fuse_enabled() { return env_flag("VXG_PLAN_FUSE", true); }

vxg_status launch_varbin_dicts(const std::vector<VarBinChunk>& dicts, uint32_t* err, hipStream_t s, DevTables* dt) {
    for (const VarBinChunk* it = dicts.data(), * const end = dicts.data() + dicts.size(); it != end;) {
        VarBinTable tab{};
        tab.err = err;
        uint64_t groups;
        VXG_TRY(pack_chunk_table(
            tab, it, end, dt, [](const VarBinChunk& d) { return &d; },
            [](const VarBinChunk& d) { return d.n ? (d.n + 255) / 256 : uint64_t(1); }, &groups));
        VXG_TRY(launch_varbin_chunks(tab, groups, s));
    }
    return VXG_OK;
}

vxg_status flush_plan_batch(PlanBatch& b, uint32_t* err, hipStream_t s, DevTables* dt) {
    FsstFused ff;
    if (!b.fssts.empty()) {
        void* scratch = nullptr;
        VXG_TRY(hip_check(hipMalloc(&scratch, (fsst_batch_scratch_bytes(b.fssts.data(), b.fssts.size()) + 15) & ~15ull),
                            "hipMalloc (plan FSST scratch)"));
        dt->allocs.push_back(scratch);
        VXG_TRY(launch_fsst_batch(b.fssts, scratch, err, s, dt, plan_fuse_enabled() ? &ff : nullptr));
    }
    VXG_TRY(launch_varbin_dicts(b.dicts, err, s, dt));
    std::vector<std::pair<int, RunEndChunk>> gen_runs;
    std::vector<PlanBatch::Run> rest;
    for (const PlanBatch::Run& r : b.runs) {
        if (r.c.len == 0) continue;
        if (r.indep && r.c.len <= kRunEndShortRun * r.c.n_runs && gen_runs_kind(r.w) >= 0) gen_runs.emplace_back(r.w, r.c);
        else rest.push_back(r);
    }
    VXG_TRY(launch_k1_jobs(b.jobs, err, s, dt, true, &gen_runs, nullptr, &ff));
    std::vector<int> widths;
    for (const auto& r : rest) widths.push_back(r.w);
    std::sort(widths.begin(), widths.end());
    widths.erase(std::unique(widths.begin(), widths.end()), widths.end());
    for (int w : widths) {
        std::vector<RunEndChunk> rs;
        for (const auto& r : rest)
            if (r.w == w) rs.push_back(r.c);
        VXG_TRY(launch_runs(rs, w, err, s, dt));
    }
    return VXG_OK;
}

}
```

vortex_amd/csrc/vxg_internal.hpp:

```cpp
#pragma once

#include <hip/hip_runtime.h>

#include <cstdint>
#include <mutex>
#include <string>
#include <type_traits>
#include <vector>

#include "../../include/vortex_gpu.h"
#include "env.hpp"

namespace vxg {

__host__ __device__ constexpr int fl_order(int i) {
    constexpr int o[8] = {0, 4, 2, 6, 1, 5, 3, 7};
    return o[i];
}
__host__ __device__ constexpr int fl_index(int row, int lane) {
    return fl_order(row / 8) * 16 + (row % 8) * 128 + lane;
}

template <class T>
using gptr = __attribute__((address_space(1))) T*;
// ... 25 lines not shown
    if constexpr (sizeof(T) == 16 && !std::is_scalar_v<T>) {
        using u32x4 = unsigned int __attribute__((ext_vector_type(4)));
        const u32x4 x = *(__attribute__((address_space(3))) const u32x4*)p;
        T r;
        __builtin_memcpy(&r, &x, 16);
        return r;
    } else {
        return *(__attribute__((address_space(3))) const T*)p;
    }
}

template <typename V>
__device__ __forceinline__ void nt_store(V* p, const V& v) {
    if constexpr (sizeof(V) == 16) {
        using u32x4 = unsigned int __attribute__((ext_vector_type(4)));
        u32x4 vv;
        __builtin_memcpy(&vv, &v, 16);
        __builtin_nontemporal_store(vv, (gptr<u32x4>)p);
    } else {
        __builtin_nontemporal_store(v, (gptr<V>)p);
    }
}

inline int ptype_width(int p) {
    switch (p) {
    case VXG_U8: case VXG_I8: return 1;
    case VXG_U16: case VXG_I16: case VXG_F16: return 2;
    case VXG_U32: case VXG_I32: case VXG_F32: return 4;
    case VXG_U64: case VXG_I64: case VXG_F64: return 8;
    default: return 0;
    }
}
inline bool ptype_is_int(int p) { return p >= VXG_U8 && p <= VXG_I64; }
inline bool ptype_is_signed(int p) { return p >= VXG_I8 && p <= VXG_I64; }
inline bool ptype_is_unsigned(int p) { return p >= VXG_U8 && p <= VXG_U64; }

extern const float kF10f[11];
extern const float kIF10f[11];
extern const double kF10d[24];
extern const double kIF10d[24];

enum : uint32_t { kErrTakeOOB = 1u, kErrPatchOOB = 2u, kErrRunEnd = 4u, kErrFsst = 8u, kErrRoaring = 16u, kErrVarBin = 32u,
                  kErrPatchOrder = 64u, kErrPlanSync = 128u };

struct Options {
    int64_t k1w_min_groups = 1024;
    int64_t k1w_bpw = 0;
    int64_t k1_wave = -1;
};
struct LaunchStats {
    uint64_t k1w_launches = 0, k1w_last_groups = 0;
    uint32_t k1w_last_bpw = 0, k1w_min_bpw = 0, k1w_max_bpw = 0, k1w_last_bpw_max = 0;
};

struct Ctx {
    int device = 0;
    uint32_t* err_word = nullptr;
    Options opt;
    std::mutex mu;
    LaunchStats st;
};
extern thread_local Ctx* g_cur_ctx;
Options default_options();
inline Options cur_options() { return g_cur_ctx ? g_cur_ctx->opt : default_options(); }
inline int k1_wave_mode() {
    const int64_t o = cur_options().k1_wave;
    if (o >= 0) return int(o > 2 ? 2 : o);
    const char* e = env_str("VXG_K1_WAVE");
    if (!e) return 1;
    return e[0] == '0' ? 0 : (e[0] == 'f' ? 2 : 1);
}
void note_k1w_launch(uint32_t bpw, uint32_t bpw_max, uint64_t groups);

vxg_status set_error(vxg_status s, const std::string& msg);
vxg_status hip_check(hipError_t e, const char* what);

struct DevTables {
    std::vector<void*> allocs;
    std::vector<std::pair<void*, std::vector<uint8_t>>> uploads;
    template <class E>
    vxg_status table(size_t n, E** host, const E** dev) {
        void* d = nullptr;
        const hipError_t e = hipMalloc(&d, n * sizeof(E) + 16);
        if (e != hipSuccess) return hip_check(e, "hipMalloc (plan chunk table)");
        allocs.push_back(d);
        uploads.emplace_back(d, std::vector<uint8_t>(n * sizeof(E), 0));
        *host = reinterpret_cast<E*>(uploads.back().second.data());
        *dev = static_cast<const E*>(d);
        return VXG_OK;
    }
    vxg_status upload() {
        for (auto& u : uploads) {
            const hipError_t e = hipMemcpy(u.first, u.second.data(), u.second.size(), hipMemcpyHostToDevice);
            if (e != hipSuccess) return hip_check(e, "plan chunk table upload");
        }
        uploads.clear();
        return VXG_OK;
    }
};

template <class E, class Key>
__device__ __forceinline__ uint32_t ext_chunk_index(const E* __restrict__ ext, uint32_t n, uint64_t g, Key key) {
    const uint32_t lane = threadIdx.x & 63u;
    uint32_t cnt = 0;
    for (uint32_t base = 0; base < n; base += 256) {
        uint64_t kv[4];
#pragma unroll
        for (int k = 0; k < 4; k++) {
            const uint32_t i = base + 64u * uint32_t(k) + lane;
            kv[k] = uint64_t(key(ext[i < n ? i : n - 1]));
        }
#pragma unroll
        for (int k = 0; k < 4; k++) {
            const bool le = base + 64u * uint32_t(k) + lane < n && kv[k] <= g;
            cnt += uint32_t(__popcll(__ballot(le)));
        }
    }
    return cnt ? cnt - 1 : 0;
}

template <class E, class Key>
__device__ __forceinline__ uint32_t ext_chunk_index_gpe(const E* __restrict__ ext, uint32_t n, uint64_t g, uint64_t gpe,
                                                        Key key) {
    if (gpe) {
        const uint32_t q = uint32_t(g) / uint32_t(gpe);
        const uint32_t ci = __builtin_amdgcn_readfirstlane(q < n - 1 ? q : n - 1);
        const uint64_t f0 = uint64_t(key(ext[ci]));
        const uint64_t f1 = ci + 1 < n ? uint64_t(key(ext[ci + 1])) : ~0ull;
        if (f0 <= g && g < f1) return ci;
    }
    return ext_chunk_index(ext, n, g, key);
}
inline uint64_t common_groups(const uint64_t* counts, size_t n) {
    if (n == 0 || counts[0] == 0) return 0;
    for (size_t i = 1; i + 1 < n; i++)
        if (counts[i] != counts[0]) return 0;
    return counts[n - 1] <= counts[0] ? counts[0] : 0;
}

enum class Epi : int { Plain = 0, For = 1, ForZigZag = 2, AlpF32 = 3, AlpF64 = 4, Dict = 5 };

struct UnpackArgs {
    const uint8_t* packed;
    void* out;
    uint64_t n_blocks;
    uint32_t offset;
    uint64_t len;
    uint64_t reference;
    uint32_t shift;
    double alp_a, alp_b;
    const void* dict;
    uint64_t dict_len;
    uint32_t* err;
};

struct ChunkDev {
    const uint8_t* packed;
    void* out;
    uint64_t n_blocks;
    uint64_t len;
    uint64_t first_group;
    uint64_t reference;
    double alp_a, alp_b;
    const void* dict;
    uint64_t dict_len;
    uint32_t offset;
    uint32_t shift;
};
constexpr int kArgChunks = 32;
struct ChunkTable;

vxg_status launch_fl_unpack(int T, int W, Epi epi, int value_width, const ChunkTable& tab, uint64_t groups,
                            hipStream_t s);

struct IntCol {
    const void* p;
    int width;
    bool sgn;
    bool packed;
    uint32_t W;
    uint32_t shift;
    uint32_t offset;
    uint64_t reference;
};
struct PatchCol {
    IntCol idx;
    const void* vals;
    uint64_t n;
    uint64_t idx_off;
};

struct ChunkTable {
    ChunkDev c[kArgChunks];
    uint32_t n;
    uint32_t* err;
    const ChunkDev* ext;
    ChunkDev* host;
    PatchCol patch;
    uint32_t bpw;
};

extern thread_local bool g_k1w_wrote_patches;

inline uint64_t split_below_groups() {
    static const uint64_t v = env_u64("VXG_SPLIT_BELOW", 1024);
    return v;
}
bool k1_takes_wave(int T, int W, Epi epi, uint64_t groups32);

vxg_status launch_patch(int val_width, const IntCol& indices, Epi epi, int T, void* out, uint64_t out_len,
                        uint64_t indices_offset, const void* values, uint64_t n, const UnpackArgs& ep,
                        hipStream_t s);

vxg_status launch_for(int width, const void* in, uint64_t n, uint64_t ref, unsigned shift,
                      bool zigzag, void* out, hipStream_t s);
vxg_status launch_zigzag(int width, const void* in, uint64_t n, void* out, hipStream_t s);
vxg_status launch_alp(int float_ptype, const void* enc, uint64_t n, double a, double b, void* out,
                      hipStream_t s);
vxg_status launch_take(int value_width, const void* values, uint64_t n_values, int code_width, bool code_signed,
                       const void* codes, uint64_t n, void* out, uint32_t* err, hipStream_t s);
vxg_status launch_alprd(int float_ptype, const uint16_t* left, const uint16_t* dict, unsigned dict_len,
                        unsigned right_bw, const void* right, uint64_t n, const void* exc_pos,
                        int pos_width, bool pos_signed, uint64_t pos_off, const uint16_t* exc,
                        uint64_t n_exc, void* out, uint32_t* err, hipStream_t s);
vxg_status launch_copy_bits(void* dst, uint64_t dst_off, const uint8_t* src, uint64_t src_off, uint64_t n,
                            bool set_all, hipStream_t s);
vxg_status launch_roaring_bool(const uint8_t* buf, uint64_t n, uint64_t len, void* bits, uint64_t off, uint32_t* err,
                               hipStream_t s);
vxg_status launch_runend_bool(const void* ends, int ew, uint64_t n_runs, uint64_t offset, bool start, uint64_t len,
                              void* dst, uint64_t dst_off, uint32_t* err, hipStream_t s);
vxg_status launch_bytebool(const uint8_t* src, uint64_t n, void* dst, uint64_t dst_off, hipStream_t s);
vxg_status launch_assign_bits_at(void* dst, uint64_t dst_off, const void* idx, int iw, bool isg, uint64_t ioff,
                                 uint64_t n, uint64_t len, const uint8_t* vals, hipStream_t s);
vxg_status launch_gather_bits(void* dst, const void* codes, int cw, bool csg, uint64_t n, const uint8_t* src,
                              uint64_t n_values, uint32_t* err, hipStream_t s);
vxg_status launch_set_bits_at(void* dst, const void* idx, int iw, bool isg, uint64_t off, uint64_t n,
                              uint64_t len, hipStream_t s);
vxg_status launch_sum(const void* p, int w, bool sg, uint64_t n, void* out_u64, hipStream_t s);
vxg_status fl_plain_8(int W, Epi epi, const ChunkTable& t, uint64_t g, hipStream_t s);
vxg_status fl_plain_16(int W, Epi epi, const ChunkTable& t, uint64_t g, hipStream_t s);
vxg_status fl_plain_32(int W, Epi epi, const ChunkTable& t, uint64_t g, hipStream_t s);
vxg_status fl_plain_64(int W, Epi epi, const ChunkTable& t, uint64_t g, hipStream_t s);
vxg_status fl_alp(int T, int W, Epi epi, const ChunkTable& t, uint64_t g, hipStream_t s);
vxg_status launch_dict_rows(int T, int W, const ChunkTable& tab, hipStream_t s);
#define VXG_DECL_DICT(VW) vxg_status fl_dict_##VW(int T, int W, const ChunkTable& t, uint64_t g, hipStream_t s);
VXG_DECL_DICT(1)
VXG_DECL_DICT(2)
VXG_DECL_DICT(4)
VXG_DECL_DICT(8)
#undef VXG_DECL_DICT
constexpr int kDictFusedMaxW = 16;
vxg_status launch_delta(int width, const void* bases, const void* deltas, uint64_t n_deltas,
                        uint64_t offset, uint64_t len, void* out, hipStream_t s);
struct RunEndChunk {
    IntCol ends;
    IntCol values;
    void* out;
    uint64_t n_runs;
    uint64_t offset;
    uint64_t len;
    uint64_t first_group;
};
vxg_status launch_runend(int value_width, const RunEndChunk& chunk, uint32_t* err, hipStream_t s);
constexpr uint64_t kRunEndSpan = 4096;
constexpr int kRunEndArgChunks = 32;
struct RunEndTable {
    RunEndChunk c[kRunEndArgChunks];
    uint32_t n;
    uint32_t* err;
    const RunEndChunk* ext;
};
vxg_status launch_runend_chunks(int value_width, const RunEndTable& t, uint64_t groups, hipStream_t s);
constexpr uint64_t kRunEndShortRun = 16;
constexpr uint64_t kRunEndRunsPerGroup = 1024;
vxg_status launch_runend_runs(int value_width, const RunEndTable& t, uint64_t groups, hipStream_t s);

struct VarBinChunk {
    const uint8_t* src;
    uint8_t* dst;
    const void* offsets;
    uint8_t* views;
    uint64_t bytes;
    uint64_t n;
    uint64_t first_group;
    uint32_t offs_width;
    uint32_t bidx;
};
constexpr int kVarBinArgChunks = 48;
struct VarBinTable {
    VarBinChunk c[kVarBinArgChunks];
    uint32_t n;
    const VarBinChunk* ext;
    uint32_t* err;
};
vxg_status launch_varbin_chunks(const VarBinTable& t, uint64_t groups, hipStream_t s);

vxg_status launch_copy_bytes(void* dst, const void* src, uint64_t n, hipStream_t s);
vxg_status launch_fill(int value_width, const uint8_t* scalar16, uint64_t n, void* out,
                       hipStream_t s);
struct FsstChunk {
    const uint64_t* symbols;
    const uint8_t* sym_lens;
    const uint8_t* codes;
    const uint8_t* validity;
    uint8_t* heap;
    uint8_t* views;
    IntCol offs;
    IntCol lens;
    uint64_t n;
    uint64_t heap_len;
    uint64_t first_tile;
    uint64_t first_scan;
    uint32_t n_symbols;
    uint32_t bidx;
};
constexpr int kFsstArgChunks = 24;
struct FsstTable {
    FsstChunk c[kFsstArgChunks];
    uint32_t n;
    const FsstChunk* ext;
};
uint64_t fsst_scratch_bytes(uint64_t n);
uint64_t fsst_batch_scratch_bytes(const FsstChunk* chunks, size_t n_chunks);
struct FsstFusedArgs {
    const FsstChunk* ext;
    const int64_t* tp;
    const int64_t* bt;
    const int64_t* tc;
    const uint32_t* wg_chunk;
    uint64_t tiles;
    uint64_t mix;
    uint64_t prepass;
    uint64_t delay;
    const uint32_t* scan_chunk;
    uint32_t tag;
};
bool is_fsst_fused_kernel(const void* func);
struct FsstFused {
    bool valid = false;
    int oa = 0, la = 0;
    FsstFusedArgs a{};
};
hipError_t fsst_diag_init();
vxg_status launch_fsst_batch(std::vector<FsstChunk>& chunks, void* scratch, uint32_t* err, hipStream_t s,
                             DevTables* dt = nullptr, FsstFused* fuse = nullptr);
vxg_status launch_varbin_views(const uint8_t* heap, uint64_t heap_len, int offs_width, const void* offsets, uint64_t n,
                               const uint8_t* validity, uint32_t bidx, uint8_t* views, uint32_t* err, hipStream_t s);
vxg_status launch_views_rebase(const uint8_t* src, uint64_t n, uint32_t add, uint8_t* dst, hipStream_t s);

}
```

Measured before the change: 4847.

## Pack kernarg chunk table into compact ChunkArg entries and add direct chunk lookup

Replaces the 80+-byte ChunkDev entries in the kernel-argument chunk table with a packed 40-byte ChunkArg. This raises the in-argument chunk capacity from 32 to 96, so more chunks can be decoded in one launch without spilling to a device-side external table. Kernels expand the compact entry back into a ChunkDev, recomputing the ALP factors from stored exponents. A groups-per-entry fast path replaces the binary search when all chunks have equal group counts. The costs are the per-block expansion work and new host-side validation limits on length, shift and dictionary size.

Result: no change. 4871 (median of 6 runs) (+0.5%).

```diff
diff --git a/include/vortex_gpu.h b/include/vortex_gpu.h
--- a/include/vortex_gpu.h
+++ b/include/vortex_gpu.h
@@ -122,7 +122,8 @@
 typedef enum vxg_option {
     VXG_OPT_K1W_MIN_GROUPS = 1,
     VXG_OPT_K1W_BPW = 2,
-    VXG_OPT_K1_WAVE = 3
+    VXG_OPT_K1_WAVE = 3,
+    VXG_OPT_K1_ARG_CHUNKS = 4
 } vxg_option;
 vxg_status vxg_set_option(vxg_ctx* ctx, int option, int64_t value);
 vxg_status vxg_get_option(vxg_ctx* ctx, int option, int64_t* value);
diff --git a/rust/vortex-gpu/src/ffi.rs b/rust/vortex-gpu/src/ffi.rs
--- a/rust/vortex-gpu/src/ffi.rs
+++ b/rust/vortex-gpu/src/ffi.rs
@@ -247,6 +247,7 @@
 pub const VXG_OPT_K1W_MIN_GROUPS: vxg_option = 1;
 pub const VXG_OPT_K1W_BPW: vxg_option = 2;
 pub const VXG_OPT_K1_WAVE: vxg_option = 3;
+pub const VXG_OPT_K1_ARG_CHUNKS: vxg_option = 4;
 
 #[repr(C)]
 #[derive(Copy, Clone, Debug)]
diff --git a/vortex_amd/_lib.py b/vortex_amd/_lib.py
--- a/vortex_amd/_lib.py
+++ b/vortex_amd/_lib.py
@@ -143,7 +143,7 @@
 PLAN_SELECTION = {0: "single", 1: "faster", 2: "tie_fewer_nodes", 3: "unmeasured"}
 
 
-OPT_K1W_MIN_GROUPS, OPT_K1W_BPW, OPT_K1_WAVE = 1, 2, 3
+OPT_K1W_MIN_GROUPS, OPT_K1W_BPW, OPT_K1_WAVE, OPT_K1_ARG_CHUNKS = 1, 2, 3, 4
 
 
 class VxgLaunchStats(C.Structure):
diff --git a/vortex_amd/arrays.py b/vortex_amd/arrays.py
--- a/vortex_amd/arrays.py
+++ b/vortex_amd/arrays.py
@@ -457,7 +457,7 @@
         _lib.check(self.lib.vxg_stream_sync(self.handle, self.stream_ptr()))
 
     _OPTIONS = {"k1w_min_groups": _lib.OPT_K1W_MIN_GROUPS, "k1w_bpw": _lib.OPT_K1W_BPW,
-                "k1_wave": _lib.OPT_K1_WAVE}
+                "k1_wave": _lib.OPT_K1_WAVE, "k1_arg_chunks": _lib.OPT_K1_ARG_CHUNKS}
 
     def set_option(self, name: str, value: int):
         _lib.check(self.lib.vxg_set_option(self.handle, self._OPTIONS[name], int(value)))
diff --git a/vortex_amd/csrc/capi.hip b/vortex_amd/csrc/capi.hip
--- a/vortex_amd/csrc/capi.hip
+++ b/vortex_amd/csrc/capi.hip
@@ -128,6 +128,8 @@
         if (value < -1 || value > 2) return set_error(VXG_ERR_INVALID_ARGUMENT, "K1_WAVE must be -1, 0, 1 or 2");
         o.k1_wave = value;
         return VXG_OK;
+    case VXG_OPT_K1_ARG_CHUNKS:
+        return set_error(VXG_ERR_INVALID_ARGUMENT, "K1_ARG_CHUNKS is read-only");
     }
     return set_error(VXG_ERR_INVALID_ARGUMENT, "unknown option " + std::to_string(option));
 }
@@ -139,6 +141,7 @@
     case VXG_OPT_K1W_MIN_GROUPS: *value = o.k1w_min_groups; return VXG_OK;
     case VXG_OPT_K1W_BPW: *value = o.k1w_bpw; return VXG_OK;
     case VXG_OPT_K1_WAVE: *value = o.k1_wave; return VXG_OK;
+    case VXG_OPT_K1_ARG_CHUNKS: *value = kArgChunks; return VXG_OK;
     }
     return set_error(VXG_ERR_INVALID_ARGUMENT, "unknown option " + std::to_string(option));
 }
@@ -291,6 +294,8 @@
     a.shift = for_shift;
     a.alp_a = f32 ? double(kF10f[f]) : kF10d[f];
     a.alp_b = f32 ? double(kIF10f[e]) : kIF10d[e];
+    a.alp_e = uint8_t(e);
+    a.alp_f = uint8_t(f);
     return bitunpack_common(ctx, f32 ? 32 : 64, bit_width, offset, len, packed, packed_bytes,
                             f32 ? Epi::AlpF32 : Epi::AlpF64, 0, a, out, stream);
 }
diff --git a/vortex_amd/csrc/chunk_pack.hpp b/vortex_amd/csrc/chunk_pack.hpp
--- a/vortex_amd/csrc/chunk_pack.hpp
+++ b/vortex_amd/csrc/chunk_pack.hpp
@@ -7,33 +7,49 @@
 
 namespace vxg {
 
+template <class Tab>
+constexpr size_t kPlanArgCap = sizeof(Tab::c) / sizeof(Tab::c[0]);
+template <>
+inline constexpr size_t kPlanArgCap<ChunkTable> = 32;
+
+template <class E>
+vxg_status assign_entry(E& dst, const E& src) {
+    dst = src;
+    return VXG_OK;
+}
+
 template <class Tab, class It, class Entry, class Groups>
 vxg_status pack_chunk_table(Tab& tab, It& it, It end, DevTables* dt, Entry entry, Groups groups_of, uint64_t* groups) {
-    using E = std::remove_reference_t<decltype(tab.c[0])>;
+    using D = std::remove_cv_t<std::remove_pointer_t<decltype(tab.ext)>>;
     constexpr size_t cap = sizeof(tab.c) / sizeof(tab.c[0]);
     size_t take = 0;
     for (It k = it; k != end; ++k) take += entry(*k) != nullptr;
-    E* cs = tab.c;
-    if (dt && take > cap) {
+    D* host = nullptr;
+    if (dt && take > kPlanArgCap<Tab>) {
         if (take > 0xFFFFFFFFull) return set_error(VXG_ERR_INVALID_ARGUMENT, "too many chunks");
-        E* host;
         const vxg_status st = dt->table(take, &host, &tab.ext);
         if (st != VXG_OK) return st;
         if constexpr (requires { tab.host; }) tab.host = host;
-        cs = host;
     } else {
         take = std::min(take, cap);
     }
     tab.n = 0;
     *groups = 0;
-    for (; it != end && tab.n < take; ++it) {
-        const E* e = entry(*it);
-        if (!e) continue;
-        E& c = cs[tab.n++];
-        c = *e;
-        c.first_group = *groups;
-        *groups += groups_of(c);
-    }
+    auto fill = [&](auto* cs) -> vxg_status {
+        for (; it != end && tab.n < take; ++it) {
+            const auto* e = entry(*it);
+            if (!e) continue;
+            auto& c = cs[tab.n];
+            const vxg_status st = assign_entry(c, *e);
+            if (st != VXG_OK) return st;
+            tab.n++;
+            c.first_group = static_cast<decltype(c.first_group)>(*groups);
+            *groups += groups_of(c);
+        }
+        return VXG_OK;
+    };
+    const vxg_status st = host ? fill(host) : fill(tab.c);
+    if (st != VXG_OK) return st;
     while (it != end && !entry(*it)) ++it;
     if (*groups > 0xFFFFFFFFull) return set_error(VXG_ERR_INVALID_ARGUMENT, "array too long for one launch");
     return VXG_OK;
diff --git a/vortex_amd/csrc/compare.hip b/vortex_amd/csrc/compare.hip
--- a/vortex_amd/csrc/compare.hip
+++ b/vortex_amd/csrc/compare.hip
@@ -34,35 +34,6 @@
     V s;
     __builtin_memcpy(&s, &bits, sizeof(V));
     return s;
-}
-
-template <Epi EPI>
-__device__ __forceinline__ void alp_factors(uint32_t e, uint32_t f, double& a, double& b) {
-    if constexpr (EPI == Epi::AlpF32) {
-        constexpr float f10[11] = {1.0f, 10.0f, 100.0f, 1000.0f, 10000.0f, 100000.0f, 1000000.0f,
-                                   10000000.0f, 100000000.0f, 1000000000.0f, 10000000000.0f};
-        constexpr float if10[11] = {1.0f, 0.1f, 0.01f, 0.001f, 0.0001f, 0.00001f, 0.000001f,
-                                    0.0000001f, 0.00000001f, 0.000000001f, 0.0000000001f};
-        a = double(f10[f < 11 ? f : 0]);
-        b = double(if10[e < 11 ? e : 0]);
-    } else if constexpr (EPI == Epi::AlpF64) {
-        constexpr double f10[24] = {
-            1.0, 10.0, 100.0, 1000.0, 10000.0, 100000.0, 1000000.0, 10000000.0, 100000000.0,
-            1000000000.0, 10000000000.0, 100000000000.0, 1000000000000.0, 10000000000000.0,
-            100000000000000.0, 1000000000000000.0, 10000000000000000.0, 100000000000000000.0,
-            1000000000000000000.0, 10000000000000000000.0, 100000000000000000000.0,
-            1000000000000000000000.0, 10000000000000000000000.0, 100000000000000000000000.0};
-        constexpr double if10[24] = {
-            1.0, 0.1, 0.01, 0.001, 0.0001, 0.00001, 0.000001, 0.0000001, 0.00000001, 0.000000001,
-            0.0000000001, 0.00000000001, 0.000000000001, 0.0000000000001, 0.00000000000001,
-            0.000000000000001, 0.0000000000000001, 0.00000000000000001, 0.000000000000000001,
-            0.0000000000000000001, 0.00000000000000000001, 0.000000000000000000001,
-            0.0000000000000000000001, 0.00000000000000000000001};
-        a = f10[f < 24 ? f : 0];
-        b = if10[e < 24 ? e : 0];
-    } else {
-        a = b = 0.0;
-    }
 }
 
 template <int T, Epi EPI, int CK, int OP>
diff --git a/vortex_amd/csrc/dict_rows.hip b/vortex_amd/csrc/dict_rows.hip
--- a/vortex_amd/csrc/dict_rows.hip
+++ b/vortex_amd/csrc/dict_rows.hip
@@ -16,18 +16,10 @@
     using V = typename DVal<VW>::t;
     constexpr unsigned LANES = 1024 / T;
     const uint64_t g = blockIdx.x;
-    uint32_t ci;
-    if constexpr (EXT) {
-        ci = ext_chunk_index(tab.ext, tab.n, g, [](const ChunkDev& d) { return d.first_group; });
-    } else {
-        uint32_t lo = 0, hi = tab.n;
-        while (hi - lo > 1) {
-            const uint32_t mid = (lo + hi) >> 1;
-            if (tab.c[mid].first_group <= g) lo = mid; else hi = mid;
-        }
-        ci = lo;
-    }
-    const ChunkDev& c = EXT ? tab.ext[ci] : tab.c[ci];
+    ChunkDev ca;
+    if constexpr (!EXT) ca = expand_chunk<Epi::Dict>(tab.c[arg_chunk_index(tab, blockIdx.x)]);
+    const ChunkDev& c =
+        EXT ? tab.ext[ext_chunk_index(tab.ext, tab.n, g, [](const ChunkDev& d) { return d.first_group; })] : ca;
     __shared__ __attribute__((aligned(16))) E s_packed[BPW * 128 * kRowsMaxW / sizeof(E)];
     __shared__ __attribute__((aligned(16))) uint8_t s_dict[LDSD ? kDictLdsBytes : 16];
     const unsigned tid = threadIdx.x;
@@ -66,12 +58,7 @@
 
 template <int T, int VW, int BPW, bool LDSD, bool EXT>
 vxg_status launch_rows(ChunkTable tab, unsigned W, hipStream_t s) {
-    ChunkDev* cs = tab.ext ? tab.host : tab.c;
-    uint64_t groups = 0;
-    for (uint32_t k = 0; k < tab.n; k++) {
-        cs[k].first_group = groups;
-        groups += (cs[k].n_blocks + BPW - 1) / BPW;
-    }
+    const uint64_t groups = set_first_groups(tab, uint64_t(BPW));
     if (groups == 0) return VXG_OK;
     if (groups > 0xFFFFFFFFull) return set_error(VXG_ERR_INVALID_ARGUMENT, "array too long for one launch");
     hipLaunchKernelGGL((dict_rows_kernel<T, VW, BPW, LDSD, EXT>), dim3(unsigned(groups)), dim3(kRowsThreads), 0, s,
@@ -87,13 +74,13 @@
 
 template <int T, int VW>
 vxg_status launch_rows_t(const ChunkTable& tab, unsigned W, hipStream_t s) {
-    const ChunkDev* cs = tab.ext ? tab.host : tab.c;
     bool lds = true;
     uint64_t max_dict = 0;
-    for (uint32_t k = 0; k < tab.n; k++) {
-        lds = lds && cs[k].dict_len * VW <= uint64_t(kDictLdsBytes) && (reinterpret_cast<uintptr_t>(cs[k].dict) & 15) == 0;
-        max_dict = cs[k].dict_len * VW > max_dict ? cs[k].dict_len * VW : max_dict;
-    }
+    for_each_chunk(tab, [&](const auto& c) {
+        const uint64_t bytes = chunk_dict_len(c) * VW;
+        lds = lds && bytes <= uint64_t(kDictLdsBytes) && (reinterpret_cast<uintptr_t>(chunk_dict(c)) & 15) == 0;
+        max_dict = bytes > max_dict ? bytes : max_dict;
+    });
     if (lds && max_dict > 1024) return launch_rows_b<T, VW, 8>(tab, W, lds, s);
     return launch_rows_b<T, VW, 1>(tab, W, lds, s);
 }
diff --git a/vortex_amd/csrc/fl_unpack_impl.hpp b/vortex_amd/csrc/fl_unpack_impl.hpp
--- a/vortex_amd/csrc/fl_unpack_impl.hpp
+++ b/vortex_amd/csrc/fl_unpack_impl.hpp
@@ -323,6 +323,79 @@
                                                           std::make_integer_sequence<int, T / S>{});
     if constexpr (EPI == Epi::Dict)
         if (oob) __hip_atomic_fetch_or(ep.err, kErrTakeOOB, __ATOMIC_RELAXED, __HIP_MEMORY_SCOPE_AGENT);
+}
+
+template <Epi EPI>
+__device__ __forceinline__ void alp_factors(uint32_t e, uint32_t f, double& a, double& b) {
+    if constexpr (EPI == Epi::AlpF32) {
+        constexpr float f10[11] = {1.0f, 10.0f, 100.0f, 1000.0f, 10000.0f, 100000.0f, 1000000.0f,
+                                   10000000.0f, 100000000.0f, 1000000000.0f, 10000000000.0f};
+        constexpr float if10[11] = {1.0f, 0.1f, 0.01f, 0.001f, 0.0001f, 0.00001f, 0.000001f,
+                                    0.0000001f, 0.00000001f, 0.000000001f, 0.0000000001f};
+        a = double(f10[f < 11 ? f : 0]);
+        b = double(if10[e < 11 ? e : 0]);
+    } else if constexpr (EPI == Epi::AlpF64) {
+        constexpr double f10[24] = {
+            1.0, 10.0, 100.0, 1000.0, 10000.0, 100000.0, 1000000.0, 10000000.0, 100000000.0,
+            1000000000.0, 10000000000.0, 100000000000.0, 1000000000000.0, 10000000000000.0,
+            100000000000000.0, 1000000000000000.0, 10000000000000000.0, 100000000000000000.0,
+            1000000000000000000.0, 10000000000000000000.0, 100000000000000000000.0,
+            1000000000000000000000.0, 10000000000000000000000.0, 100000000000000000000000.0};
+        constexpr double if10[24] = {
+            1.0, 0.1, 0.01, 0.001, 0.0001, 0.00001, 0.000001, 0.0000001, 0.00000001, 0.000000001,
+            0.0000000001, 0.00000000001, 0.000000000001, 0.0000000000001, 0.00000000000001,
+            0.000000000000001, 0.0000000000000001, 0.00000000000000001, 0.000000000000000001,
+            0.0000000000000000001, 0.00000000000000000001, 0.000000000000000000001,
+            0.0000000000000000000001, 0.00000000000000000000001};
+        a = f10[f < 24 ? f : 0];
+        b = if10[e < 24 ? e : 0];
+    } else {
+        a = b = 0.0;
+    }
+}
+
+template <Epi EPI>
+__device__ __forceinline__ ChunkDev expand_chunk(const ChunkArg& a) {
+    ChunkDev c;
+    c.packed = a.packed;
+    c.out = a.out;
+    c.len = a.len();
+    c.offset = a.offset;
+    c.n_blocks = a.n_blocks();
+    c.first_group = a.first_group;
+    if constexpr (EPI == Epi::Dict) {
+        c.reference = 0;
+        c.shift = 0;
+        c.dict = reinterpret_cast<const void*>(uintptr_t(a.ref_or_dict));
+        c.dict_len = a.aux;
+    } else {
+        c.reference = a.ref_or_dict;
+        c.shift = a.aux & 0xFFu;
+        c.dict = nullptr;
+        c.dict_len = 0;
+    }
+    alp_factors<EPI>((a.aux >> 8) & 0xFFu, (a.aux >> 16) & 0xFFu, c.alp_a, c.alp_b);
+    return c;
+}
+
+__device__ __forceinline__ uint32_t arg_chunk_index(const ChunkTable& tab, uint32_t g) {
+    const uint32_t n = tab.n;
+    uint32_t lo = 0;
+    if (n > 1) {
+        if (tab.gpe) {
+            const uint32_t q = g / tab.gpe;
+            const uint32_t ci = __builtin_amdgcn_readfirstlane(q < n - 1 ? q : n - 1);
+            const uint32_t nx = ci + 1 < n ? ci + 1 : ci;
+            const uint32_t f0 = tab.c[ci].first_group, f1 = tab.c[nx].first_group;
+            if (f0 <= g && (nx == ci || g < f1)) return ci;
+        }
+        uint32_t hi = n;
+        while (hi - lo > 1) {
+            const uint32_t mid = (lo + hi) >> 1;
+            if (tab.c[mid].first_group <= g) lo = mid; else hi = mid;
+        }
+    }
+    return lo;
 }
 
 constexpr int kDictLdsBytes = 16 * 1024;
@@ -618,12 +691,8 @@
             tab.ext[ext_chunk_index(tab.ext, tab.n, g, [](const ChunkDev& d) { return d.first_group; })];
         unpack_chunk_w<T, W, EPI, VW, LDSD>(c, g, tab.err, PatchCol{}, tab.bpw);
     } else {
-        uint32_t lo = 0, hi = tab.n;
-        while (hi - lo > 1) {
-            const uint32_t mid = (lo + hi) >> 1;
-            if (tab.c[mid].first_group <= g) lo = mid; else hi = mid;
-        }
-        unpack_chunk_w<T, W, EPI, VW, LDSD>(tab.c[lo], g, tab.err, tab.patch, tab.bpw);
+        const ChunkDev c = expand_chunk<EPI>(tab.c[arg_chunk_index(tab, blockIdx.x)]);
+        unpack_chunk_w<T, W, EPI, VW, LDSD>(c, g, tab.err, tab.patch, tab.bpw);
     }
 }
 
@@ -635,15 +704,30 @@
             tab.ext[ext_chunk_index(tab.ext, tab.n, g, [](const ChunkDev& d) { return d.first_group; })];
         unpack_chunk<T, W, EPI, VW, LDSD, S>(c, g, tab.err);
     } else {
-        uint32_t lo = 0, hi = tab.n;
-        while (hi - lo > 1) {
-            const uint32_t mid = (lo + hi) >> 1;
-            if (tab.c[mid].first_group <= g) lo = mid; else hi = mid;
-        }
-        unpack_chunk<T, W, EPI, VW, LDSD, S>(tab.c[lo], g, tab.err);
-    }
-}
-
+        const ChunkDev c = expand_chunk<EPI>(tab.c[arg_chunk_index(tab, blockIdx.x)]);
+        unpack_chunk<T, W, EPI, VW, LDSD, S>(c, g, tab.err);
+    }
+}
+
+
+template <class Tab, class F>
+void for_each_chunk(Tab& tab, F f) {
+    if (tab.ext) for (uint32_t k = 0; k < tab.n; k++) f(tab.host[k]);
+    else for (uint32_t k = 0; k < tab.n; k++) f(tab.c[k]);
+}
+inline uint64_t set_first_groups(ChunkTable& tab, uint64_t bpg) {
+    uint64_t groups = 0, cnt[kArgChunks];
+    uint32_t k = 0;
+    for_each_chunk(tab, [&](auto& c) {
+        const uint64_t n = (chunk_blocks(c) + bpg - 1) / bpg;
+        c.first_group = static_cast<decltype(c.first_group)>(groups);
+        if (!tab.ext) cnt[k++] = n;
+        groups += n;
+    });
+    const uint64_t gpe = tab.ext ? 0 : common_groups(cnt, tab.n);
+    tab.gpe = gpe <= 0xFFFFFFFFull ? uint32_t(gpe) : 0;
+    return groups;
+}
 
 inline int k1w_pick_bpw(uint64_t blocks, int bpw_max, int64_t min_groups, int64_t forced) {
     if (forced > 0) return int(forced < bpw_max ? forced : bpw_max);
@@ -656,18 +740,18 @@
 template <int T, int W, Epi EPI, int VW, bool LDSD, bool EXT>
 vxg_status launch_w(ChunkTable tab, hipStream_t s) {
     constexpr int BPW_MAX = kw_bpw(W, LDSD);
-    ChunkDev* cs = tab.ext ? tab.host : tab.c;
     uint64_t blocks = 0;
-    for (uint32_t k = 0; k < tab.n; k++) blocks += cs[k].n_blocks;
+    for_each_chunk(tab, [&](const auto& c) { blocks += chunk_blocks(c); });
     const Options o = cur_options();
     const int BPW = k1w_pick_bpw(blocks, BPW_MAX, o.k1w_min_groups, o.k1w_bpw);
     tab.bpw = uint32_t(BPW);
-    uint64_t groups = 0, dict_bytes = 0;
-    for (uint32_t k = 0; k < tab.n; k++) {
-        cs[k].first_group = groups;
-        groups += (cs[k].n_blocks + BPW - 1) / BPW;
-        const uint64_t db = (cs[k].dict_len * uint64_t(VW > 0 ? VW : 1) + 15) & ~15ull;
-        dict_bytes = db > dict_bytes ? db : dict_bytes;
+    const uint64_t groups = set_first_groups(tab, uint64_t(BPW));
+    uint64_t dict_bytes = 0;
+    if constexpr (EPI == Epi::Dict) {
+        for_each_chunk(tab, [&](const auto& c) {
+            const uint64_t db = (chunk_dict_len(c) * uint64_t(VW > 0 ? VW : 1) + 15) & ~15ull;
+            dict_bytes = db > dict_bytes ? db : dict_bytes;
+        });
     }
     if (groups == 0) return VXG_OK;
     if (groups > 0xFFFFFFFFull) return set_error(VXG_ERR_INVALID_ARGUMENT, "array too long for one launch");
@@ -684,12 +768,7 @@
 
 template <int T, int W, Epi EPI, int VW, bool LDSD, int S, bool EXT = false>
 vxg_status launch_s(ChunkTable tab, hipStream_t s) {
-    ChunkDev* cs = tab.ext ? tab.host : tab.c;
-    uint64_t groups = 0;
-    for (uint32_t k = 0; k < tab.n; k++) {
-        cs[k].first_group = groups;
-        groups += (cs[k].n_blocks + (32 / S) - 1) / (32 / S);
-    }
+    const uint64_t groups = set_first_groups(tab, uint64_t(32 / S));
     if (groups == 0) return VXG_OK;
     if (groups > 0xFFFFFFFFull) return set_error(VXG_ERR_INVALID_ARGUMENT, "array too long for one launch");
     hipLaunchKernelGGL((fl_unpack_kernel<T, W, EPI, VW, LDSD, S, EXT>), dim3(unsigned(groups)), dim3(256), 0, s, tab);
@@ -703,11 +782,11 @@
     const bool split = kSplit && groups32 < split_below_groups();
     bool lds = false;
     if constexpr (EPI == Epi::Dict) {
-        const ChunkDev* cs = tab.ext ? tab.host : tab.c;
         lds = true;
-        for (uint32_t k = 0; k < tab.n; k++)
-            lds = lds && cs[k].dict_len * VW <= uint64_t(kDictLdsBytes) &&
-                  (reinterpret_cast<uintptr_t>(cs[k].dict) & 15) == 0;
+        for_each_chunk(tab, [&](const auto& c) {
+            lds = lds && chunk_dict_len(c) * VW <= uint64_t(kDictLdsBytes) &&
+                  (reinterpret_cast<uintptr_t>(chunk_dict(c)) & 15) == 0;
+        });
     }
     constexpr uint64_t kExtWaveGroups = 128;
     const int mode = k1_wave_mode();
diff --git a/vortex_amd/csrc/planner.hpp b/vortex_amd/csrc/planner.hpp
--- a/vortex_amd/csrc/planner.hpp
+++ b/vortex_amd/csrc/planner.hpp
@@ -37,6 +37,7 @@
     Epi epi;
     int vw;
     ChunkDev d;
+    uint8_t alp_e = 0, alp_f = 0;
     bool vb = false;
     VarBinChunk vbc{};
 };
diff --git a/vortex_amd/csrc/planner_decode.hip b/vortex_amd/csrc/planner_decode.hip
--- a/vortex_amd/csrc/planner_decode.hip
+++ b/vortex_amd/csrc/planner_decode.hip
@@ -139,6 +139,8 @@
     UnpackArgs ua{};
     ua.alp_a = f32 ? double(kF10f[f]) : kF10d[f];
     ua.alp_b = f32 ? double(kIF10f[e]) : kIF10d[e];
+    ua.alp_e = uint8_t(e);
+    ua.alp_f = uint8_t(f);
     const Epi epi = f32 ? Epi::AlpF32 : Epi::AlpF64;
     const vxg_array* bp = nullptr;
     if (enc->encoding == VXG_ENC_FL_FOR && child(*enc, 0) &&
diff --git a/vortex_amd/csrc/planner_launch.hip b/vortex_amd/csrc/planner_launch.hip
--- a/vortex_amd/csrc/planner_launch.hip
+++ b/vortex_amd/csrc/planner_launch.hip
@@ -5,7 +5,6 @@
 #include "k1g.hpp"
 #include "planner.hpp"
 
-static_assert(sizeof(vxg::ChunkTable) <= 4096, "ChunkTable exceeds the kernarg limit");
 static_assert(sizeof(vxg::FsstTable) <= 4096, "FsstTable exceeds the kernarg limit");
 static_assert(sizeof(vxg::RunEndTable) <= 4096, "RunEndTable exceeds the kernarg limit");
 static_assert(sizeof(vxg::VarBinTable) <= 4096, "VarBinTable exceeds the kernarg limit");
@@ -61,6 +60,40 @@
         return set_error(VXG_ERR_INVALID_ARGUMENT, "bad dictionary value width");
     }
     return VXG_ERR_INVALID_ARGUMENT;
+}
+
+vxg_status assign_entry(ChunkDev& dst, const K1Job& jb) {
+    dst = jb.d;
+    return VXG_OK;
+}
+vxg_status assign_entry(ChunkArg& dst, const K1Job& jb) {
+    const ChunkDev& d = jb.d;
+    if (d.len > kArgMaxLen) return set_error(VXG_ERR_INVALID_ARGUMENT, "array too long for one launch");
+    dst = ChunkArg{};
+    dst.packed = d.packed;
+    dst.out = d.out;
+    dst.len_lo = uint32_t(d.len);
+    dst.len_hi = uint16_t(d.len >> 32);
+    dst.offset = uint16_t(d.offset);
+    if (jb.epi == Epi::Dict) {
+        if (d.dict_len > 0xFFFFFFFFull)
+            return set_error(VXG_ERR_INVALID_ARGUMENT, "dictionary too long for a fused decode (>= 2^32 values)");
+        dst.ref_or_dict = uint64_t(reinterpret_cast<uintptr_t>(d.dict));
+        dst.aux = uint32_t(d.dict_len);
+        return VXG_OK;
+    }
+    if (d.shift > 0xFFu) return set_error(VXG_ERR_INVALID_ARGUMENT, "FoR shift out of range");
+    dst.ref_or_dict = d.reference;
+    dst.aux = d.shift;
+    if (jb.epi == Epi::AlpF32 || jb.epi == Epi::AlpF64) {
+        const bool f32 = jb.epi == Epi::AlpF32;
+        const unsigned e = jb.alp_e, f = jb.alp_f, lim = f32 ? 11 : 24;
+        if (e >= lim || f >= lim || d.alp_a != (f32 ? double(kF10f[f]) : kF10d[f]) ||
+            d.alp_b != (f32 ? double(kIF10f[e]) : kIF10d[e]))
+            return set_error(VXG_ERR_INVALID_ARGUMENT, "internal: ALP exponents do not match the factors");
+        dst.aux |= uint32_t(e) << 8 | uint32_t(f) << 16;
+    }
+    return VXG_OK;
 }
 
 static bool same_kernel(const K1Job& a, const K1Job& b) {
@@ -92,8 +125,8 @@
             if (patch && jobs.size() == 1) tab.patch = *patch;
             uint64_t groups;
             VXG_TRY(pack_chunk_table(
-                tab, it, end, dt, [](const K1Job& jb) { return jb.d.n_blocks ? &jb.d : nullptr; },
-                [](const ChunkDev& c) { return (c.n_blocks + 31) / 32; }, &groups));
+                tab, it, end, dt, [](const K1Job& jb) { return jb.d.n_blocks ? &jb : nullptr; },
+                [](const auto& c) { return (chunk_blocks(c) + 31) / 32; }, &groups));
             if (tab.n) VXG_TRY(launch_fl_unpack(jobs[i].T, jobs[i].W, jobs[i].epi, jobs[i].vw, tab, groups, s));
         }
         return VXG_OK;
@@ -218,6 +251,8 @@
     j.d.dict_len = a.dict_len;
     j.d.offset = offset;
     j.d.shift = a.shift;
+    j.alp_e = a.alp_e;
+    j.alp_f = a.alp_f;
     return VXG_OK;
 }
 
diff --git a/vortex_amd/csrc/vxg_internal.hpp b/vortex_amd/csrc/vxg_internal.hpp
--- a/vortex_amd/csrc/vxg_internal.hpp
+++ b/vortex_amd/csrc/vxg_internal.hpp
@@ -201,6 +201,7 @@
     const void* dict;
     uint64_t dict_len;
     uint32_t* err;
+    uint8_t alp_e, alp_f;
 };
 
 struct ChunkDev {
@@ -216,7 +217,27 @@
     uint32_t offset;
     uint32_t shift;
 };
-constexpr int kArgChunks = 32;
+struct ChunkArg {
+    const uint8_t* packed;
+    void* out;
+    uint64_t ref_or_dict;
+    uint32_t len_lo;
+    uint32_t first_group;
+    uint32_t aux;
+    uint16_t offset;
+    uint16_t len_hi;
+    __host__ __device__ uint64_t len() const { return uint64_t(len_lo) | uint64_t(len_hi) << 32; }
+    __host__ __device__ uint64_t n_blocks() const { return len() ? (len() + offset + 1023) / 1024 : 0; }
+};
+static_assert(sizeof(ChunkArg) == 40, "ChunkArg is packed to 40 bytes");
+constexpr uint64_t kArgMaxLen = (uint64_t(1) << 48) - 1;
+__host__ __device__ inline uint64_t chunk_blocks(const ChunkDev& c) { return c.n_blocks; }
+__host__ __device__ inline uint64_t chunk_blocks(const ChunkArg& c) { return c.n_blocks(); }
+inline const void* chunk_dict(const ChunkDev& c) { return c.dict; }
+inline const void* chunk_dict(const ChunkArg& c) { return reinterpret_cast<const void*>(uintptr_t(c.ref_or_dict)); }
+inline uint64_t chunk_dict_len(const ChunkDev& c) { return c.dict_len; }
+inline uint64_t chunk_dict_len(const ChunkArg& c) { return c.aux; }
+constexpr int kArgChunks = 96;
 struct ChunkTable;
 
 vxg_status launch_fl_unpack(int T, int W, Epi epi, int value_width, const ChunkTable& tab, uint64_t groups,
@@ -240,14 +261,17 @@
 };
 
 struct ChunkTable {
-    ChunkDev c[kArgChunks];
+    ChunkArg c[kArgChunks];
     uint32_t n;
+    uint32_t gpe;
     uint32_t* err;
     const ChunkDev* ext;
     ChunkDev* host;
     PatchCol patch;
     uint32_t bpw;
 };
+static_assert(sizeof(ChunkTable) <= 4096, "ChunkTable exceeds the kernarg limit");
+static_assert(sizeof(ChunkTable) + 32 * sizeof(ChunkArg) > 4096, "kArgChunks is the largest multiple of 32 that fits");
 
 extern thread_local bool g_k1w_wrote_patches;
 
```
